# Acelogic/Retrieval-based-Voice-Conversion-MLX

Hardware: AMD Instinct MI355X
Metric: audio-sec/sec (realtime factor) RVCv2 48kHz pipeline (higher is better)
Workload: dtype fp32-accurate (two-plane fp16 MFMA split); 1 GPU; C2: full RVCv2 48kHz pipeline, one 13.5 s utterance per step per GPU; samples_16k=216100, x_pad=1, f0_method=rmvpe, parallelism=dp1

## Files before the change

### retrieval-based-voice-conversion-mlx_amd/csrc/aux_kernels.hip

```cpp
#include <algorithm>
#include <cmath>
#include <cstdlib>

#include "dd_math.h"
#include "rvcx_kernels.h"

namespace rvcx {

namespace {

constexpr int TB = 256;
typedef float f32x4v __attribute__((ext_vector_type(4)));

inline unsigned nblocks(long long n, int per = TB) {
  long long b = (n + per - 1) / per;
  if (b > 65535LL * 32) b = 65535LL * 32;
  return (unsigned)(b < 1 ? 1 : b);
}

__device__ __forceinline__ float warp_sum(float v) {
#pragma unroll
  for (int o = 32; o > 0; o >>= 1) v += __shfl_xor(v, o, 64);
  return v;
}
// ... 306 lines not shown
    const int src = t >> 1 < L ? t >> 1 : L - 1;
    const float f = feats[(long long)src * D + c];
    float v = f;
    if (pitchf) {
      const float pf = pitchf[t];
      const float p = pf < 1.f ? protect : (pf > 0.f ? 1.f : pf);
      v = f * p + feats0[(long long)src * D + c] * (1.f - p);
    }
    out[i] = v;
  }
}
#pragma clang fp contract(on)
hipError_t upsample2_protect(const float* feats, const float* feats0, int L, int D, float* out, int T,
                             const float* pitchf, float protect, hipStream_t s) {
  hipLaunchKernelGGL(k_up2, dim3(nblocks((long long)T * D)), dim3(TB), 0, s, feats, feats0, L, D, out, T, pitchf,
                     protect);
  return hipGetLastError();
}

constexpr int SINE_T = 1024;
__global__ __launch_bounds__(SINE_T) void k_sine_cum(const float* __restrict__ f0, int B, int L, int upp, float sr,
                                                     double* __restrict__ cum) {
  __shared__ double wsum[SINE_T / 64];
  const int b = blockIdx.x;
  const float* fb = f0 + (long long)b * L;
  float* cf = reinterpret_cast<float*>(cum + (long long)b * L);
  const int n = L - 1;
  if (n <= 0) return;
  const int per = (n + SINE_T - 1) / SINE_T;
  const int j0 = min(n, (int)threadIdx.x * per), j1 = min(n, j0 + per);
  auto rem_at = [&](int j) {
    const float inc = (fb[j] / sr) * (float)upp;
    return fmodf(inc + 0.5f, 1.0f) - 0.5f;
  };
  double s = 0.0;
  for (int j = j0; j < j1; ++j) s += (double)rem_at(j);
  const int lane = threadIdx.x & 63, w = threadIdx.x >> 6;
  double v = s;
#pragma unroll
  for (int d = 1; d < 64; d <<= 1) {
    const double u = __shfl_up(v, d);
    if (lane >= d) v += u;
  }
  if (lane == 63) wsum[w] = v;
  __syncthreads();
  double acc = v - s;
  for (int k = 0; k < w; ++k) acc += wsum[k];
  for (int j = j0; j < j1; ++j) {
    acc += (double)rem_at(j);
    cf[j] = fmodf((float)acc, 1.0f);
  }
}
__global__ void k_sine(const float* f0, int B, int L, int upp, float sr, const double* cum, const float* eps,
                       uint64_t seed, float lin_w, float lin_b, float* har, long long har_ld) {
  const long long n = (long long)B * L * upp;
  const float two_pi = 6.283185307179586f;
  const float amp_unv = (float)(0.1 / 3.0);
  for (long long i = blockIdx.x * (long long)blockDim.x + threadIdx.x; i < n; i += (long long)gridDim.x * blockDim.x) {
    const int u = (int)(i % upp);
    const long long bl = i / upp;
    const int b = (int)(bl / L), l = (int)(bl % L);
    const float f = f0[bl];
    float ph = (f / sr) * (float)(u + 1);
    if (l > 0) ph = ph + reinterpret_cast<const float*>(cum + (long long)b * L)[l - 1];
    const float sine = sinf(two_pi * ph) * 0.1f;
    const float uv = f > 0.f ? 1.f : 0.f;
    const float amp = uv * 0.003f + (1.f - uv) * amp_unv;
    const float e = eps ? eps[i] : normal_at(seed, (uint64_t)i);
    const float merged = sine * uv + amp * e;
    har[(long long)b * har_ld + (long long)l * upp + u] = tanhf(merged * lin_w + lin_b);
  }
}
hipError_t sine_source(const float* f0, int B, int L, int upp, float sr, const float* eps, uint64_t seed,
                       float lin_w, float lin_b, double* cum_ws, float* har, long long har_ld, hipStream_t s) {
  hipLaunchKernelGGL(k_sine_cum, dim3(B), dim3(SINE_T), 0, s, f0, B, L, upp, sr, cum_ws);
  hipLaunchKernelGGL(k_sine, dim3(nblocks((long long)B * L * upp)), dim3(TB), 0, s, f0, B, L, upp, sr, cum_ws, eps,
                     seed, lin_w, lin_b, har, har_ld);
  return hipGetLastError();
}

constexpr int CP_T = 256, CP_IT = 24;
__global__ __launch_bounds__(CP_T) void k_conv_post(const float* __restrict__ x, int T, int C,
                                                    const float* __restrict__ wg, int K, float slope,
                                                    float* __restrict__ y, float bias) {
  extern __shared__ float tile[];
  const int b = blockIdx.y;
  const int t0 = blockIdx.x * CP_T;
  const int pad = K / 2;
  const int rows = CP_T + K - 1;
  const int ldt = C + 1;
  const int C4 = C >> 2;
  float* w = tile + rows * ldt;
  for (int i = threadIdx.x; i < C * K; i += blockDim.x) w[i] = wg[i];
  const float* xb = x + (long long)b * T * C;
  f32x4v v[CP_IT];
#pragma unroll
  for (int it = 0; it < CP_IT; ++it) {
    const int idx = it * CP_T + threadIdx.x;
    const int r = idx / C4, c4 = (idx - r * C4) * 4;
    const int g = t0 - pad + r;
    v[it] = (r < rows && g >= 0 && g < T) ? *reinterpret_cast<const f32x4v*>(xb + (long long)g * C + c4)
                                          : f32x4v{0.f, 0.f, 0.f, 0.f};
  }
#pragma unroll
  for (int it = 0; it < CP_IT; ++it) {
    const int idx = it * CP_T + threadIdx.x;
    const int r = idx / C4, c4 = (idx - r * C4) * 4;
    if (r < rows) {
#pragma unroll
      for (int e = 0; e < 4; ++e) {
        const float u = v[it][e];
        tile[r * ldt + c4 + e] = u > 0.f ? u : u * slope;
      }
    }
  }
  __syncthreads();
  const int t = t0 + threadIdx.x;
  if (t >= T) return;
  float acc = 0.f;
  for (int c = 0; c < C; ++c)
    for (int k = 0; k < K; ++k) acc = fmaf(tile[(threadIdx.x + k) * ldt + c], w[c * K + k], acc);
  y[(long long)b * T + t] = tanhf(acc + bias);
}
constexpr int CPF_C = 32, CPF_K = 7, CPF_LD = 36, CPF_ROWS = CP_T + CPF_K - 1;
__global__ __launch_bounds__(CP_T) void k_conv_post32(const float* __restrict__ x, int T,
                                                      const float* __restrict__ wg, float slope,
                                                      float* __restrict__ y, float bias) {
  __shared__ __attribute__((aligned(16))) float tile[CPF_ROWS * CPF_LD];
  __shared__ __attribute__((aligned(16))) float w[CPF_K * CPF_C];
  const int b = blockIdx.y;
  const int t0 = blockIdx.x * CP_T;
  constexpr int pad = CPF_K / 2;
  constexpr int C4 = CPF_C / 4;
  constexpr int IT = (CPF_ROWS * C4 + CP_T - 1) / CP_T;
  if (threadIdx.x < CPF_K * CPF_C) {
    const int k = threadIdx.x / CPF_C, c = threadIdx.x - k * CPF_C;
    w[threadIdx.x] = wg[c * CPF_K + k];
  }
  const float* xb = x + (long long)b * T * CPF_C;
  f32x4v v[IT];
#pragma unroll
  for (int it = 0; it < IT; ++it) {
    const int idx = it * CP_T + threadIdx.x;
    const int r = idx / C4, c4 = (idx - r * C4) * 4;
    const int g = t0 - pad + r;
    const bool ok = r < CPF_ROWS && g >= 0 && g < T;
    v[it] = *reinterpret_cast<const f32x4v*>(xb + (long long)(ok ? g : 0) * CPF_C + c4);
    if (!ok) v[it] = f32x4v{0.f, 0.f, 0.f, 0.f};
  }
#pragma unroll
  for (int it = 0; it < IT; ++it) {
    const int idx = it * CP_T + threadIdx.x;
    const int r = idx / C4, c4 = (idx - r * C4) * 4;
    if (r < CPF_ROWS) {
      f32x4v u = v[it];
#pragma unroll
      for (int e = 0; e < 4; ++e) u[e] = u[e] > 0.f ? u[e] : u[e] * slope;
      *reinterpret_cast<f32x4v*>(&tile[r * CPF_LD + c4]) = u;
    }
  }
  __syncthreads();
  const int t = t0 + threadIdx.x;
  if (t >= T) return;
  f32x4v acc = {0.f, 0.f, 0.f, 0.f};
#pragma unroll
  for (int c4 = 0; c4 < C4; ++c4)
#pragma unroll
    for (int k = 0; k < CPF_K; ++k) {
      const f32x4v xv = *reinterpret_cast<const f32x4v*>(&tile[(threadIdx.x + k) * CPF_LD + 4 * c4]);
      const f32x4v wv = *reinterpret_cast<const f32x4v*>(&w[k * CPF_C + 4 * c4]);
#pragma unroll
      for (int e = 0; e < 4; ++e) acc[e] = fmaf(xv[e], wv[e], acc[e]);
    }
  y[(long long)b * T + t] = tanhf(((acc[0] + acc[1]) + (acc[2] + acc[3])) + bias);
}

hipError_t conv_post_tanh(const float* x, int B, int T, int C, const float* w, int K, float slope, float* y,
                          hipStream_t s, float bias) {
  if (C == CPF_C && K == CPF_K && (reinterpret_cast<uintptr_t>(x) & 15) == 0) {
    hipLaunchKernelGGL(k_conv_post32, dim3((T + CP_T - 1) / CP_T, B), dim3(CP_T), 0, s, x, T, w, slope, y, bias);
    return hipGetLastError();
  }
  if (C % 4 != 0 || (long long)(CP_T + K - 1) * (C / 4) > (long long)CP_IT * CP_T ||
      (reinterpret_cast<uintptr_t>(x) & 15) != 0)
    return hipErrorInvalidValue;
  const size_t smem = ((size_t)(CP_T + K - 1) * (C + 1) + (size_t)C * K) * sizeof(float);
  hipLaunchKernelGGL(k_conv_post, dim3((T + CP_T - 1) / CP_T, B), dim3(CP_T), smem, s, x, T, C, w, K, slope, y, bias);
  return hipGetLastError();
}

__global__ void k_zp(const float* stats, int B, int T, int I, const float* eps, uint64_t seed, const float* mask,
                     float* zp) {
  const long long n = (long long)B * T * I;
  for (long long i = blockIdx.x * (long long)blockDim.x + threadIdx.x; i < n; i += (long long)gridDim.x * blockDim.x) {
    const int c = (int)(i % I);
    const long long bt = i / I;
    const int b = (int)(bt / T), t = (int)(bt % T);
    const float m = stats[bt * 2 * I + c];
    const float lg = stats[bt * 2 * I + I + c];
    const long long ei = ((long long)b * I + c) * T + t;
    const float e = eps ? eps[ei] : normal_at(seed, (uint64_t)ei);
    zp[i] = (m + expf(lg) * e * 0.66666f) * mask[bt];
  }
}
hipError_t zp_sample(const float* stats, int B, int T, int I, const float* eps, uint64_t seed, const float* mask,
                     float* zp, hipStream_t s) {
  hipLaunchKernelGGL(k_zp, dim3(nblocks((long long)B * T * I)), dim3(TB), 0, s, stats, B, T, I, eps, seed, mask, zp);
  return hipGetLastError();
}

__global__ void k_gn_stats(const float* x, int T, int C, int chunk, double* ws) {
  const int c = blockIdx.x * 64 + (threadIdx.x & 63);
  const int rl = threadIdx.x >> 6;
  const int t0 = blockIdx.y * chunk;
  const int t1 = min(T, t0 + chunk);
  x += (long long)blockIdx.z * T * C;
  ws += (long long)blockIdx.z * gridDim.y * C * 2;
  double s = 0.0, q = 0.0;
  if (c < C) {
    for (int t = t0 + rl; t < t1; t += 4) {
      const double v = x[(long long)t * C + c];
      s += v;
      q += v * v;
    }
  }
  __shared__ double ss[4][64], qq[4][64];
  ss[rl][threadIdx.x & 63] = s;
  qq[rl][threadIdx.x & 63] = q;
  __syncthreads();
  if (rl == 0 && c < C) {
    s = ss[0][threadIdx.x] + ss[1][threadIdx.x] + ss[2][threadIdx.x] + ss[3][threadIdx.x];
    q = qq[0][threadIdx.x] + qq[1][threadIdx.x] + qq[2][threadIdx.x] + qq[3][threadIdx.x];
    ws[((long long)blockIdx.y * C + c) * 2] = s;
    ws[((long long)blockIdx.y * C + c) * 2 + 1] = q;
  }
}
__global__ void k_gn_finalize(const double* ws, int nchunks, int T, int C, const float* gamma, const float* beta,
                              float eps, float* ss) {
  const int c = blockIdx.x * 64 + (threadIdx.x & 63);
  const int rl = threadIdx.x >> 6;
  ws += (long long)blockIdx.y * nchunks * C * 2;
  ss += (long long)blockIdx.y * 2 * C;
  double s = 0.0, q = 0.0;
  if (c < C) {
    for (int k = rl; k < nchunks; k += 4) {
      s += ws[((long long)k * C + c) * 2];
      q += ws[((long long)k * C + c) * 2 + 1];
    }
  }
  __shared__ double sp[4][64], qp[4][64];
  sp[rl][threadIdx.x & 63] = s;
  qp[rl][threadIdx.x & 63] = q;
  __syncthreads();
  if (rl != 0 || c >= C) return;
  s = ((sp[0][threadIdx.x] + sp[1][threadIdx.x]) + sp[2][threadIdx.x]) + sp[3][threadIdx.x];
  q = ((qp[0][threadIdx.x] + qp[1][threadIdx.x]) + qp[2][threadIdx.x]) + qp[3][threadIdx.x];
  const double mean = s / T;
  double var = q / T - mean * mean;
  if (var < 0) var = 0;
  const float rstd = (float)(1.0 / sqrt(var + (double)eps));
  const float scale = rstd * gamma[c];
  ss[c] = scale;
  ss[C + c] = beta[c] - (float)mean * scale;
}
__global__ void k_gn_apply(float* __restrict__ x, unsigned n4, unsigned n4_per, unsigned C4, const float* __restrict__ ss,
                           int C) {
  for (unsigned i = blockIdx.x * blockDim.x + threadIdx.x; i < n4; i += gridDim.x * blockDim.x) {
    const int c = (int)(i % C4) * 4;
    const float* sb = ss + (size_t)(i / n4_per) * 2 * C;
    f32x4v v = reinterpret_cast<f32x4v*>(x)[i];
// ... 660 lines not shown
```

### retrieval-based-voice-conversion-mlx_amd/csrc/capi.cpp

```cpp
#include <algorithm>
#include <cmath>
#include <cstdio>
#include <cstdlib>
#include <cstring>
#include <string>
#include <unistd.h>
#include <vector>

#include "../../include/rvcx_test.h"
#include "runtime.h"

extern char** environ;

using namespace rvcx;

namespace rvcx {
static bool experimental_on() {
  const char* e = std::getenv("RVCX_EXPERIMENTAL");
  return e && std::atoi(e) == 1;
}
const char* rvcx_knob(const char* name) { return experimental_on() ? std::getenv(name) : nullptr; }
}

struct rvcx_ctx : public Ctx {};
// ... 160 lines not shown
  if (c.conv_math > 0 && b.math == 0) b.math = c.conv_math;
  if (!(b.w_static || c.is_weight(b.w)) || b.force_cfg >= 0) return false;
  if (!(conv_math_of(b) == 3 || b.lowp)) return false;
  if (conv_wsb_route(b, false) != 1) return false;
  b.wsb = 1;
  return conv_plan_splitk(b, false) == 0 && conv_wsb_pick(b) >= 23;
}

void launch_conv(Ctx& c, const ConvArgs& a_in, bool two_d, hipStream_t s, double flops) {
  ConvArgs a = a_in;
  if (c.conv_math > 0 && a.math == 0) a.math = c.conv_math;
  const bool stat = a.w_static || c.is_weight(a.w);
  a.wsb = !stat ? 0
          : (a.force_cfg >= 30 && a.force_cfg < 40 ? 2
             : (a.force_cfg >= 20 && !two_d) ? 1 : (a.force_cfg < 0 ? conv_wsb_route(a, two_d) : 0));
  if (a.force_cfg == 40 && !two_d && stat) a.wsb = 1;
  const long long need = conv_plan_splitk(a, two_d);
  if (two_d && !a.wsb && stat && !a.wsplit && conv_math_of(a) == 3 && conv2d_small_fits(a)) {
    a.wsplit_fmt = WSPLIT_S2D;
    a.wsplit = c.wsplit_for(a, s);
  }
  if (a.wsb) {
    if (!a.wsplit)
      a.wsplit_fmt = ((a.wsb == 1 && a.lowp) || conv_math_of(a) == 3) ? WSPLIT_H16 : WSPLIT_BF16;
    if (!a.wsplit) a.wsplit = c.wsplit_for(a, s);
    a.wsplit_npad = conv_wsplit_npad(a.N);
  }
  static const int aux_lds = [] {
    const char* e = rvcx_knob("RVCX_AUX_LDS");
    return e ? std::max(0, std::atoi(e)) : 64;
  }();
  if (aux_lds > 0 && c.aux_front) a.lds_pad = aux_lds * 1024;
  if (need > 0) {
    a.ws = c.buf<float>(c.aux && s == c.aux ? "conv.splitk.aux" : "conv.splitk", (size_t)need, s);
  }
  if (flops < 0) {
    const double M = two_d ? (double)a.T_out * a.W_out : (double)a.T_out;
    flops = 2.0 * M * a.N * (double)a.C_in * a.taps * a.batch * a.batch_inner;
  }
  if (!c.prof) {
    check(two_d ? conv2d(a, s) : conv1d(a, s), two_d ? "conv2d" : "conv1d");
    return;
  }
  auto get_ev = [&]() {
    hipEvent_t e;
    if (!c.prof_pool.empty()) {
      e = c.prof_pool.back();
      c.prof_pool.pop_back();
    } else {
      RVCX_HIP(hipEventCreate(&e));
    }
    return e;
  };
  const double in_rows = two_d ? (double)a.T_in * a.W_in : (double)a.T_in;
  const double out_el = (two_d ? (double)a.T_out * a.W_out : (double)a.T_out) * a.N * a.batch * a.batch_inner;
  const double alg_bytes = 4.0 * (in_rows * a.C_in * a.batch * a.batch_inner + (double)a.taps * a.N * a.C_in +
                                  out_el * (1 + (a.res && a.res_mode != RES_NONE ? 1 : 0) +
                                            (a.acc_mode != ACC_STORE ? 1 : 0)));
  const double peak = (a.wsb && a.wsplit_fmt == WSPLIT_H16) ? ((a.lowp && a.wsb == 1) ? Ctx::PEAK_F16 : Ctx::PEAK_F16X2)
                      : (a.wsplit && a.wsplit_fmt == WSPLIT_S2D) ? Ctx::PEAK_F16X2
                                                                  : Ctx::PEAK_SPLIT;
  Ctx::ProfRec r{get_ev(), get_ev(), flops, two_d ? 1 : 0, two_d ? a.T_out * a.W_out : a.T_out, a.N, a.C_in,
                 a.taps, a.batch * a.batch_inner, a.ksplit, alg_bytes, peak};
  RVCX_HIP(hipEventRecord(r.a, s));
  check(two_d ? conv2d(a, s) : conv1d(a, s), two_d ? "conv2d" : "conv1d");
  r.kind = conv_last_kind();
  RVCX_HIP(hipEventRecord(r.b, s));
  c.prof_recs.push_back(r);
}

__global__ void k_set_i32(int32_t* p, int32_t v) { p[0] = v; }
void set_i32(int32_t* p, int32_t v, hipStream_t s) {
  hipLaunchKernelGGL(k_set_i32, dim3(1), dim3(1), 0, s, p, v);
  check(hipGetLastError(), "set_i32");
}
void set_i32_once(Ctx& c, const std::string& name, int32_t* p, int32_t v, hipStream_t s) {
  auto it = c.i32_marks.find(name);
  if (it != c.i32_marks.end() && it->second.first == p && it->second.second == v) return;
  set_i32(p, v, s);
  c.i32_marks[name] = {p, v};
}
}

extern "C" {

int rvcx_create(rvcx_ctx** out, int device) {
  if (!out) return RVCX_E_INVALID;
  *out = nullptr;
  int n = 0;
  if (hipGetDeviceCount(&n) != hipSuccess || device < 0 || device >= n) return RVCX_E_HIP;
  auto* c = new rvcx_ctx();
  c->device = device;
  *out = c;
  return RVCX_OK;
}

int rvcx_destroy(rvcx_ctx* ctx) {
  if (!ctx) return RVCX_E_INVALID;
  (void)hipSetDevice(ctx->device);
  (void)hipDeviceSynchronize();
  delete ctx;
  return RVCX_OK;
}

const char* rvcx_last_error(const rvcx_ctx* ctx) { return ctx ? ctx->err.c_str() : "null context"; }

int rvcx_set_synth_config(rvcx_ctx* ctx, const rvcx_synth_desc* d) {
  return guard(ctx, [&] {
    if (!d) throw Error(RVCX_E_INVALID, "null desc");
    SynthCfg g;
    g.I = d->inter_channels;
    g.H = d->hidden_channels;
    g.F = d->filter_channels;
    g.n_heads = d->n_heads;
    g.n_layers = d->n_layers;
    g.ksize = d->kernel_size;
    if (d->n_resblocks < 1 || d->n_resblocks > 4 || d->n_dilations < 1 || d->n_dilations > 4)
      throw Error(RVCX_E_INVALID, "resblock config out of range");
    g.rb_k.assign(d->resblock_kernel_sizes, d->resblock_kernel_sizes + d->n_resblocks);
    g.rb_d.clear();
    for (int j = 0; j < d->n_resblocks; ++j)
      g.rb_d.emplace_back(d->resblock_dilation_sizes[j], d->resblock_dilation_sizes[j] + d->n_dilations);
    if (d->n_upsample < 1 || d->n_upsample > 8) throw Error(RVCX_E_INVALID, "n_upsample out of range");
    g.ups.assign(d->upsample_rates, d->upsample_rates + d->n_upsample);
    g.up_k.assign(d->upsample_kernel_sizes, d->upsample_kernel_sizes + d->n_upsample);
    g.C0 = d->upsample_initial_channel;
    g.n_spk = d->spk_embed_dim;
    g.gin = d->gin_channels;
    g.sr = d->sr;
    g.emb_dim = d->text_enc_hidden_dim;
    g.f0 = d->no_f0 == 0;
    g.vocoder = d->vocoder;
    if (g.vocoder < 0 || g.vocoder > 2) throw Error(RVCX_E_INVALID, "unsupported vocoder id");
    if (!g.f0 && g.vocoder != 0)
      throw Error(RVCX_E_INVALID, "models without pitch guidance use the HiFi-GAN decoder only (synthesizers.py:119-139)");
    if (g.H % g.n_heads || g.I % 2 || g.C0 % (1 << g.ups.size()))
      throw Error(RVCX_E_INVALID, "inconsistent synthesizer dimensions");
    ctx->scfg = g;
    ctx->synth_cfg_set = true;
    ctx->ready[0] = false;
  });
}

int rvcx_upload(rvcx_ctx* ctx, int model, const char* name, const float* host, const int64_t* shape, int ndim) {
  return guard(ctx, [&] {
    if (model < 0 || model > RVCX_MODEL_FCPE || !name || !host || (ndim > 0 && !shape) || ndim < 0 || ndim > 8)
      throw Error(RVCX_E_INVALID, "rvcx_upload: bad arguments");
    HostTensor t;
    size_t n = 1;
    for (int i = 0; i < ndim; ++i) {
      if (shape[i] < 0) throw Error(RVCX_E_INVALID, "negative dim");
      t.shape.push_back(shape[i]);
      n *= (size_t)shape[i];
    }
    t.v.assign(host, host + n);
    ctx->host[model][name] = std::move(t);
    ctx->ready[model] = false;
  });
}

int rvcx_finalize(rvcx_ctx* ctx, int model) {
  return guard(ctx, [&] {
    set_device(ctx);
    if (model == RVCX_MODEL_SYNTH) {
      finalize_synth(*ctx);
    } else if (model == RVCX_MODEL_HUBERT) {
      finalize_hubert(*ctx);
    } else if (model == RVCX_MODEL_RMVPE) {
      finalize_rmvpe(*ctx);
    } else if (model == RVCX_MODEL_CREPE) {
      finalize_crepe(*ctx);
    } else if (model == RVCX_MODEL_FCPE) {
      finalize_fcpe(*ctx);
    } else {
      throw Error(RVCX_E_INVALID, "unknown model");
    }
    RVCX_HIP(hipDeviceSynchronize());
    ctx->ready[model] = true;
  });
}

int rvcx_synth_upp(const rvcx_ctx* ctx) { return ctx ? ctx->scfg.upp() : 0; }

int rvcx_hubert(rvcx_ctx* ctx, const float* d_audio, int64_t n, int version, float* d_feats, int64_t cap_rows,
                int64_t* rows_out, void* stream) {
  return guard(ctx, [&] {
    if (!ctx->ready[1]) throw Error(RVCX_E_STATE, "hubert weights not finalized");
    if (!d_audio || !d_feats || n <= 0) throw Error(RVCX_E_INVALID, "rvcx_hubert: bad arguments");
    set_device(ctx);
    const int64_t L = hubert_forward(*ctx, d_audio, n, version == 1 ? 1 : 2, d_feats, cap_rows,
                                     static_cast<hipStream_t>(stream));
    if (rows_out) *rows_out = L;
  });
}

int rvcx_rmvpe(rvcx_ctx* ctx, const float* d_audio, int64_t n, float thred, double* d_f0, int64_t cap_frames,
               int64_t* frames_out, float* d_hidden, void* stream) {
  return guard(ctx, [&] {
    if (!ctx->ready[2]) throw Error(RVCX_E_STATE, "rmvpe weights not finalized");
    if (!d_audio || !d_f0 || n <= 0) throw Error(RVCX_E_INVALID, "rvcx_rmvpe: bad arguments");
    set_device(ctx);
    const int64_t F = rmvpe_forward(*ctx, d_audio, n, thred, d_f0, cap_frames, d_hidden,
                                    static_cast<hipStream_t>(stream));
    if (frames_out) *frames_out = F;
  });
}

int rvcx_crepe(rvcx_ctx* ctx, const float* d_audio, int64_t n, float f0_min, float f0_max, float threshold,
               float* d_f0, float* d_periodicity, float* d_probs, int64_t cap_frames, int64_t* frames_out,
               void* stream) {
  return guard(ctx, [&] {
    if (!ctx->ready[RVCX_MODEL_CREPE]) throw Error(RVCX_E_STATE, "crepe weights not finalized");
    if (!d_audio || !d_f0 || n <= 0) throw Error(RVCX_E_INVALID, "rvcx_crepe: bad arguments");
    if (cap_frames < 1 + n / 160) throw Error(RVCX_E_SHAPE, "rvcx_crepe: output capacity below 1 + n/160 frames");
    set_device(ctx);
    const int64_t F = crepe_forward(*ctx, d_audio, n, f0_min, f0_max, threshold, d_f0, nullptr, d_periodicity,
                                    d_probs, static_cast<hipStream_t>(stream));
    if (frames_out) *frames_out = F;
  });
}

// ... 381 lines not shown
    try {
      RVCX_HIP(hipMalloc(&audio.p, sizeof(double) * (size_t)(B * n)));
      RVCX_HIP(hipMalloc(&out.p, sizeof(float) * (size_t)(B * cap)));
      RVCX_HIP(hipMemsetAsync(audio.p, 0, sizeof(double) * (size_t)(B * n), s));
      auto measure = [&](const rvcx_pipeline_opts& o) {
        if (B == 1) {
          pipeline_forward_ex(*ctx, static_cast<const double*>(audio.p), n, o, nullptr, nullptr, 0,
                              static_cast<float*>(out.p), cap, nullptr, s);
        } else {
          std::vector<int32_t> sids((size_t)B, o.sid);
          pipeline_forward_batch(*ctx, static_cast<const double*>(audio.p), n, n, B, o, sids.data(), nullptr, nullptr, 0,
                                 static_cast<float*>(out.p), cap, nullptr, nullptr, s);
        }
        RVCX_HIP(hipStreamSynchronize(s));
        return (int64_t)ctx->carved;
      };
      need = measure(*opts);
      if (opts->f0_method == 3) {
        rvcx_pipeline_opts o0 = *opts;
        o0.f0_method = 0;
        ctx->release_pool();
        need = std::max(need, measure(o0));
      }
      if (B == 1 && opts->t_max > 0 && n + 160 > opts->t_max && opts->t_center > 0) {
        const int64_t nts = n > opts->t_center ? (n - 1 - opts->t_center) / opts->t_center + 1 : 0;
        need += (nts + 1) * ((int64_t)ctx->scfg.emb_dim * 4 + 512);
      }
    } catch (...) {
      ctx->release_pool();
      ctx->arena = arena;
      ctx->arena_bytes = arena_bytes;
      throw;
    }
    ctx->release_pool();
    ctx->arena = arena;
    ctx->arena_bytes = arena_bytes;
    *bytes = need;
  });
}

int rvcx_device_status(rvcx_ctx* ctx, void* stream) {
  return guard(ctx, [&] {
    RVCX_HIP(hipSetDevice(ctx->device));
    RVCX_HIP(hipStreamSynchronize(static_cast<hipStream_t>(stream)));
    if (ctx->aux) RVCX_HIP(hipStreamSynchronize(ctx->aux));
    ctx->check_device_status();
  });
}

int rvcx_index_parse(const void* bytes, int64_t nbytes, int64_t* d, int64_t* ntotal, int64_t* nlist,
                     int64_t* nprobe, char* err, int64_t err_cap) {
  try {
    if (!bytes || nbytes <= 0) throw Error(RVCX_E_INVALID, "index_parse: empty buffer");
    const ParsedIvf P = parse_ivf(static_cast<const uint8_t*>(bytes), nbytes);
    if (d) *d = P.d;
    if (ntotal) *ntotal = P.ntotal;
    if (nlist) *nlist = P.nlist;
    if (nprobe) *nprobe = P.nprobe;
    if (err && err_cap > 0) err[0] = 0;
    return RVCX_OK;
  } catch (const Error& e) {
    if (err && err_cap > 0) std::snprintf(err, (size_t)err_cap, "%s", e.what());
    return e.code;
  } catch (const std::exception& e) {
    if (err && err_cap > 0) std::snprintf(err, (size_t)err_cap, "%s", e.what());
    return RVCX_E_INVALID;
  }
}

int rvcx_set_conv_math(rvcx_ctx* ctx, int mode) {
  return guard(ctx, [&] {
    if (mode < 0 || mode > 3) throw Error(RVCX_E_INVALID, "conv math mode must be 0, 1, 2 or 3");
    ctx->conv_math = mode;
  });
}

int rvcx_config_info(const rvcx_ctx* ctx, char* buf, int64_t cap, int64_t* len) {
  std::string j = "{\"arch\": \"gfx950\"";
  if (ctx) j += ", \"conv_math_ctx\": " + std::to_string(ctx->conv_math);
  const char* cm = rvcx_knob("RVCX_CONV_MATH");
  j += ", \"conv_math_default\": \"" + std::string(cm ? cm : "h16") + "\"";
  j += ", \"experimental\": " + std::string(experimental_on() ? "true" : "false");
  if (ctx) j += ", \"arena_bytes\": " + std::to_string(ctx->arena_bytes);
  j += ", \"env\": {";
  bool first = true;
  for (char** e = environ; e && *e; ++e) {
    if (std::strncmp(*e, "RVCX_", 5) != 0) continue;
    const char* eq = std::strchr(*e, '=');
    if (!eq) continue;
    std::string k(*e, eq - *e), v(eq + 1);
    std::string ve;
    for (char ch : v)
      if (ch != '"' && ch != '\\' && (unsigned char)ch >= 32) ve += ch;
    const bool honoured = k == "RVCX_EXPERIMENTAL" || k == "RVCX_PROF_DUMP" || k == "RVCX_LIB" || experimental_on();
    j += std::string(first ? "" : ", ") + "\"" + k + "\": {\"value\": \"" + ve + "\", \"honoured\": " +
         (honoured ? "true" : "false") + "}";
    first = false;
  }
  j += "}}";
  if (len) *len = (int64_t)j.size();
  if (buf && cap > 0) {
    const size_t n = std::min<size_t>(j.size(), (size_t)cap - 1);
    std::memcpy(buf, j.data(), n);
    buf[n] = 0;
  }
  return (int64_t)j.size() < cap || !buf ? RVCX_OK : RVCX_E_CAPACITY;
}

int rvcx_set_generator_precision(rvcx_ctx* ctx, int) {
  return guard(ctx, [&] {
    throw Error(RVCX_E_INVALID,
                "rvcx_set_generator_precision was removed: set rvcx_rt_opts.gen_precision per streaming hop instead");
  });
}

int rvcx_conv1d(rvcx_ctx* ctx, const float* d_x, int64_t T, int C_in, const float* d_w, const float* d_bias, int N,
                int taps, int dilation, int pad, int stride, int math, float* d_y, int64_t T_out, void* stream) {
  return guard(ctx, [&] {
    set_device(ctx);
    ctx->check_device_status();
    if (!d_x || !d_w || !d_y || T <= 0 || C_in <= 0 || N <= 0 || taps <= 0 || dilation <= 0 || stride <= 0 ||
        pad < 0 || T_out <= 0 || math < 0 || math > 7)
      throw Error(RVCX_E_INVALID, "rvcx_conv1d: bad argument");
    if ((T_out - 1) * stride + (int64_t)(taps - 1) * dilation + 1 > T + 2 * (int64_t)pad)
      throw Error(RVCX_E_SHAPE, "rvcx_conv1d: T_out exceeds the padded input");
    if (T > INT32_MAX || T_out > INT32_MAX || (int64_t)taps * N * C_in > INT32_MAX)
      throw Error(RVCX_E_SHAPE, "rvcx_conv1d: size out of range");
    ConvArgs a;
    a.x = d_x; a.ldx = C_in; a.T_in = (int)T; a.C_in = C_in;
    a.w = d_w; a.ldw = C_in; a.w_ts = (long long)N * C_in; a.taps = taps; a.dil = dilation; a.pad = pad;
    a.stride = stride;
    a.y = d_y; a.ldy = N; a.T_out = (int)T_out; a.N = N; a.bias = d_bias;
    a.math = math >= 5 ? 3 : (math >= 3 ? 2 : math);
    if (math == 7) a.wsplit_fmt = WSPLIT_H16;
    if (math == 5 || math == 6) {
      a.wsplit_fmt = WSPLIT_H16;
      a.lowp = math == 6;
    }
    if (math == 3 || math == 5 || math == 6) {
      if (!conv_wsb_eligible(a)) throw Error(RVCX_E_SHAPE, "rvcx_conv1d: shape not eligible for the weight-streamed kernel");
      a.w_static = 1;
      a.force_cfg = conv_wsb_pick(a);
      a.no_splitk = 1;
      void* img = ctx->buf<char>("conv.test.wsplit", (size_t)conv_wsplit_bytes(a), static_cast<hipStream_t>(stream));
      check(conv_wsplit_build(a, img, static_cast<hipStream_t>(stream)), "conv_wsplit_build");
      a.wsplit = img;
    }
    if (math == 4 || math == 7) {
      if (!conv_gs_eligible(a, false)) throw Error(RVCX_E_SHAPE, "rvcx_conv1d: shape not eligible for the gather-streamed kernel");
      a.w_static = 1;
      a.force_cfg = 30;
      void* img = ctx->buf<char>("conv.test.wsplit", (size_t)conv_wsplit_bytes(a), static_cast<hipStream_t>(stream));
      check(conv_wsplit_build(a, img, static_cast<hipStream_t>(stream)), "conv_wsplit_build");
      a.wsplit = img;
    }
    launch_conv(*ctx, a, false, static_cast<hipStream_t>(stream), -1.0);
  });
}

int rvcx_conv1d_gen(rvcx_ctx* ctx, const float* d_x, int64_t T, int C_in, const float* d_w, const float* d_bias,
                    int N, int taps, int dilation, int pad, int pre_act, float pre_slope, int act, float slope,
                    const float* d_res, int acc_mode, float acc_div, int kernel, float* d_y, void* stream) {
  return guard(ctx, [&] {
    set_device(ctx);
    ctx->check_device_status();
    if (!d_x || !d_w || !d_y || T <= 0 || C_in <= 0 || N <= 0 || taps <= 0 || dilation <= 0 || pad < 0 || act < 0 ||
        act > 1 || pre_act < 0 || pre_act > 1 || acc_mode < 0 || acc_mode > 2 || kernel < 0 || kernel > 2 || (d_res && d_res == d_x))
      throw Error(RVCX_E_INVALID, "rvcx_conv1d_gen: bad argument");
    const int64_t T_out = T + 2 * (int64_t)pad - (int64_t)(taps - 1) * dilation;
    if (T_out <= 0 || T > INT32_MAX || (int64_t)taps * N * C_in > INT32_MAX)
      throw Error(RVCX_E_SHAPE, "rvcx_conv1d_gen: size out of range");
    ConvArgs a;
    a.x = d_x; a.ldx = C_in; a.T_in = (int)T; a.C_in = C_in;
    a.w = d_w; a.ldw = C_in; a.w_ts = (long long)N * C_in; a.taps = taps; a.dil = dilation; a.pad = pad;
    a.y = d_y; a.ldy = N; a.T_out = (int)T_out; a.N = N; a.bias = d_bias;
    a.pre_act = pre_act ? ACT_LRELU : ACT_NONE;
    a.pre_slope = pre_slope;
    a.act = act ? ACT_LRELU : ACT_NONE;
    a.slope = slope;
    if (d_res) {
      a.res = d_res;
      a.ldr = N;
      a.res_mode = RES_ADD_POST;
    }
    a.acc_mode = acc_mode == 0 ? ACC_STORE : (acc_mode == 1 ? ACC_ADD : ACC_ADD_DIV);
    a.acc_div = acc_div;
    a.math = 3;
    a.wsplit_fmt = WSPLIT_H16;
    a.w_static = 1;
// ... 474 lines not shown
```

### retrieval-based-voice-conversion-mlx_amd/csrc/conv_dispatch.hip

```cpp
#include <algorithm>
#include <cstdlib>
#include <string>

#include "conv_common.h"

namespace rvcx {

constexpr int CK = 32;

namespace {

inline int env_cfg(const char* name, int dflt) {
  const char* e = rvcx_knob(name);
  return e ? std::atoi(e) : dflt;
}
inline int conv_math(const ConvArgs& a) {
  static const int env = [] {
    const char* e = rvcx_knob("RVCX_CONV_MATH");
    if (e && (std::string(e) == "f32" || std::string(e) == "1")) return 1;
    if (e && (std::string(e) == "split" || std::string(e) == "2")) return 2;
    return 3;
  }();
  return a.math > 0 ? a.math : env;
}

template <bool TWO_D>
int pick_emu(const ConvArgs& a) {
  if (TWO_D) return a.N <= 32 ? 12 : 13;
  if (a.N <= 32) return a.taps >= 5 ? 12 : 1;
  if (a.taps >= 5) return 12;
  return 13;
}

template <bool TWO_D>
int pick_cfg(const ConvArgs& a) {
  if (a.force_cfg >= 0) return a.force_cfg;
  if (conv_math(a) >= 2) return pick_emu<TWO_D>(a);
  if (a.N <= 32) return 1;
  if (!TWO_D && a.taps >= 5) return 1;
  return 3;
}

inline void cfg_tile(int cfg, int& BM, int& BN) {
  if (conv_emu_tile(cfg, BM, BN)) return;
  static const int t[10][2] = {{256, 32}, {128, 32}, {128, 64}, {64, 64}, {128, 128}, {64, 128}, {256, 64},
                               {64, 64}, {128, 32}, {128, 128}};
  BM = t[cfg][0];
  BN = t[cfg][1];
}

inline int pick_wsb(const ConvArgs& a) {
  static const int c_long = env_cfg("RVCX_WCFG_LONG", 0);
  if (a.wsb == 2) return 30;
  if (a.N <= 32) return 24;
  if (a.taps <= 3 && a.N >= 1024 && a.T_out >= 8192 && a.C_in < 512 && c_long == 0) return 25;
  if (a.taps <= 3) return 27;
  if (c_long > 0) return c_long;
  return (a.C_in < 256 && a.N >= 128) ? 25 : 23;
}
}
int conv_wsb_pick(const ConvArgs& a) {
  ConvArgs b = a;
  b.wsb = 1;
  return pick_wsb(b);
}
thread_local int g_conv_kind = CK_OTHER;
int conv_last_kind() { return g_conv_kind; }
const char* conv_kind_name(int k) {
  static const char* const names[CK_COUNT] = {"conv_wsb16_kernel", "conv_wsb_kernel", "conv_gs16_kernel",
                                              "conv_gsw16_kernel", "k_rb_pair", "k_conv2d_h16/k_conv2d_small",
                                              "conv_emu_kernel", "conv_gemm_kernel", "conv_tiny_kernel",
                                              "conv_wst16_kernel", "other"};
  return (k >= 0 && k < CK_COUNT) ? names[k] : "other";
}

namespace {

template <bool TWO_D>
hipError_t dispatch(const ConvArgs& a_in, hipStream_t s) {
  const ConvArgs& a = a_in;
  if (a.N <= 0 || a.T_out <= 0 || a.batch <= 0) return hipSuccess;
  if (a.C_in <= 0 || a.taps <= 0) return hipErrorInvalidValue;
  const bool nz = a.nz_har != nullptr;
  if (nz && (TWO_D || (a.ws && a.ksplit > 1) || a.nz_C <= 0 || a.nz_stride <= 0 ||
             a.nz_kk != 1 ||
             a.N != a.nz_u * a.nz_C || a.out_map != OUT_ROWS))
    return hipErrorInvalidValue;
  if ((a.gate_h > 0 || a.ln_g) && !(a.ws && a.ksplit > 1)) return hipErrorInvalidValue;
  if (tiny_fits(a)) {
    if (nz) return hipErrorInvalidValue;
    g_conv_kind = CK_TINY;
    return launch_tiny(a, TWO_D, s);
  }
  if (!nz && !(a.ws && a.ksplit > 1) && rows1x1_fits(a, TWO_D)) {
    g_conv_kind = CK_TINY;
    return launch_rows1x1(a, TWO_D, s);
  }
  if (a.wsb == 2 && a.wsplit && conv_math(a) >= 2 && conv_gs_eligible(a, TWO_D)) {
    const int ks = (a.ws && a.ksplit > 1) ? a.ksplit : 1;
    const int cfg = a.force_cfg >= 30 ? a.force_cfg : pick_wsb(a);
    g_conv_kind = (TWO_D && cfg == 30 && conv_gsw_eligible(a)) ? CK_GSW : CK_GS;
    hipError_t e = conv_gs_launch(a, cfg, s, TWO_D, ks);
    if (e == hipSuccess && ks > 1) e = launch_splitk_reduce(a, ks, TWO_D, s);
    if (e != hipErrorInvalidValue) return e;
  }
  if (a.wsb == 1 && a.wsplit && conv_math(a) >= 2 && conv_wsb_eligible(a, TWO_D)) {
    const int ks = (a.ws && a.ksplit > 1) ? a.ksplit : 1;
    if (ks == 1 && (a.force_cfg < 20 || a.force_cfg == 40) && conv_wst_fits(a, TWO_D)) {
      g_conv_kind = CK_WST;
      hipError_t e = conv_wst_launch(a, s);
      if (e != hipErrorInvalidValue) return e;
    }
    const int cfg = a.force_cfg >= 20 && a.force_cfg < 40 ? a.force_cfg : pick_wsb(a);
    g_conv_kind = CK_WSB16;
    hipError_t e = conv_wsb_launch(a, cfg, s, TWO_D, ks);
    if (e == hipSuccess && ks > 1) e = launch_splitk_reduce(a, ks, TWO_D, s);
    if (e != hipErrorInvalidValue) return e;
  }
  if (nz) return hipErrorInvalidValue;
  if (TWO_D && a.force_cfg < 0 && conv2d_small_fits(a)) {
    g_conv_kind = CK_SMALL2D;
    return conv2d_small(a, s);
  }
  const int cfg = pick_cfg<TWO_D>(a);
  const bool emu = cfg >= 10;
  g_conv_kind = emu ? CK_EMU : CK_GEMM;
  const bool gemm = !TWO_D && a.taps == 1 && a.stride == 1;
  const bool pipe = gemm && a.pipe >= 0;
  const int ksplit = (a.ws && a.ksplit > 1) ? a.ksplit : 1;
  auto run = [&](int c, bool p) -> hipError_t {
    hipError_t e = emu ? conv_emu_launch(a, c, TWO_D, p, ksplit, s) : conv_gemm_launch(a, c, TWO_D, p, ksplit, s);
    if (e != hipSuccess || ksplit == 1) return e;
    return launch_splitk_reduce(a, ksplit, TWO_D, s);
  };
  hipError_t e = run(cfg, pipe);
  if (e == hipErrorInvalidValue && pipe) e = run(cfg, false);
  if (e == hipErrorInvalidValue && a.force_cfg < 0) {
    for (int alt : {emu ? 13 : 3, emu ? 12 : 1}) {
      if (alt == cfg) continue;
      e = run(alt, false);
      if (e != hipErrorInvalidValue) break;
    }
  }
  return e;
}

}

long long conv_plan_splitk(ConvArgs& a, bool two_d) {
  a.ksplit = 1;
  if (a.N <= 0 || a.T_out <= 0 || a.no_splitk) return 0;
  if (tiny_fits(a)) return 0;
  if (two_d && a.force_cfg < 0 && conv2d_small_fits(a)) return 0;
  int BM, BN;
  if (a.wsb == 2) {
    conv_gs_tile(a.force_cfg >= 30 ? a.force_cfg : pick_wsb(a), BM, BN);
  } else if (a.wsb) {
    if (!conv_wsb_tile(a.force_cfg >= 20 ? a.force_cfg : pick_wsb(a), BM, BN)) return 0;
  } else {
    cfg_tile(two_d ? pick_cfg<true>(a) : pick_cfg<false>(a), BM, BN);
  }
  long long mtiles;
  if (!two_d) {
    mtiles = (a.T_out + BM - 1) / BM;
  } else {
    const int rw = a.W_out < BM ? a.W_out : BM;
    const int rh = BM / rw;
    mtiles = (long long)((a.T_out + rh - 1) / rh) * ((a.W_out + rw - 1) / rw);
  }
  const long long tiles = mtiles * ((a.N + BN - 1) / BN) * a.batch * a.batch_inner;
  const int iters = ((a.C_in + CK - 1) / CK) * a.taps;
  const double M = two_d ? (double)a.T_out * a.W_out : (double)a.T_out;
  const double flops = 2.0 * M * a.N * (double)a.C_in * a.taps * a.batch * a.batch_inner;
  static const int target = env_cfg("RVCX_SPLITK_TARGET", 512);
  constexpr int min_tiles = 192;
  constexpr int min_iters = 4;
  const bool combine_epi = a.gate_h > 0 || a.ln_g;
  if (!combine_epi && (tiles >= min_tiles || iters < min_iters || (flops < 1.0e8 && iters < 16))) return 0;
  int ks = (int)((target + tiles - 1) / tiles);
  constexpr int gs_min_steps = 8;
  ks = std::min(ks, a.wsb == 2 ? iters / gs_min_steps : iters / 2);
  ks = std::min(ks, 32);
  if (a.wsb == 2 && two_d && (a.force_cfg < 0 || a.force_cfg == 30) && conv_gsw_eligible(a))
    ks = std::min(ks, (a.C_in + CK - 1) / CK);
  if (combine_epi && iters >= 2) ks = std::max(ks, 2);
  if (ks < 2) return 0;
  a.ksplit = ks;
  a.ws_rows = two_d ? (long long)a.T_out * a.W_out : a.T_out;
  return std::max((long long)ks * a.ws_rows * a.N * a.batch * a.batch_inner, tiles * ks * BM * BN);
}

bool conv_wsb_wants(const ConvArgs& a) {
  if (conv_math(a) < 2 || !conv_wsb_eligible(a)) return false;
  constexpr int min_taps = 2, min_tiles = 512, min_n = 64;
  if (a.N < min_n || a.taps < min_taps) return false;
  const long long tiles = (long long)((a.T_out + 127) / 128) * ((a.N + 63) / 64) * a.batch;
  return tiles >= min_tiles;
}

int conv_wsb_route(const ConvArgs& a, bool two_d) {
  if (conv_math(a) < 2 || tiny_fits(a)) return 0;
  if (two_d && conv2d_small_fits(a)) return 0;
  if (!two_d && conv_wsb_wants(a)) return 1;
  if (a.N >= 64 && conv_gs_eligible(a, two_d)) return 2;
  return 0;
}

int conv_math_of(const ConvArgs& a) { return conv_math(a); }
int conv_unstreamed_kind(const ConvArgs& a) {
  if (tiny_fits(a) || (!(a.ws && a.ksplit > 1) && rows1x1_fits(a, false))) return CK_TINY;
  return pick_cfg<false>(a) >= 10 ? CK_EMU : CK_GEMM;
}
hipError_t conv1d(const ConvArgs& a, hipStream_t s) { return dispatch<false>(a, s); }
hipError_t conv2d(const ConvArgs& a, hipStream_t s) { return dispatch<true>(a, s); }

}
```

### retrieval-based-voice-conversion-mlx_amd/csrc/runtime.h

```cpp
#pragma once
#include <hip/hip_runtime.h>

#include <cstdint>
#include <cstdlib>
#include <functional>
#include <map>
#include <memory>
#include <stdexcept>
#include <string>
#include <tuple>
#include <vector>

#include "../../include/rvcx.h"
#include "rvcx_kernels.h"

namespace rvcx {

struct Error : std::runtime_error {
  int code;
  Error(int c, const std::string& m) : std::runtime_error(m), code(c) {}
};

#define RVCX_HIP(expr)                                                                                 \
  do {                                                                                                 \
// ... 23 lines not shown

struct SynthCfg {
  int I = 192, H = 192, F = 768, n_heads = 2, n_layers = 6, ksize = 3;
  std::vector<int> rb_k{3, 7, 11};
  std::vector<std::vector<int>> rb_d{{1, 3, 5}, {1, 3, 5}, {1, 3, 5}};
  std::vector<int> ups{12, 10, 2, 2};
  int C0 = 512;
  std::vector<int> up_k{24, 20, 4, 4};
  int n_spk = 109, gin = 256, sr = 48000, emb_dim = 768;
  int window = 10, flow_k = 5, flow_layers = 3, flow_n = 4;
  bool f0 = true;
  int vocoder = 0;
  int upp() const {
    int u = 1;
    for (int x : ups) u *= x;
    return u;
  }
  int src_harmonics() const { return vocoder == 1 ? 9 : 1; }
  long long src_noise_row(long long T) const { return f0 ? T * upp() * src_harmonics() : 0; }
  long long src_noise_tail() const { return (f0 && vocoder != 0) ? src_harmonics() : 0; }
  long long src_noise_total(int B, long long T) const;
};

struct FcpeCfg {
  int sr = 16000, n_fft = 1024, win = 1024, hop = 160, n_mels = 128;
  double fmin = 0.0, fmax = 8000.0;
  int n_layers = 6, n_chans = 512, out_dims = 360;
  int n_heads = 8, dim_head = 64;
  int n_feat = 0;
  int conv_k = 31;
};

struct UpsLayer {
  int cin = 0, cout = 0, u = 0, k = 0, taps = 0, pad = 0;
  float* w = nullptr;
  float* b = nullptr;
};

struct IvfIndex {
  IvfView view;
  DevBuf cent, vecs, off, ids, slot_of_id;
};

struct Ctx {
  int device = 0;
  std::string err;
  SynthCfg scfg;
  bool synth_cfg_set = false;
  FcpeCfg fcfg;
  std::map<std::string, HostTensor> host[5];
  std::map<std::string, std::unique_ptr<DevBuf>> dev;
  bool ready[5] = {false, false, false, false, false};
  std::vector<UpsLayer> ups;
  int hp_order = 0;
  std::vector<double> hp_b, hp_a, hp_zi;
  SosPlan hp_sos;
  DevBuf hp_sos_buf;
  std::map<std::string, std::unique_ptr<DevBuf>> ws;
  uint64_t call_counter = 0;
  bool prof = false;
  int conv_math = 0;
  int conv_math_default() const {
    ConvArgs a;
    a.math = conv_math;
    return conv_math_of(a);
  }
  static constexpr double PEAK_SPLIT = 2500.0 / 6.0, PEAK_F16X2 = 2500.0 / 3.0, PEAK_F16 = 2500.0;
  struct ProfRec {
    hipEvent_t a, b;
    double flops;
    int two_d, M, N, C_in, taps, batch, ksplit;
    double bytes;
    double peak_tf;
    int kind = CK_OTHER;
  };
  std::vector<ProfRec> prof_recs;
  std::vector<hipEvent_t> prof_pool;
  std::unique_ptr<IvfIndex> ivf;
  std::map<std::tuple<const void*, int, long long, int, int, int, int>, std::unique_ptr<DevBuf>> wsplit_cache;
  const void* wsplit_for(const ConvArgs& a, hipStream_t s);
  std::map<std::pair<const void*, int>, std::unique_ptr<DevBuf>> rb_wsplit_cache;
  const void* rb_wsplit_for(const float* w, int C, int k, int wfmt, hipStream_t s);
  bool synth_full_lengths = false;
  bool aux_front = false;
  hipStream_t aux = nullptr;
  hipEvent_t ev_fork = nullptr, ev_join = nullptr, ev_gate = nullptr;
  hipStream_t aux_stream();
  std::function<void(hipStream_t)> before_gru;
  std::map<std::string, std::pair<const void*, long long>> zero_marks;
  std::map<std::string, std::pair<const void*, int32_t>> i32_marks;
  bool zero_once(const std::string& name, void* p, size_t bytes, long long layout, hipStream_t s) {
    auto& m = zero_marks[name];
    if (m.first == p && m.second == layout) return false;
    RVCX_HIP(hipMemsetAsync(p, 0, bytes, s));
    m = {p, layout};
    return true;
  }
  std::map<const void*, unsigned> gru_tags;
  unsigned* status_host = nullptr;
  unsigned* status_dev = nullptr;
  unsigned* device_status();
  void check_device_status();
  ~Ctx();

  float* W(const std::string& name) const;
  std::map<uintptr_t, uintptr_t> wranges;
  bool is_weight(const void* p) const;
  void drop_splits(uintptr_t lo, uintptr_t hi);
  float* alloc_weight(const std::string& name, const std::vector<float>& data);
  template <class T>
  T* buf(const std::string& name, size_t count, hipStream_t s);
  char* arena = nullptr;
  size_t arena_bytes = 0, arena_used = 0;
  size_t carved = 0;
  bool sizing_plan = false;
  std::vector<hipStream_t> call_streams;
  std::vector<std::pair<hipStream_t, hipEvent_t>> prev_call_events;
  std::map<hipStream_t, hipEvent_t> call_ev;
  void begin_call() {
    prev_call_events.clear();
    for (hipStream_t st : call_streams) {
      hipEvent_t& e = call_ev[st];
      if (!e) RVCX_HIP(hipEventCreateWithFlags(&e, hipEventDisableTiming));
      RVCX_HIP(hipEventRecord(e, st));
      prev_call_events.emplace_back(st, e);
    }
    call_streams.clear();
    arena_rewind();
  }
  void touch_stream(hipStream_t s) {
    for (hipStream_t st : call_streams)
      if (st == s) return;
    call_streams.push_back(s);
    for (const auto& pe : prev_call_events)
      if (pe.first != s) RVCX_HIP(hipStreamWaitEvent(s, pe.second, 0));
  }
  void arena_rewind() {
    if (!arena) return;
    ws.clear();
    zero_marks.clear();
    i32_marks.clear();
    gru_tags.clear();
    arena_used = 0;
    carved = 0;
  }
  void release_pool() {
    RVCX_HIP(hipDeviceSynchronize());
    ws.clear();
    zero_marks.clear();
    i32_marks.clear();
    gru_tags.clear();
    arena_used = 0;
    carved = 0;
  }
  size_t pool_bytes() const {
    size_t t = 0;
    for (const auto& kv : ws) t += kv.second ? kv.second->bytes : 0;
    return t;
  }
};

template <class T>
T* Ctx::buf(const std::string& name, size_t count, hipStream_t s) {
  size_t bytes = count * sizeof(T);
  if (bytes == 0) bytes = 16;
  bytes = (bytes + 255) & ~size_t(255);
  touch_stream(s);
  auto& slot = ws[name];
  if (!slot || slot->bytes < bytes) {
    if (slot && slot->p) RVCX_HIP(hipStreamSynchronize(s));
    slot.reset(new DevBuf());
    if (arena) {
      const size_t off = (arena_used + 255) & ~size_t(255);
      if (off + bytes > arena_bytes) {
        ws.erase(name);
        throw Error(RVCX_E_OOM, "workspace arena exhausted: " + name + " needs " + std::to_string(bytes) + " B at offset " +
                                    std::to_string(off) + " of " + std::to_string(arena_bytes));
      }
      slot->p = arena + off;
      slot->borrowed = true;
      arena_used = off + bytes;
    } else if (hipMalloc(&slot->p, bytes) != hipSuccess) {
      (void)hipGetLastError();
      ws.erase(name);
      throw Error(RVCX_E_OOM, "workspace allocation failed: " + name + " (" + std::to_string(bytes) + " B)");
    }
    slot->bytes = bytes;
    carved += bytes;
  }
  return static_cast<T*>(slot->p);
}

void finalize_synth(Ctx& c);
void finalize_refinegan(Ctx& c);
long long refinegan_noise_floats(const SynthCfg& g, int B, long long T);
void refinegan_forward(Ctx& c, int B, int T, const float* z_btc, const float* mask, const float* f0, const float* g,
                       const float* eps_src, uint64_t seed, float* out, hipStream_t s);
void finalize_hubert(Ctx& c);
void finalize_rmvpe(Ctx& c);
void finalize_crepe(Ctx& c);
void finalize_fcpe(Ctx& c);
int64_t fcpe_frames(const Ctx& c, int64_t n);
int fcpe_mel(Ctx& c, const float* audio, int64_t n, int64_t ld, int B, float* mel, hipStream_t s);
int64_t fcpe_forward_b(Ctx& c, const float* audio, int64_t n, int64_t ld, int B, float thr, int mode, double* f0,
                       int64_t cap, float* sal_out, hipStream_t s);
int64_t fcpe_forward(Ctx& c, const float* audio, int64_t n, float thr, int mode, int interp_uv, int64_t pad_to,
                     double* f0, float* sal_out, int64_t cap, hipStream_t s);
int64_t fcpe_decode_run(Ctx& c, const float* sal, int64_t F, float thr, int mode, int interp_uv, int64_t pad_to,
                        double* f0, hipStream_t s);
int64_t split_intervals(Ctx& c, const double* audio, int64_t n, int sr, double silence_thresh_db, int min_silence_ms,
                        int64_t* iv, int64_t cap, hipStream_t s);
int64_t crepe_forward(Ctx& c, const float* audio, int64_t n, double f0_min, double f0_max, float thr, float* f0,
                      double* f0d, float* per, float* probs_out, hipStream_t s, int sem = 0,
                      const float* dither = nullptr);
int64_t hubert_forward(Ctx& c, const float* audio, int64_t n, int version, float* feats, int64_t cap,
                       hipStream_t s);
constexpr int HUBERT_LAYERS = 12;
struct HubertRun {
  int B = 0, L = 0, version = 0;
  float* feats = nullptr;
};
HubertRun hubert_front(Ctx& c, const float* audio, int64_t n, int64_t lda, int B, int version, float* feats,
                       int64_t cap, hipStream_t s);
void hubert_layers(Ctx& c, const HubertRun& run, int l0, int l1, hipStream_t s);
int64_t hubert_tail(Ctx& c, const HubertRun& run, hipStream_t s);
int64_t rmvpe_forward(Ctx& c, const float* audio, int64_t n, float thred, double* f0, int64_t cap, float* hidden,
                      hipStream_t s);
int64_t hubert_forward_b(Ctx& c, const float* audio, int64_t n, int64_t lda, int B, int version, float* feats,
                         int64_t cap, hipStream_t s);
int64_t rmvpe_forward_b(Ctx& c, const float* audio, int64_t n, int64_t lda, int B, float thred, double* f0,
                        int64_t cap, float* hidden, hipStream_t s);
void synth_forward(Ctx& c, int B, int T, const float* phone, const int32_t* lengths, const int32_t* pitch,
                   const float* pitchf, const int32_t* sid, const float* eps_z, const float* eps_src, uint64_t seed,
                   float* out, float* zp_out, float* z_out, hipStream_t s, int gen_lowp = 0, int head = 0,
                   float* mp_out = nullptr, float* logsp_out = nullptr);
void dec_forward(Ctx& c, int B, int T, const float* z_btc, const float* mask, const float* f0, const float* g,
                 const float* eps_src, uint64_t seed, float* out, hipStream_t s, int gen_lowp = 0,
                 bool noise_pre = false);
bool dec_noise_prepare(Ctx& c, int B, int T, const float* f0, const float* eps_src, uint64_t seed, hipStream_t s);

void set_highpass(Ctx& c, const double* b, const double* a, const double* zi, int order);
void set_highpass_sos(Ctx& c, const double* sos, int nsec);
void highpass_pad(Ctx& c, const double* audio, int64_t n, int64_t t_pad, double* pad64, float* pad32, hipStream_t s);
int hubert_version_for(const Ctx& c);
int64_t vc_forward(Ctx& c, const float* audio, int64_t n, const int32_t* pitch, const float* pitchf,
                   int64_t pitch_len, int sid, float protect, double index_rate, const float* eps_z,
                   const float* eps_src, uint64_t seed, float* out, int64_t cap, hipStream_t s,
                   const float* feats_pre = nullptr, int64_t L_pre = 0);
struct RtState;
RtState* rt_create(Ctx& c, const rvcx_rt_desc& d);
void rt_destroy(RtState* s);
void rt_geometry(const RtState& s, int64_t* g);
void rt_reset(Ctx& c, RtState& s, hipStream_t st);
void rt_reset_stream(Ctx& c, RtState& s, int stream_index, hipStream_t st);
int rt_streams(const RtState& s);
void rt_process(Ctx& c, RtState& s, const float* in48, const int32_t* sids, const rvcx_rt_opts* opts,
                const uint8_t* active, const float* eps_z, const float* eps_src, uint64_t seed, float* out48,
                float* vol_out, int* offs_out, hipStream_t st);
struct ParsedIvf {
  int d = 0, nprobe = 1;
  long long nlist = 0, ntotal = 0;
  std::vector<float> cent, vecs;
  std::vector<long long> off, ids;
  std::vector<int> slot;
};
ParsedIvf parse_ivf(const uint8_t* bytes, int64_t nbytes);
void index_load(Ctx& c, const uint8_t* bytes, int64_t nbytes);
void index_search(Ctx& c, const float* x, int64_t n, int k, float* dist, int64_t* ids, hipStream_t s);
void index_retrieve(Ctx& c, const float* feats, int64_t L, int d, double index_rate, float* out, hipStream_t s);
void index_retrieve_rows(Ctx& c, const float* feats, int64_t L, int64_t off, int d, int n_seq, const int* seqs,
                         const float* rate, const float* one_minus_rate, float* out, hipStream_t s);
void index_reconstruct_n(Ctx& c, int64_t i0, int64_t ni, float* out, hipStream_t s);
int64_t pipeline_forward_ex(Ctx& c, const double* audio, int64_t n, const rvcx_pipeline_opts& o,
                            const float* eps_z, const float* eps_src, uint64_t seed, float* out, int64_t cap,
                            double* f0_out, hipStream_t s);
int64_t pipeline_forward_batch(Ctx& c, const double* audio, int64_t n, int64_t lda, int B, const rvcx_pipeline_opts& o,
                               const int32_t* sids, const float* eps_z, const float* eps_src, uint64_t seed,
                               float* out, int64_t ldo, double* f0_out, float* hidden_out, hipStream_t s);
rvcx_pipeline_opts default_pipeline_opts();
int proposed_key(const std::vector<double>& f0, double threshold);
int64_t hubert_frames(int64_t n);
void set_i32(int32_t* p, int32_t v, hipStream_t s);
void set_i32_once(Ctx& c, const std::string& name, int32_t* p, int32_t v, hipStream_t s);
hipStream_t fork_aux(Ctx& c, hipStream_t s);
bool conv_routes_wsb16(Ctx& c, const ConvArgs& a);
struct ScopedFullLengths {
  Ctx& c;
  explicit ScopedFullLengths(Ctx& cc) : c(cc) { c.synth_full_lengths = true; }
  ~ScopedFullLengths() { c.synth_full_lengths = false; }
};
void join_aux(Ctx& c, hipStream_t s, hipStream_t ax);
void launch_conv(Ctx& c, const ConvArgs& a_in, bool two_d, hipStream_t s, double flops = -1.0);
void launch_rb_pair(Ctx& c, const RbPairArgs& a, hipStream_t s);
inline void check(hipError_t e, const char* what) {
  if (e != hipSuccess) throw Error(RVCX_E_HIP, std::string(what) + ": " + hipGetErrorString(e));
}

}
```

### retrieval-based-voice-conversion-mlx_amd/csrc/runtime_pipeline.cpp

```cpp
#include <algorithm>
#include <cmath>
#include <cstdlib>
#include <cstring>

#include "runtime.h"

namespace rvcx {

void set_highpass(Ctx& c, const double* b, const double* a, const double* zi, int order) {
  if (order < 1 || order > IIR_MAXO) throw Error(RVCX_E_INVALID, "highpass order out of range");
  if (!(a[0] != 0.0)) throw Error(RVCX_E_INVALID, "highpass a[0] == 0");
  c.hp_order = order;
  c.hp_sos = SosPlan();
  c.hp_b.assign(b, b + order + 1);
  c.hp_a.assign(a, a + order + 1);
  c.hp_zi.assign(zi, zi + order);
  const double a0 = a[0];
  for (auto& v : c.hp_b) v /= a0;
  for (auto& v : c.hp_a) v /= a0;
}

void set_highpass_sos(Ctx& c, const double* sos, int nsec) {
  if (nsec < 1 || nsec > IIR_MAXO) throw Error(RVCX_E_INVALID, "highpass: bad section count");
  SosPlan p;
// ... 34 lines not shown
  const size_t casc_off = tab.size();
  tab.resize(casc_off + 48 + 64 * 12 + 8 * (size_t)L, 0.0);
  double* ct = tab.data() + casc_off;
  std::vector<double> A((size_t)NS * NS), C(NS);
  auto step = [&](const double* z, double x, double* zo) {
    double u = x;
    for (int j = 0; j < nsec; ++j) {
      const double* t = tab.data() + (size_t)j * p.stride();
      const double y = t[0] * u + z[2 * j];
      zo[2 * j] = t[1] * u - t[3] * y + z[2 * j + 1];
      zo[2 * j + 1] = t[2] * u - t[4] * y;
      u = y;
    }
    return u;
  };
  for (int i = 0; i < NS; ++i) {
    std::vector<double> z(NS, 0.0), zo(NS, 0.0);
    z[i] = 1.0;
    C[i] = step(z.data(), 0.0, zo.data());
    for (int r = 0; r < NS; ++r) A[(size_t)r * NS + i] = zo[r];
  }
  for (int j = 0; j < nsec; ++j) {
    const double* t = tab.data() + (size_t)j * p.stride();
    for (int q = 0; q < 5; ++q) ct[5 * j + q] = t[q];
    ct[40 + 2 * j] = t[8];
    ct[40 + 2 * j + 1] = t[9];
  }
  auto mul = [&](const std::vector<double>& X, const std::vector<double>& Y) {
    std::vector<double> Z((size_t)NS * NS, 0.0);
    for (int r = 0; r < NS; ++r)
      for (int q = 0; q < NS; ++q)
        for (int k = 0; k < NS; ++k) Z[(size_t)r * NS + q] += X[(size_t)r * NS + k] * Y[(size_t)k * NS + q];
    return Z;
  };
  std::vector<double> M((size_t)NS * NS, 0.0);
  for (int i = 0; i < NS; ++i) M[(size_t)i * NS + i] = 1.0;
  std::vector<double> row(C);
  for (int k = 0; k < L; ++k) {
    for (int i = 0; i < NS; ++i) ct[48 + 64 * 12 + 8 * k + i] = row[i];
    std::vector<double> nr(NS, 0.0);
    for (int q = 0; q < NS; ++q)
      for (int i = 0; i < NS; ++i) nr[q] += row[i] * A[(size_t)i * NS + q];
    row = nr;
    M = mul(A, M);
  }
  for (int sidx = 0; sidx < 12; ++sidx) {
    for (int r = 0; r < NS; ++r)
      for (int q = 0; q < NS; ++q) ct[48 + 64 * sidx + 8 * r + q] = M[(size_t)r * NS + q];
    M = mul(M, M);
  }
  RVCX_HIP(hipSetDevice(c.device));
  c.hp_sos_buf.~DevBuf();
  new (&c.hp_sos_buf) DevBuf();
  const size_t bytes = tab.size() * sizeof(double);
  if (hipMalloc(&c.hp_sos_buf.p, bytes) != hipSuccess) {
    (void)hipGetLastError();
    throw Error(RVCX_E_OOM, "highpass: device allocation failed");
  }
  c.hp_sos_buf.bytes = bytes;
  RVCX_HIP(hipMemcpy(c.hp_sos_buf.p, tab.data(), bytes, hipMemcpyHostToDevice));
  p.dev = static_cast<const double*>(c.hp_sos_buf.p);
  p.casc = p.dev + casc_off;
  c.hp_sos = p;
}

void highpass_pad(Ctx& c, const double* audio, int64_t n, int64_t t_pad, double* pad64, float* pad32, hipStream_t s) {
  if (c.hp_order == 0) throw Error(RVCX_E_STATE, "pipeline: high-pass filter not configured");
  if (c.hp_sos.nsec > 0) {
    double* ws = c.buf<double>("pl.sosws", filtfilt_sos_ws_doubles(n, c.hp_order, c.hp_sos.L), s);
    check(filtfilt_sos_pad(c.hp_sos, c.hp_order, audio, n, t_pad, ws, pad64, pad32, s), "filtfilt_sos");
    return;
  }
  double* ws = c.buf<double>("pl.iirws", filtfilt_ws_doubles(n, c.hp_order), s);
  check(filtfilt_pad(audio, n, c.hp_b.data(), c.hp_a.data(), c.hp_zi.data(), nullptr, c.hp_order, t_pad, ws, pad64,
                     pad32, s),
        "filtfilt_pad");
}

int hubert_version_for(const Ctx& c) { return c.scfg.emb_dim == 256 ? 1 : 2; }

int64_t vc_forward(Ctx& c, const float* audio, int64_t n, const int32_t* pitch, const float* pitchf,
                   int64_t pitch_len, int sid, float protect, double index_rate, const float* eps_z,
                   const float* eps_src, uint64_t seed, float* out, int64_t cap, hipStream_t s,
                   const float* feats_pre, int64_t L_pre) {
  if (sid < 0 || sid >= c.scfg.n_spk) throw Error(RVCX_E_INVALID, "sid out of range");
  const int E = c.scfg.emb_dim;
  const float* feats = feats_pre;
  int64_t L = L_pre;
  if (!feats) {
    const int64_t cap_rows = n / 320 + 8;
    float* fb = c.buf<float>("vc.feats", (size_t)cap_rows * E, s);
    L = hubert_forward(c, audio, n, hubert_version_for(c), fb, cap_rows, s);
    feats = fb;
  }
  const int T = (int)std::min<int64_t>(n / 160, 2 * L);
  if (T <= 0) throw Error(RVCX_E_SHAPE, "voice_conversion: input shorter than one frame");
  if (c.scfg.f0 && (!pitch || !pitchf)) throw Error(RVCX_E_INVALID, "voice_conversion: pitch-guided model needs pitch");
  if (!c.scfg.f0) pitch = nullptr, pitchf = nullptr;
  if (pitch && T > pitch_len) throw Error(RVCX_E_SHAPE, "voice_conversion: pitch track shorter than the features");
  const int upp = c.scfg.upp();
  if ((int64_t)T * upp > cap)
    throw Error(RVCX_E_CAPACITY, "voice_conversion: output needs " + std::to_string((int64_t)T * upp) + " samples");
  const float* fx = feats;
  if (index_rate > 0 && c.ivf) {
    float* fr = c.buf<float>("vc.feats_idx", (size_t)L * E, s);
    index_retrieve(c, feats, L, E, index_rate, fr, s);
    fx = fr;
  }
  float* phone = c.buf<float>("vc.phone", (size_t)T * E, s);
  check(upsample2_protect(fx, feats, (int)L, E, phone, T, protect < 0.5f ? pitchf : nullptr, protect, s),
        "upsample");
  int32_t* lens = c.buf<int32_t>("vc.len", 4, s);
  set_i32_once(c, "vc.len.T", lens, T, s);
  set_i32_once(c, "vc.len.sid", lens + 1, sid, s);
  {
    ScopedFullLengths full(c);
    synth_forward(c, 1, T, phone, lens, pitch, pitchf, lens + 1, eps_z, eps_src, seed, out, nullptr, nullptr, s);
  }
  return (int64_t)T * upp;
}

int proposed_key(const std::vector<double>& f0, double threshold) {
  std::vector<int64_t> valid;
  for (size_t i = 0; i < f0.size(); ++i)
    if (f0[i] > 0) valid.push_back((int64_t)i);
  if (valid.size() < 2) return 0;
  std::vector<double> v(f0.size());
  size_t k = 0;
  for (size_t i = 0; i < f0.size(); ++i) {
    const int64_t x = (int64_t)i;
    if (x <= valid.front()) {
      v[i] = f0[valid.front()];
    } else if (x >= valid.back()) {
      v[i] = f0[valid.back()];
    } else {
      while (valid[k + 1] < x) ++k;
      const double x0 = (double)valid[k], x1 = (double)valid[k + 1];
      const double y0 = f0[valid[k]], y1 = f0[valid[k + 1]];
      v[i] = (x == valid[k + 1]) ? y1 : y0 + (y1 - y0) * ((double)x - x0) / (x1 - x0);
    }
  }
  std::sort(v.begin(), v.end());
  const size_t m = v.size();
  const double med = (m & 1) ? v[m / 2] : 0.5 * (v[m / 2 - 1] + v[m / 2]);
  if (!(med > 0)) return 0;
  const double key = std::nearbyint(12.0 * std::log2(threshold / med));
  return (int)std::max(-12.0, std::min(12.0, key));
}

static void check_f0_method(const Ctx& c, const rvcx_pipeline_opts& o) {
  if (o.f0_method < 0 || o.f0_method > 3)
    throw Error(RVCX_E_INVALID, "pipeline: f0_method must be 0 (rmvpe), 1 (crepe, MLX), 2 (crepe, rvc/) or 3 (fcpe)");
  if (!c.scfg.f0) return;
  if ((o.f0_method == 1 || o.f0_method == 2) && !c.ready[RVCX_MODEL_CREPE])
    throw Error(RVCX_E_STATE, "pipeline: f0_method crepe but no CREPE weights finalized");
  if (o.f0_method == 3) {
    if (!c.ready[RVCX_MODEL_FCPE]) throw Error(RVCX_E_STATE, "pipeline: f0_method fcpe but no FCPE weights finalized");
    if (c.fcfg.sr != 16000 || c.fcfg.hop != 160)
      throw Error(RVCX_E_SHAPE, "pipeline: the FCPE model must run at 16 kHz with hop_size 160");
  }
}
static float fcpe_thr(const rvcx_pipeline_opts& o) { return o.fcpe_threshold > 0 ? o.fcpe_threshold : 0.006f; }

int64_t pipeline_forward_ex(Ctx& c, const double* audio, int64_t n, const rvcx_pipeline_opts& o,
                            const float* eps_z, const float* eps_src, uint64_t seed, float* out, int64_t cap,
                            double* f0_out, hipStream_t s) {
  if (c.hp_order == 0) throw Error(RVCX_E_STATE, "pipeline: high-pass filter not configured");
  if (o.t_pad < 0 || o.t_pad_tgt < 0 || o.t_pad >= n) throw Error(RVCX_E_INVALID, "pipeline: bad t_pad");
  check_f0_method(c, o);
  if (o.index_rate > 0 && !c.ivf) throw Error(RVCX_E_STATE, "pipeline: index_rate > 0 but no feature index loaded");
  if (o.index_rate > 0 && c.ivf->view.d != c.scfg.emb_dim)
    throw Error(RVCX_E_SHAPE, "pipeline: feature index dimension does not match the model's feature width");
  if (o.version != 0 && o.version != hubert_version_for(c))
    throw Error(RVCX_E_INVALID, "pipeline: version does not match the synthesizer's embedding width");
  const int64_t W = 160;
  const int64_t m = n + 2 * o.t_pad;
  float* pad32 = c.buf<float>("pl.pad32", (size_t)m, s);
  double* pad64 = c.buf<double>("pl.pad64", (size_t)m, s);
  highpass_pad(c, audio, n, o.t_pad, pad64, pad32, s);
  const double* filtered = pad64 + o.t_pad;
  std::vector<int64_t> opt_ts;
  if (o.t_max > 0 && n + W > o.t_max && o.t_center > 0) {
    if (o.t_query <= 0 || o.t_query > o.t_center) throw Error(RVCX_E_INVALID, "pipeline: bad t_query/t_center");
    const int nts = n > o.t_center ? (int)((n - 1 - o.t_center) / o.t_center + 1) : 0;
    double* sum = c.buf<double>("pl.winsum", (size_t)n, s);
    long long* dts = c.buf<long long>("pl.ts", (size_t)std::max(1, nts), s);
    check(split_points(filtered, n, (int)W, o.t_center, o.t_query, sum, dts, nts, s), "split_points");
    opt_ts.resize(nts);
    if (nts > 0 && c.sizing_plan) {
      for (int k = 0; k < nts; ++k) opt_ts[k] = (int64_t)(k + 1) * o.t_center;
      if (nts == 1) opt_ts[0] += o.t_query;
      else opt_ts[0] -= o.t_query, opt_ts[1] += o.t_query;
      for (auto& t : opt_ts) t = std::max<int64_t>(0, std::min<int64_t>(t, n - 1));
    } else if (nts > 0) {
      RVCX_HIP(hipMemcpyAsync(opt_ts.data(), dts, sizeof(long long) * nts, hipMemcpyDeviceToHost, s));
      RVCX_HIP(hipStreamSynchronize(s));
      c.check_device_status();
    }
  }
  struct Chunk {
// ... 68 lines not shown
  if (guided) {
  double* f0 = c.buf<double>("pl.f0", (size_t)F, s);
  if (o.f0_method >= 1) {
    if (c.before_gru) {
      auto rest = std::move(c.before_gru);
      c.before_gru = nullptr;
      gate_here(s);
      rest(s);
    }
    if (o.f0_method == 3) {
      fcpe_forward(c, pad32, m, fcpe_thr(o), 0, 0, 0, f0, nullptr, F, s);
    } else {
      float* f0f = c.buf<float>("pl.f0f", (size_t)F, s);
      crepe_forward(c, pad32, m, 50.0, 1100.0, 0.1f, f0f, f0, nullptr, nullptr, s, o.f0_method == 2 ? 1 : 0);
    }
  } else {
    rmvpe_forward(c, pad32, m, o.rmvpe_threshold > 0 ? o.rmvpe_threshold : 0.03f, f0, F, nullptr, s);
  }
  if (c.before_gru) {
    auto rest = std::move(c.before_gru);
    c.before_gru = nullptr;
    gate_here(s);
    rest(s);
  }
  double shift_semitones = o.pitch;
  if (o.f0_autotune) {
    check(f0_autotune(f0, (int)F, o.f0_autotune_strength, o.mlx_semantics ? 1 : 0, s), "f0_autotune");
    if (!o.mlx_semantics) shift_semitones = 0.0;
  } else if (o.proposed_pitch) {
    std::vector<double> h(F);
    RVCX_HIP(hipMemcpyAsync(h.data(), f0, sizeof(double) * F, hipMemcpyDeviceToHost, s));
    RVCX_HIP(hipStreamSynchronize(s));
    c.check_device_status();
    shift_semitones = o.pitch + proposed_key(h, o.proposed_pitch_threshold);
  }
  pitch = c.buf<int32_t>("pl.pitch", (size_t)F, s);
  pitchf = c.buf<float>("pl.pitchf", (size_t)F, s);
  check(f0_post(f0, (int)F, std::pow(2.0, shift_semitones / 12.0), pitch, pitchf, f0_out, s), "f0_post");
  } else {
    auto rest = std::move(c.before_gru);
    c.before_gru = nullptr;
    gate_here(s);
    rest(s);
    if (f0_out) RVCX_HIP(hipMemsetAsync(f0_out, 0, sizeof(double) * (size_t)F, s));
  }
  join_aux(c, s, ax);
  const int upp = c.scfg.upp();
  const int I = c.scfg.I;
  const size_t nch = chunks.size();
  std::vector<int64_t> ez_off(nch), es_off(nch), pos(nch);
  std::vector<uint64_t> cseed(nch);
  int64_t written = 0;
  {
    int64_t ez = 0, es = 0;
    uint64_t sd = seed;
    for (size_t i = 0; i < nch; ++i) {
      ez_off[i] = ez;
      es_off[i] = es;
      cseed[i] = sd;
      pos[i] = written;
      if (nch > 1) {
        const int64_t T = std::min<int64_t>((chunks[i].a1 - chunks[i].a0) / W, 2 * cL[i]);
        ez += (int64_t)I * T;
        es += c.scfg.src_noise_total(1, T);
        const int64_t keep = T * upp - 2 * o.t_pad_tgt;
        if (keep <= 0) throw Error(RVCX_E_SHAPE, "pipeline: chunk too short for the padding");
        written += keep;
      }
      sd += 0x9E3779B97F4A7C15ull;
    }
    if (written > cap)
      throw Error(RVCX_E_CAPACITY, "pipeline: output needs more than " + std::to_string(cap) + " samples");
  }
  const bool fuse_trim = nch == 1 && o.volume_envelope == 1.0;
  const float* trimmed = out;
  for (size_t i : order) {
    const Chunk& ch = chunks[i];
    const int64_t len = ch.a1 - ch.a0;
    const int64_t cap_vc = (len / W) * upp;
    float* vc = c.buf<float>("pl.vc", (size_t)std::max<int64_t>(cap_vc, 1), s);
    const int64_t nvc = vc_forward(c, pad32 + ch.a0, len, pitch ? pitch + ch.f_lo : nullptr,
                                   pitchf ? pitchf + ch.f_lo : nullptr, ch.f_hi - ch.f_lo, o.sid,
                                   o.protect, o.index_rate, eps_z ? eps_z + ez_off[i] : nullptr,
                                   eps_src ? eps_src + es_off[i] : nullptr, cseed[i], vc, cap_vc, s, cfeats[i], cL[i]);
    const int64_t keep = nvc - 2 * o.t_pad_tgt;
    if (keep <= 0) throw Error(RVCX_E_SHAPE, "pipeline: chunk too short for the padding");
    if (nch == 1) {
      if (keep > cap)
        throw Error(RVCX_E_CAPACITY, "pipeline: output needs more than " + std::to_string(cap) + " samples");
      written = keep;
    }
    if (fuse_trim)
      trimmed = vc + o.t_pad_tgt;
    else
      RVCX_HIP(hipMemcpyAsync(out + pos[i], vc + o.t_pad_tgt, (size_t)keep * sizeof(float), hipMemcpyDeviceToDevice,
                              s));
  }
  if (o.volume_envelope != 1.0) {
    const int n1 = rms_frame_count(n, 16000), n2 = rms_frame_count(written, c.scfg.sr);
    float* rws = c.buf<float>("pl.rms", (size_t)(n1 + n2), s);
    check(change_rms(filtered, n, 16000, out, written, c.scfg.sr, (float)o.volume_envelope, rws, s), "change_rms");
  }
  float* mx = c.buf<float>("pl.max", peak_normalize_ws_floats(1), s);
  check(peak_normalize(trimmed, out, written, mx, s), "peak_normalize");
  return written;
}

int64_t pipeline_forward_batch(Ctx& c, const double* audio, int64_t n, int64_t lda, int B, const rvcx_pipeline_opts& o,
                               const int32_t* sids, const float* eps_z, const float* eps_src, uint64_t seed,
                               float* out, int64_t ldo, double* f0_out, float* hidden_out, hipStream_t s) {
  if (B < 1) throw Error(RVCX_E_INVALID, "pipeline_batch: B < 1");
  if (c.hp_order == 0) throw Error(RVCX_E_STATE, "pipeline: high-pass filter not configured");
  if (o.t_pad < 0 || o.t_pad_tgt < 0 || o.t_pad >= n) throw Error(RVCX_E_INVALID, "pipeline: bad t_pad");
  check_f0_method(c, o);
  if (o.t_max > 0 && n + 160 > o.t_max)
    throw Error(RVCX_E_INVALID, "pipeline_batch: utterances longer than t_max take the single-utterance path");
  if (o.index_rate > 0 && !c.ivf) throw Error(RVCX_E_STATE, "pipeline: index_rate > 0 but no feature index loaded");
  if (o.version != 0 && o.version != hubert_version_for(c))
    throw Error(RVCX_E_INVALID, "pipeline: version does not match the synthesizer's embedding width");
  for (int b = 0; b < B; ++b)
    if (sids[b] < 0 || sids[b] >= c.scfg.n_spk) throw Error(RVCX_E_INVALID, "pipeline_batch: sid out of range");
  const int64_t W = 160;
  const int64_t m = n + 2 * o.t_pad;
  const int64_t ldm = (m + 7) & ~int64_t(7);
  const int E = c.scfg.emb_dim, upp = c.scfg.upp();
  float* pad32 = c.buf<float>("pb.pad32", (size_t)B * ldm, s);
  double* pad64 = c.buf<double>("pb.pad64", (size_t)B * m, s);
  for (int b = 0; b < B; ++b)
    highpass_pad(c, audio + (size_t)b * lda, n, o.t_pad, pad64 + (size_t)b * m, pad32 + (size_t)b * ldm, s);
  const int64_t F = 1 + m / W, T = m / W;
  double* f0 = c.buf<double>("pb.f0", (size_t)B * F, s);
  const int64_t L = hubert_frames(m);
  float* feats = c.buf<float>("pb.feats", (size_t)B * L * E, s);
  hipStream_t ax = fork_aux(c, s);
  hubert_forward_b(c, pad32, m, ldm, B, hubert_version_for(c), feats, L, ax);
  const bool guided = c.scfg.f0;
  int32_t* pitch = nullptr;
  float* pitchf = nullptr;
  if (guided) {
  if (o.f0_method == 3) {
    for (int b = 0; b < B; ++b)
      fcpe_forward(c, pad32 + (size_t)b * ldm, m, fcpe_thr(o), 0, 0, 0, f0 + (size_t)b * F, nullptr, F, s);
  } else if (o.f0_method >= 1) {
    float* f0f = c.buf<float>("pb.f0f", (size_t)F, s);
    for (int b = 0; b < B; ++b)
      crepe_forward(c, pad32 + (size_t)b * ldm, m, 50.0, 1100.0, 0.1f, f0f, f0 + (size_t)b * F, nullptr, nullptr, s,
                    o.f0_method == 2 ? 1 : 0);
  } else {
    rmvpe_forward_b(c, pad32, m, ldm, B, o.rmvpe_threshold > 0 ? o.rmvpe_threshold : 0.03f, f0, F, hidden_out, s);
  }
  std::vector<double> shift(B, o.pitch);
  if (o.f0_autotune) {
    check(f0_autotune(f0, (int)(B * F), o.f0_autotune_strength, o.mlx_semantics ? 1 : 0, s), "f0_autotune");
    if (!o.mlx_semantics) std::fill(shift.begin(), shift.end(), 0.0);
  } else if (o.proposed_pitch) {
    std::vector<double> h((size_t)B * F);
    RVCX_HIP(hipMemcpyAsync(h.data(), f0, sizeof(double) * h.size(), hipMemcpyDeviceToHost, s));
    RVCX_HIP(hipStreamSynchronize(s));
    c.check_device_status();
    for (int b = 0; b < B; ++b) {
      std::vector<double> one(h.begin() + (size_t)b * F, h.begin() + (size_t)(b + 1) * F);
      shift[b] = o.pitch + proposed_key(one, o.proposed_pitch_threshold);
    }
  }
  pitch = c.buf<int32_t>("pb.pitch", (size_t)B * F, s);
  pitchf = c.buf<float>("pb.pitchf", (size_t)B * F, s);
  for (int b = 0; b < B; ++b)
    check(f0_post(f0 + (size_t)b * F, (int)F, std::pow(2.0, shift[b] / 12.0), pitch + (size_t)b * F,
                  pitchf + (size_t)b * F, f0_out ? f0_out + (size_t)b * F : nullptr, s),
          "f0_post");
  } else if (f0_out) {
    RVCX_HIP(hipMemsetAsync(f0_out, 0, sizeof(double) * (size_t)B * F, s));
  }
  join_aux(c, s, ax);
  const int64_t Tv = std::min<int64_t>(T, 2 * L);
  if (Tv <= 0) throw Error(RVCX_E_SHAPE, "pipeline_batch: input shorter than one frame");
  const float* fx = feats;
  if (o.index_rate > 0) {
    if (c.ivf->view.d != E) throw Error(RVCX_E_SHAPE, "pipeline: feature index dimension mismatch");
    float* fr = c.buf<float>("pb.feats_idx", (size_t)B * L * E, s);
    index_retrieve(c, feats, B * L, E, o.index_rate, fr, s);
    fx = fr;
  }
  float* phone = c.buf<float>("pb.phone", (size_t)B * Tv * E, s);
  int32_t* pc = nullptr;
  float* pf = nullptr;
  if (guided) {
    pc = c.buf<int32_t>("pb.pc", (size_t)B * Tv, s);
    pf = c.buf<float>("pb.pf", (size_t)B * Tv, s);
    RVCX_HIP(hipMemcpy2DAsync(pc, Tv * sizeof(int32_t), pitch, F * sizeof(int32_t), Tv * sizeof(int32_t), B,
                              hipMemcpyDeviceToDevice, s));
    RVCX_HIP(hipMemcpy2DAsync(pf, Tv * sizeof(float), pitchf, F * sizeof(float), Tv * sizeof(float), B,
                              hipMemcpyDeviceToDevice, s));
  }
  for (int b = 0; b < B; ++b)
    check(upsample2_protect(fx + (size_t)b * L * E, feats + (size_t)b * L * E, (int)L, E, phone + (size_t)b * Tv * E,
                            (int)Tv, (guided && o.protect < 0.5f) ? pf + (size_t)b * Tv : nullptr, o.protect, s),
          "upsample");
  int32_t* meta = c.buf<int32_t>("pb.meta", 2 * (size_t)B, s);
  std::vector<int32_t> hm(2 * (size_t)B);
  for (int b = 0; b < B; ++b) {
    hm[b] = (int32_t)Tv;
    hm[B + b] = sids[b];
  }
  RVCX_HIP(hipMemcpyAsync(meta, hm.data(), sizeof(int32_t) * hm.size(), hipMemcpyHostToDevice, s));
  const int64_t nvc = Tv * upp;
  float* vc = c.buf<float>("pb.vc", (size_t)B * nvc, s);
  {
    ScopedFullLengths full(c);
    synth_forward(c, B, (int)Tv, phone, meta, pc, pf, meta + B, eps_z, eps_src, seed, vc, nullptr, nullptr, s);
  }
  const int64_t keep = nvc - 2 * o.t_pad_tgt;
  if (keep <= 0) throw Error(RVCX_E_SHAPE, "pipeline_batch: utterance too short for the padding");
  if (keep > ldo) throw Error(RVCX_E_CAPACITY, "pipeline_batch: output rows need " + std::to_string(keep));
  float* mx = c.buf<float>("pb.max", peak_normalize_ws_floats(B), s);
  if (o.volume_envelope == 1.0) {
    check(peak_normalize(vc + o.t_pad_tgt, out, keep, mx, s, B, nvc, ldo), "peak_normalize");
    return keep;
  }
  RVCX_HIP(hipMemcpy2DAsync(out, ldo * sizeof(float), vc + o.t_pad_tgt, nvc * sizeof(float), keep * sizeof(float), B,
                            hipMemcpyDeviceToDevice, s));
  for (int b = 0; b < B; ++b) {
    const int n1 = rms_frame_count(n, 16000), n2 = rms_frame_count(keep, c.scfg.sr);
    float* rws = c.buf<float>("pl.rms", (size_t)(n1 + n2), s);
    check(change_rms(pad64 + (size_t)b * m + o.t_pad, n, 16000, out + (size_t)b * ldo, keep, c.scfg.sr,
                     (float)o.volume_envelope, rws, s),
          "change_rms");
  }
  check(peak_normalize(out, out, keep, mx, s, B, ldo, ldo), "peak_normalize");
  return keep;
}

rvcx_pipeline_opts default_pipeline_opts() {
  rvcx_pipeline_opts o;
  std::memset(&o, 0, sizeof(o));
  o.version = 0;
  o.protect = 0.33f;
  o.rmvpe_threshold = 0.03f;
  o.t_pad = 16000;
  o.t_pad_tgt = 48000;
  o.t_query = 16000 * 6;
  o.t_center = 16000 * 38;
  o.t_max = 16000 * 41;
  o.f0_autotune_strength = 1.0;
  o.proposed_pitch_threshold = 155.0;
  o.volume_envelope = 1.0;
  o.fcpe_threshold = 0.006f;
  return o;
}

}
```

### retrieval-based-voice-conversion-mlx_amd/csrc/runtime_stream.cpp

```cpp
#include <cmath>
#include <cstring>

#include "runtime.h"

namespace rvcx {

namespace {

struct SincKernel {
  int orig = 1, nw = 1, width = 0, K = 0;
  std::vector<float> k;
};

SincKernel sinc_kernel(int orig_freq, int new_freq) {
  auto gcd = [](int a, int b) {
    while (b) {
      const int t = a % b;
      a = b;
      b = t;
    }
    return a;
  };
  const int g = gcd(orig_freq, new_freq);
  SincKernel r;
// ... 303 lines not shown
  const int64_t L = hubert_frames(s.conv16);
  float* feats = c.buf<float>("rt.feats", (size_t)Ba * L * E, st);
  hipStream_t ax = fork_aux(c, st);
  hubert_forward_b(c, conv, s.conv16, s.conv16, Ba, hubert_version_for(c), feats, L, ax);
  if (guided) {
  if (s.f0_method == 1) {
    if (!c.ready[RVCX_MODEL_FCPE] || c.fcfg.sr != 16000 || c.fcfg.hop != 160)
      throw Error(RVCX_E_STATE, "stream: the FCPE model this group was created with has been replaced");
    if (fcpe_forward_b(c, conv + s.silence_front, nf, s.conv16, Ba, s.fcpe_thr, 0, f0, F, nullptr, st) != F)
      throw Error(RVCX_E_SHAPE, "stream: FCPE frame count differs from the pitch track's");
  } else {
    rmvpe_forward_b(c, conv + s.silence_front, nf, s.conv16, Ba, 0.03f, f0, F, nullptr, st);
  }
  }
  if (all) upload_plan();
  if (guided) {
  if (any_tune)
    check(f0_autotune_rows(f0, F, reinterpret_cast<const double*>(dplan + P.strength),
                           reinterpret_cast<const int*>(dplan + P.autotune), Ba, st),
          "f0_autotune");
  if (n_prop > 0) {
    std::vector<double> h((size_t)Ba * F);
    for (int r = 0; r < Ba;) {
      auto asks = [&](int q) { return !opts[row2slot[q]].f0_autotune && opts[row2slot[q]].proposed_pitch; };
      if (!asks(r)) {
        ++r;
        continue;
      }
      int e = r + 1;
      while (e < Ba && asks(e)) ++e;
      RVCX_HIP(hipMemcpyAsync(h.data() + (size_t)r * F, f0 + (size_t)r * F, sizeof(double) * (size_t)(e - r) * F,
                              hipMemcpyDeviceToHost, st));
      r = e;
    }
    RVCX_HIP(hipStreamSynchronize(st));
    c.check_device_status();
    for (int r = 0; r < Ba; ++r) {
      const rvcx_rt_opts& o = opts[row2slot[r]];
      if (o.f0_autotune || !o.proposed_pitch) continue;
      std::vector<double> one(h.begin() + (size_t)r * F, h.begin() + (size_t)(r + 1) * F);
      h_fac[r] = std::pow(2.0, (o.f0_up_key + proposed_key(one, o.proposed_pitch_threshold)) / 12.0);
    }
    RVCX_HIP(hipMemcpyAsync(dplan + P.factor, h_fac, sizeof(double) * Ba, hipMemcpyHostToDevice, st));
  }
  check(rt_pitch(f0, F, d_fac, static_cast<const int*>(s.pbuf[s.cur].p), static_cast<int*>(s.pbuf[nxt].p),
                 static_cast<const float*>(s.fbuf[s.cur].p), static_cast<float*>(s.fbuf[nxt].p), s.pbuf_n, d_s2r, B,
                 st),
        "rt_pitch");
  } else if (!all) {
    RVCX_HIP(hipMemcpyAsync(s.pbuf[nxt].p, s.pbuf[s.cur].p, s.pbuf[nxt].bytes, hipMemcpyDeviceToDevice, st));
    RVCX_HIP(hipMemcpyAsync(s.fbuf[nxt].p, s.fbuf[s.cur].p, s.fbuf[nxt].bytes, hipMemcpyDeviceToDevice, st));
  }
  join_aux(c, st, ax);
  const float* fx = feats;
  if (n_ret > 0) {
    float* fr = c.buf<float>("rt.feats_idx", (size_t)Ba * L * E, st);
    RVCX_HIP(hipMemcpyAsync(fr, feats, sizeof(float) * (size_t)Ba * L * E, hipMemcpyDeviceToDevice, st));
    index_retrieve_rows(c, feats, L, s.skip_head / 2, E, n_ret, reinterpret_cast<const int*>(dplan + P.seqs),
                        reinterpret_cast<const float*>(dplan + P.rate),
                        reinterpret_cast<const float*>(dplan + P.one_minus_rate), fr, st);
    fx = fr;
  }
  float* phone = c.buf<float>("rt.phone", (size_t)Ba * T * E, st);
  int32_t* pitch = c.buf<int32_t>("rt.pitch", (size_t)Ba * T, st);
  float* pitchf = c.buf<float>("rt.pitchf", (size_t)Ba * T, st);
  const double formant = std::ceil(s.return_length * 1.0);
  const float pscale = (float)(formant / (double)s.return_length);
  check(rt_up2(fx, feats, (int)L, E, phone, T, static_cast<const float*>(s.fbuf[nxt].p), s.pbuf_n, pscale,
               reinterpret_cast<const float*>(dplan + P.protect), reinterpret_cast<const int*>(dplan + P.use_protect),
               pitch, static_cast<const int*>(s.pbuf[nxt].p), pitchf, d_r2s, Ba, st),
        "rt_up2");
  const int64_t n_model = (int64_t)T * upp;
  if (!all && eps_z) {
    float* ez = c.buf<float>("rt.eps_z", (size_t)Ba * I * T, st);
    check(gather_rows(eps_z, I * T, d_r2s, ez, Ba, I * T, st), "rt_eps_z");
    eps_z = ez;
  }
  if (!all && eps_src) {
    float* es = c.buf<float>("rt.eps_src", (size_t)Ba * n_model, st);
    check(gather_rows(eps_src, (int)n_model, d_r2s, es, Ba, (int)n_model, st), "rt_eps_src");
    eps_src = es;
  }
  float* model = c.buf<float>("rt.model", (size_t)Ba * n_model, st);
  {
    ScopedFullLengths full(c);
    synth_forward(c, Ba, T, phone, dmeta, guided ? pitch : nullptr, guided ? pitchf : nullptr, dmeta + B, eps_z,
                  eps_src, seed, model, nullptr, nullptr, st, gen_precision);
  }
  check(rt_clip(model, n_model, (int)n_model, Ba, st), "rt_clip");
  if (any_rms) {
    const int n1 = rms_frame_count(s.conv16, 16000), n2 = rms_frame_count(n_model, s.tgt_sr);
    float* ws = c.buf<float>("rt.rms", (size_t)Ba * (n1 + n2), st);
    check(change_rms_f32src_rows(conv, s.conv16, s.conv16, 16000, model, n_model, n_model, s.tgt_sr,
                                 reinterpret_cast<const float*>(dplan + P.rms), ws, Ba, st),
          "change_rms");
  }
  const float* a48 = model;
  int64_t lda = n_model;
  const float* scale = static_cast<const float*>(s.volsq.p);
  if (!s.out_identity) {
    const int64_t n48 = (int64_t)std::ceil((double)s.kout.nw * n_model / s.kout.orig);
    float* r48 = c.buf<float>("rt.model48", (size_t)Ba * n48, st);
    check(rt_resample(model, n_model, (int)n_model, static_cast<const float*>(s.d_kout.p), s.kout.K, s.kout.width,
                      s.kout.orig, s.kout.nw, r48, n48, (int)n48, scale, nullptr, Ba, st),
          "rt_resample_out");
    a48 = r48;
    lda = n48;
    scale = nullptr;
  }
  check(rt_sola(a48, lda, scale, static_cast<const int*>(s.gate.p), static_cast<float*>(s.sola.p), s.cross48,
                s.sola48, static_cast<const float*>(s.fade_in.p), out48, s.block48,
                offs_out ? offs_out : static_cast<int*>(s.offs.p), d_s2r, B, st),
        "rt_sola");
  if (vol_out) RVCX_HIP(hipMemcpyAsync(vol_out, s.vol.p, sizeof(float) * B, hipMemcpyDeviceToDevice, st));
  s.cur = nxt;
}

}
```

### retrieval-based-voice-conversion-mlx_amd/csrc/runtime_synth.cpp

```cpp
#include <algorithm>
#include <cmath>
#include <cstring>

#include "runtime.h"

namespace rvcx {

namespace {
constexpr long long HAR_PAD = 64;

uint64_t splitmix(uint64_t x) {
  x += 0x9E3779B97F4A7C15ull;
  x = (x ^ (x >> 30)) * 0xBF58476D1CE4E5B9ull;
  x = (x ^ (x >> 27)) * 0x94D049BB133111EBull;
  return x ^ (x >> 31);
}

const HostTensor& get(Ctx& c, int model, const std::string& n, std::vector<int64_t> shape) {
  auto it = c.host[model].find(n);
  if (it == c.host[model].end()) throw Error(RVCX_E_STATE, "missing weight: " + n);
  if (it->second.shape != shape) {
    std::string got, want;
    for (auto s : it->second.shape) got += std::to_string(s) + ",";
    for (auto s : shape) want += std::to_string(s) + ",";
// ... 281 lines not shown
                                       : n;
          c.alloc_weight(n + ".w", pack_conv1d(get(c, M, nref + ".weight", {C, C, k})));
          c.alloc_weight(n + ".b", get(c, M, nref + ".bias", {C}).v);
        }
      }
    }
  }
  const int Cl = C0 >> nu;
  c.alloc_weight("dec.post.w", get(c, M, "dec.conv_post.weight", {1, Cl, 7}).v);
  const float post_b = mrf ? get(c, M, "dec.conv_post.bias", {1}).v[0] : 0.f;
  c.host[M]["__post_b__"] = HostTensor{{post_b}, {1}};
}

namespace {
struct NoiseFrame {
  int stride = 1, kern = 1, npad = 0, ntap = 1;
};
NoiseFrame noise_frame(const SynthCfg& cf, size_t i) {
  NoiseFrame f;
  for (size_t j = i + 1; j < cf.ups.size(); ++j) f.stride *= cf.ups[j];
  f.kern = f.stride == 1 ? 1 : f.stride * 2 - f.stride % 2;
  f.npad = f.stride == 1 ? 0 : (f.kern - f.stride) / 2;
  f.ntap = f.kern == 1 ? 1 : 2;
  if (f.npad > HAR_PAD || f.ntap * f.stride - f.npad > HAR_PAD + f.stride)
    throw Error(RVCX_E_SHAPE, "noise conv stride too large for the source padding");
  return f;
}
bool noise_row_kernel(const NoiseFrame& f, int B, long long Ti, int C) {
  return f.ntap * f.stride <= 16 && C % 4 == 0 && (long long)B * Ti * (C / 4) < (1LL << 31) && f.ntap * f.stride * C <= 4096;
}
float* dec_source(Ctx& c, int B, int T, const float* f0, const float* eps_src, uint64_t seed, hipStream_t s) {
  const SynthCfg& cf = c.scfg;
  const int upp = cf.upp();
  const long long Nh = (long long)T * upp;
  const long long har_ld = Nh + 2 * HAR_PAD;
  float* har = c.buf<float>("dec.har", (size_t)(B * har_ld), s);
  c.zero_once("dec.har", har, sizeof(float) * (size_t)(B * har_ld), har_ld * 65536 + B, s);
  const auto& lin_wb = c.host[0].at("__src_lin__").v;
  const uint64_t sseed = splitmix(seed ^ 0x5352434e4f495345ull);
  if (cf.vocoder == 0) {
    double* cum = c.buf<double>("dec.cum", (size_t)B * T, s);
    check(sine_source(f0, B, T, upp, (float)cf.sr, eps_src, sseed, lin_wb[0], lin_wb[1], cum, har + HAR_PAD, har_ld, s),
          "sine_source");
  } else {
    const int Hs = cf.src_harmonics();
    double* ws = c.buf<double>("dec.harm_ws", harm_source_ws_doubles(B, T, upp, Hs), s);
    const float* ini = eps_src ? eps_src + (size_t)B * cf.src_noise_row(T) : nullptr;
    check(harm_source(f0, B, T, upp, (float)cf.sr, Hs, 0, eps_src, ini, sseed, c.W("dec.src.w"), lin_wb[1], ws,
                      har + HAR_PAD, har_ld, s),
          "harm_source");
  }
  return har;
}
}

bool dec_noise_prepare(Ctx& c, int B, int T, const float* f0, const float* eps_src, uint64_t seed, hipStream_t s) {
  const SynthCfg& cf = c.scfg;
  if (!cf.f0 || cf.vocoder == 2 || !f0) return false;
  const long long har_ld = (long long)T * cf.upp() + 2 * HAR_PAD;
  float* har = dec_source(c, B, T, f0, eps_src, seed, s);
  long long Ti = T;
  for (size_t i = 0; i < cf.ups.size(); ++i) {
    const int C = c.ups[i].cout;
    Ti *= cf.ups[i];
    const NoiseFrame f = noise_frame(cf, i);
    if (f.ntap * f.stride == 1) continue;
    const std::string nn = "dec.noise_convs." + std::to_string(i);
    float* nz = c.buf<float>("dec.nz" + std::to_string(i), (size_t)B * Ti * C, s);
    if (noise_row_kernel(f, B, Ti, C)) {
      check(noise_conv_add(har + HAR_PAD - f.npad, har_ld, f.stride, f.ntap, c.W(nn + ".wf"), c.W(nn + ".b"), nz, B,
                           (int)Ti, C, s, true),
            "noise_conv");
    } else {
      ConvArgs an = conv(har + HAR_PAD - f.npad, f.stride, (int)Ti + f.ntap - 1, f.stride, c.W(nn + ".wf"), C, f.ntap, 1,
                         0, c.W(nn + ".b"), nz, C, (int)Ti, B);
      an.x_bs = har_ld;
      an.lds_pad = 64 * 1024;
      run(c, an, s, 2.0 * B * (double)Ti * C * f.kern);
    }
  }
  return true;
}

void dec_forward(Ctx& c, int B, int T, const float* z_btc, const float* mask, const float* f0, const float* g,
                 const float* eps_src, uint64_t seed, float* out, hipStream_t s, int gen_lowp, bool noise_pre) {
  const SynthCfg& cf = c.scfg;
  if (cf.f0 && cf.vocoder == 2) {
    refinegan_forward(c, B, T, z_btc, mask, f0, g, eps_src, seed, out, s);
    return;
  }
  const int I = cf.I, C0 = cf.C0;
  const long long har_ld = (long long)T * cf.upp() + 2 * HAR_PAD;
  float* har = nullptr;
  if (cf.f0) {
    if (noise_pre) {
      har = c.buf<float>("dec.har", (size_t)(B * har_ld), s);
    } else {
      har = dec_source(c, B, T, f0, eps_src, seed, s);
    }
  }
  float* cv = c.buf<float>("dec.cvec", (size_t)B * C0, s);
  run(c, lin(g, cf.gin, B, cf.gin, c.W("dec.cond.w"), C0, c.W("dec.cond.b"), cv, C0), s);
  size_t maxe = (size_t)T * C0;
  {
    long long t = T;
    for (size_t i = 0; i < cf.ups.size(); ++i) {
      t *= cf.ups[i];
      maxe = std::max(maxe, (size_t)t * (C0 >> (i + 1)));
    }
  }
  float* xin = c.buf<float>("dec.x", (size_t)B * maxe, s);
  float* y = c.buf<float>("dec.y", (size_t)B * maxe, s);
  float* R = c.buf<float>("dec.r", (size_t)B * maxe, s);
  float* t1 = c.buf<float>("dec.t", (size_t)B * maxe, s);
  {
    ConvArgs a = conv(z_btc, I, T, I, c.W("dec.pre.w"), C0, 7, 1, 3, c.W("dec.pre.b"), xin, C0, T, B);
    a.pre_mask = mask;
    a.pre_mask_bs = T;
    a.res = cv;
    a.ldr = 0;
    a.res_bs = C0;
    a.res_mode = RES_ADD_PRE;
    run(c, a, s);
  }
  float* cur = xin;
  int curT = T, Cin = C0;
  const int nk = (int)cf.rb_k.size();
  for (size_t i = 0; i < cf.ups.size(); ++i) {
    const UpsLayer& L = c.ups[i];
    const int C = L.cout, u = L.u, Ti = curT * u;
    ConvArgs a = conv(cur, Cin, curT, Cin, L.w, u * C, L.taps, 1, L.pad, L.b, y, u * C, curT, B);
    a.w_static = 1;
    a.lowp = gen_lowp;
    a.pre_act = ACT_LRELU;
    a.pre_slope = 0.1f;
    NoiseFrame nf;
    int& stride = nf.stride;
    int& kern = nf.kern;
    int& npad = nf.npad;
    int& ntap = nf.ntap;
    std::string nn;
    bool nz_fused = false;
    if (cf.f0) {
      nf = noise_frame(cf, i);
      nn = "dec.noise_convs." + std::to_string(i);
      const int kk = ntap * stride;
      if (noise_pre && kk > 1) {
        a.res = c.buf<float>("dec.nz" + std::to_string(i), (size_t)B * Ti * C, s);
        a.ldr = u * C;
        a.res_bs = (long long)Ti * C;
        a.res_mode = RES_ADD_POST;
        nz_fused = true;
      } else if (kk == 1 && conv_routes_wsb16(c, a)) {
        a.nz_har = har + HAR_PAD - npad;
        a.nz_bs = har_ld;
        a.nz_stride = stride;
        a.nz_kk = ntap * stride;
        a.nz_u = u;
        a.nz_C = C;
        a.nz_w = c.W(nn + ".wf");
        a.nz_b = c.W(nn + ".b");
        nz_fused = true;
      }
    }
    run(c, a, s, 2.0 * B * curT * (double)Cin * C * L.k);
    if (cf.f0 && !nz_fused) {
      if (noise_row_kernel(nf, B, Ti, C)) {
        check(noise_conv_add(har + HAR_PAD - npad, har_ld, stride, ntap, c.W(nn + ".wf"), c.W(nn + ".b"), y, B, Ti,
                             C, s),
              "noise_conv_add");
      } else {
        ConvArgs an = conv(har + HAR_PAD - npad, stride, Ti + ntap - 1, stride, c.W(nn + ".wf"), C, ntap, 1, 0,
                           c.W(nn + ".b"), y, C, Ti, B);
        an.x_bs = har_ld;
        an.acc_mode = ACC_ADD;
        run(c, an, s, 2.0 * B * (double)Ti * C * kern);
      }
    }
    float* S = xin;
    float* T1 = t1;
    float* RR = R;
    for (int j = 0; j < nk; ++j) {
      const int k = cf.rb_k[j];
      const auto& dil = cf.rb_d[j];
      const std::string rb = "dec.resblocks." + std::to_string(i * nk + j);
      const float* r_in = y;
      bool fuse = C <= 32;
      for (int d : dil) fuse = fuse && rb_pair_fits(C, k, d);
      if (fuse) {
        for (size_t m = 0; m < dil.size(); ++m) {
          const std::string n1 = rb + ".convs1." + std::to_string(m);
          const std::string n2 = rb + ".convs2." + std::to_string(m);
          const bool last = (m + 1 == dil.size());
          float* dst = last ? S : (m % 2 == 0 ? RR : T1);
          RbPairArgs p;
          p.x = r_in;
          p.x_bs = (long long)Ti * C;
          p.wfmt = (gen_lowp || c.conv_math_default() == 3) ? RB_WF16 : RB_WBF16;
          p.w1s = c.rb_wsplit_for(c.W(n1 + ".w"), C, k, p.wfmt, s);
          p.b1 = c.W(n1 + ".b");
          p.w2s = c.rb_wsplit_for(c.W(n2 + ".w"), C, k, p.wfmt, s);
          p.b2 = c.W(n2 + ".b");
          p.C = C;
          p.k = k;
          p.d = dil[m];
          p.T = Ti;
          p.B = B;
          p.y = dst;
          p.y_bs = (long long)Ti * C;
          p.lowp = gen_lowp;
          if (last) {
            p.acc_mode = (j == 0) ? ACC_STORE : ((j + 1 == nk) ? ACC_ADD_DIV : ACC_ADD);
            p.acc_div = (float)nk;
          }
          launch_rb_pair(c, p, s);
          r_in = dst;
        }
        continue;
      }
      for (size_t m = 0; m < dil.size(); ++m) {
        const int d = dil[m];
        const std::string n1 = rb + ".convs1." + std::to_string(m);
        const std::string n2 = rb + ".convs2." + std::to_string(m);
        ConvArgs a1 = conv(r_in, C, Ti, C, c.W(n1 + ".w"), C, k, d, (k * d - d) / 2, c.W(n1 + ".b"), T1, C, Ti, B);
        a1.w_static = 1;
        a1.lowp = gen_lowp;
        a1.pre_act = ACT_LRELU;
        a1.pre_slope = 0.1f;
        a1.act = ACT_LRELU;
        a1.slope = 0.1f;
        const bool last = (m + 1 == dil.size());
        float* dst = last ? S : RR;
        ConvArgs a2 = conv(T1, C, Ti, C, c.W(n2 + ".w"), C, k, 1, (k - 1) / 2, c.W(n2 + ".b"), dst, C, Ti, B);
        a2.w_static = 1;
        a2.lowp = gen_lowp;
        run(c, a1, s);
        a2.res = r_in;
        a2.ldr = C;
        a2.res_bs = (long long)Ti * C;
        a2.res_mode = RES_ADD_POST;
        if (last) {
          a2.acc_mode = (j == 0) ? ACC_STORE : ((j + 1 == nk) ? ACC_ADD_DIV : ACC_ADD);
          a2.acc_div = (float)nk;
        }
        run(c, a2, s);
        r_in = RR;
      }
    }
    cur = S;
    curT = Ti;
    Cin = C;
  }
  check(conv_post_tanh(cur, B, curT, Cin, c.W("dec.post.w"), 7, 0.01f, out, s, c.host[0].at("__post_b__").v[0]),
        "conv_post");
}

void synth_forward(Ctx& c, int B, int T, const float* phone, const int32_t* lengths, const int32_t* pitch,
                   const float* pitchf, const int32_t* sid, const float* eps_z, const float* eps_src, uint64_t seed,
                   float* out, float* zp_out, float* z_out, hipStream_t s, int gen_lowp, int head, float* mp_out,
                   float* logsp_out) {
  const SynthCfg& cf = c.scfg;
  const int H = cf.H, I = cf.I, F = cf.F, E = cf.emb_dim, nh = cf.n_heads, dk = H / nh;
  const long long BT = (long long)B * T;
  float* mask = c.buf<float>("te.mask", BT, s);
  check(seq_mask(lengths, mask, B, T, s), "seq_mask");
  float* g = c.buf<float>("spk.g", (size_t)B * cf.gin, s);
  check(gather_rows(c.W("emb_g"), cf.gin, sid, g, B, cf.gin, s), "emb_g");
  float* pe = nullptr;
  if (cf.f0) {
    pe = c.buf<float>("te.pe", BT * H, s);
    check(gather_rows(c.W("te.emb_pitch"), H, pitch, pe, (int)BT, H, s), "emb_pitch");
  }
  float* x = c.buf<float>("te.x", BT * H, s);
  {
    ConvArgs a = lin(phone, E, (int)BT, E, c.W("te.emb_phone.w"), H, c.W("te.emb_phone.b"), x, H);
    a.res = pe;
    a.ldr = H;
    a.res_mode = pe ? RES_ADD_PRE : RES_NONE;
    a.alpha = (float)std::sqrt((double)H);
    a.act = ACT_LRELU;
    a.slope = 0.1f;
    a.mask = mask;
    run(c, a, s);
  }
  float* qkv = c.buf<float>("te.qkv", BT * 3 * H, s);
  const int nsplit = flash_attn_splits(B, nh, T);
  float* part_o = c.buf<float>("te.fa_o", (size_t)flash_attn_ws_floats(B, nh, T, dk, nsplit), s);
  float* part_ml = c.buf<float>("te.fa_ml", (size_t)nsplit * B * nh * T * 2, s);
  float* att = c.buf<float>("te.att", BT * H, s);
  float* h1 = c.buf<float>("te.h1", BT * F, s);
  const float qscale = (float)(1.0 / std::sqrt((double)dk));
  for (int i = 0; i < cf.n_layers; ++i) {
    const std::string q = "te." + std::to_string(i);
    run(c, lin(x, H, (int)BT, H, c.W(q + ".qkv.w"), 3 * H, c.W(q + ".qkv.b"), qkv, 3 * H), s);
    check(flash_attn(qkv, 3 * H, B, T, nh, dk, qscale, c.W(q + ".rel_k"), c.W(q + ".rel_v"), cf.window,
                     c.synth_full_lengths ? nullptr : mask, part_o, part_ml, nsplit, att, H, s),
          "flash_attn");
    {
      ConvArgs a = lin(att, H, (int)BT, H, c.W(q + ".o.w"), H, c.W(q + ".o.b"), x, H);
      a.res = x;
      a.ldr = H;
      a.ln_g = c.W(q + ".ln1.g");
      a.ln_b = c.W(q + ".ln1.b");
      run(c, a, s);
    }
    {
      ConvArgs a = conv(x, H, T, H, c.W(q + ".ffn1.w"), F, cf.ksize, 1, (cf.ksize - 1) / 2, c.W(q + ".ffn1.b"), h1,
                        F, T, B);
      a.pre_mask = mask;
      a.pre_mask_bs = T;
      a.act = ACT_RELU;
      run(c, a, s);
      ConvArgs b = conv(h1, F, T, F, c.W(q + ".ffn2.w"), H, cf.ksize, 1, (cf.ksize - 1) / 2, c.W(q + ".ffn2.b"), x,
                        H, T, B);
      b.pre_mask = mask;
      b.pre_mask_bs = T;
      b.mask = mask;
      b.mask_bs = T;
      b.res = x;
      b.ldr = H;
      b.res_bs = (long long)T * H;
      b.ln_g = c.W(q + ".ln2.g");
      b.ln_b = c.W(q + ".ln2.b");
      run(c, b, s);
    }
  }
  float* stats = c.buf<float>("te.stats", BT * 2 * I, s);
  {
    ConvArgs a = lin(x, H, (int)BT, H, c.W("te.proj.w"), 2 * I, c.W("te.proj.b"), stats, 2 * I);
    a.pre_mask = mask;
    a.mask = mask;
    run(c, a, s);
  }
  if (mp_out)
    RVCX_HIP(hipMemcpy2DAsync(mp_out, (size_t)I * 4, stats, (size_t)2 * I * 4, (size_t)I * 4, (size_t)BT,
                              hipMemcpyDeviceToDevice, s));
  if (logsp_out)
    RVCX_HIP(hipMemcpy2DAsync(logsp_out, (size_t)I * 4, stats + I, (size_t)2 * I * 4, (size_t)I * 4, (size_t)BT,
                              hipMemcpyDeviceToDevice, s));
  float* z = c.buf<float>("flow.z", BT * I, s);
  float* xf = c.buf<float>("flow.xf", BT * I, s);
  check(zp_sample(stats, B, T, I, eps_z, splitmix(seed ^ 0x5a505f4e4f495345ull), mask, z, s), "zp_sample");
  const int Tf = T - head;
  const long long BTf = (long long)B * Tf;
  const float* maskf = mask;
  const float* pitchff = pitchf;
  if (head > 0) {
    if (head >= T) throw Error(RVCX_E_SHAPE, "synthesizer: rate leaves no frames");
    float* z2 = c.buf<float>("flow.z_rate", (size_t)BTf * I, s);
    RVCX_HIP(hipMemcpy2DAsync(z2, (size_t)Tf * I * 4, z + (size_t)head * I, (size_t)T * I * 4, (size_t)Tf * I * 4,
                              (size_t)B, hipMemcpyDeviceToDevice, s));
    float* m2 = c.buf<float>("te.mask_rate", (size_t)BTf, s);
    RVCX_HIP(hipMemcpy2DAsync(m2, (size_t)Tf * 4, mask + head, (size_t)T * 4, (size_t)Tf * 4, (size_t)B,
                              hipMemcpyDeviceToDevice, s));
    if (pitchf) {
      float* p2 = c.buf<float>("dec.pitchf_rate", (size_t)BTf, s);
      RVCX_HIP(hipMemcpy2DAsync(p2, (size_t)Tf * 4, pitchf + head, (size_t)T * 4, (size_t)Tf * 4, (size_t)B,
                                hipMemcpyDeviceToDevice, s));
      pitchff = p2;
    }
    z = z2;
    maskf = m2;
  }
  if (zp_out) RVCX_HIP(hipMemcpyAsync(zp_out, z, BTf * I * sizeof(float), hipMemcpyDeviceToDevice, s));
  hipStream_t nax = s;
  bool noise_pre = false;
  if (cf.f0 && cf.vocoder != 2 && pitchff) {
    nax = fork_aux(c, s);
    noise_pre = dec_noise_prepare(c, B, Tf, pitchff, eps_src, seed, nax);
  }
  float* hs = c.buf<float>("flow.hs", BTf * 2 * H, s);
  float* acts = c.buf<float>("flow.acts", BTf * H, s);
  const int cl = 2 * H * cf.flow_layers;
  float* gc = c.buf<float>("flow.gc", (size_t)B * cf.flow_n * cl, s);
  run(c, lin(g, cf.gin, B, cf.gin, c.W("flow.cond.w"), cf.flow_n * cl, c.W("flow.cond.b"), gc, cf.flow_n * cl), s);
  const bool fold = cf.flow_n % 2 == 0;
  for (int f = cf.flow_n - 1; f >= 0; --f) {
    const std::string q = "flow." + std::to_string(f);
    float* x0 = xf;
    float* x1 = xf + I / 2;
    if (fold) {
      const bool rev = (cf.flow_n - 1 - f) % 2 == 0;
      x0 = rev ? z + I / 2 : z;
      x1 = rev ? z : z + I / 2;
    } else {
      check(channel_flip(z, xf, (int)BTf, I, s), "flip");
    }
    {
      ConvArgs a = lin(x0, I, (int)BTf, I / 2, c.W(q + ".pre.w"), 2 * H, c.W(q + ".pre.b"), hs, 2 * H);
      a.mask = maskf;
      run(c, a, s);
    }
    for (int L = 0; L < cf.flow_layers; ++L) {
      const std::string l = std::to_string(L);
      {
        ConvArgs a = conv(hs, 2 * H, Tf, H, c.W(q + ".in" + l + ".w"), 2 * H, cf.flow_k, 1, (cf.flow_k - 1) / 2,
                          c.W(q + ".in" + l + ".b"), acts, H, Tf, B);
        a.x_bs = (long long)Tf * 2 * H;
        a.gate_h = H;
        a.gate_g = gc + (size_t)f * cl + (size_t)L * 2 * H;
        a.gate_g_bs = (long long)cf.flow_n * cl;
        run(c, a, s);
      }
      const float* wrs = c.W(q + ".rs" + l + ".w");
      const float* brs = c.W(q + ".rs" + l + ".b");
      const bool last = L == cf.flow_layers - 1;
      ConvArgs a = lin(acts, H, (int)BTf, H, wrs, last ? H : 2 * H, brs, last ? hs + H : hs, 2 * H);
      a.acc_mode = ACC_ADD;
      a.mask = maskf;
      run(c, a, s);
    }
    {
      ConvArgs a = lin(hs + H, 2 * H, (int)BTf, H, c.W(q + ".post.w"), I / 2, c.W(q + ".post.b"), x1, I);
      a.res = x1;
      a.ldr = I;
      a.res_mode = RES_RSUB_POST;
      a.mask = maskf;
      run(c, a, s);
    }
    if (!fold) std::swap(z, xf);
  }
  if (z_out) RVCX_HIP(hipMemcpyAsync(z_out, z, BTf * I * sizeof(float), hipMemcpyDeviceToDevice, s));
  join_aux(c, s, nax);
  dec_forward(c, B, Tf, z, maskf, pitchff, g, eps_src, seed, out, s, gen_lowp, noise_pre);
}

}
```

### retrieval-based-voice-conversion-mlx_amd/csrc/rvcx_kernels.h

```cpp
#pragma once
#include <hip/hip_runtime.h>
#include <cstdint>

namespace rvcx {

const char* rvcx_knob(const char* name);

enum Act : int {
  ACT_NONE = 0,
  ACT_LRELU = 1,
  ACT_RELU = 2,
  ACT_GELU = 3,
  ACT_TANH = 4,
  ACT_SIGMOID = 5,
  ACT_LOGCLAMP = 6,
};

enum ResMode : int {
  RES_NONE = 0,
  RES_ADD_PRE = 1,
  RES_ADD_POST = 2,
  RES_RSUB_POST = 3,
};

enum AccMode : int {
  ACC_STORE = 0,
  ACC_ADD = 1,
  ACC_ADD_DIV = 2,
};

enum OutMap : int {
  OUT_ROWS = 0,
  OUT_UPSAMPLE2D = 1,
};

enum WsplitFmt : int { WSPLIT_BF16 = 0, WSPLIT_H16 = 1, WSPLIT_S2D = 2 };

struct ConvArgs {
  const float* x = nullptr;
  long long x_bs = 0;
  int ldx = 0;
  int T_in = 0;
  int W_in = 0;
  int C_in = 0;
  int pre_act = ACT_NONE;
  float pre_slope = 0.f;
  const float* pre_mask = nullptr;
  long long pre_mask_bs = 0;
  const float* w = nullptr;
  long long w_bs = 0;
  long long w_ts = 0;
  int ldw = 0;
  int b_kn = 0;
  int taps = 1;
  int stride = 1, dil = 1, pad = 0;
  int KH = 1, KW = 1, padh = 0, padw = 0;
  float* y = nullptr;
  long long y_bs = 0;
  int ldy = 0;
  int T_out = 0;
  int W_out = 0;
  int N = 0;
  int out_map = OUT_ROWS;
  int out_cv = 0;
  const float* bias = nullptr;
  long long bias_bs = 0;
  float alpha = 1.f;
  int act = ACT_NONE;
  float slope = 0.f;
  const float* res = nullptr;
  long long res_bs = 0;
  int ldr = 0;
  int res_mode = RES_NONE;
  const float* mask = nullptr;
  long long mask_bs = 0;
  int acc_mode = ACC_STORE;
  float acc_div = 1.f;
  int gate_h = 0;
  const float* gate_g = nullptr;
  long long gate_g_bs = 0;
  const float* ln_g = nullptr;
  const float* ln_b = nullptr;
  float ln_eps = 1e-5f;
  int batch = 1;
  int batch_inner = 1;
  long long x_bs2 = 0, w_bs2 = 0, y_bs2 = 0, res_bs2 = 0, bias_bs2 = 0;
  int force_cfg = -1;
  int pipe = 0;
  int astage = 0;
  int math = 0;
  int w_static = 0;
  const void* wsplit = nullptr;
  int wsplit_npad = 0;
  int wsb = 0;
  int wsplit_fmt = 0;
  int ksplit = 1;
  int no_splitk = 0;
  int lowp = 0;
  long long ws_rows = 0;
  float* ws = nullptr;
  const float* nz_har = nullptr;
  long long nz_bs = 0;
  int nz_stride = 0, nz_kk = 0, nz_u = 1, nz_C = 0;
  const float* nz_w = nullptr;
  const float* nz_b = nullptr;
  int lds_pad = 0;
};

hipError_t conv1d(const ConvArgs& a, hipStream_t s);
enum ConvKind : int { CK_WSB16 = 0, CK_WSB, CK_GS, CK_GSW, CK_RBPAIR, CK_SMALL2D, CK_EMU, CK_GEMM, CK_TINY, CK_WST,
                      CK_OTHER, CK_COUNT };
int conv_last_kind();
const char* conv_kind_name(int k);
int conv_math_of(const ConvArgs& a);
int conv_unstreamed_kind(const ConvArgs& a);
hipError_t conv2d(const ConvArgs& a, hipStream_t s);
bool conv2d_small_fits(const ConvArgs& a);
hipError_t conv2d_small(const ConvArgs& a, hipStream_t s);
long long small2d_wsplit_bytes(const ConvArgs& a);
hipError_t small2d_wsplit_build(const ConvArgs& a, void* out, hipStream_t s);
long long conv_plan_splitk(ConvArgs& a, bool two_d);

hipError_t fill(float* p, float v, long long n, hipStream_t s);
hipError_t transpose_bct_btc(const float* x, float* y, int B, int C, int T, hipStream_t s);
hipError_t transpose_btc_bct(const float* x, float* y, int B, int T, int C, int ldx, hipStream_t s);
hipError_t channel_flip(const float* x, float* y, int rows, int C, hipStream_t s);
hipError_t gather_rows(const float* table, int ld_table, const int32_t* idx, float* y, int rows, int C,
                       hipStream_t s);
hipError_t seq_mask(const int32_t* lengths, float* mask, int B, int T, hipStream_t s);
hipError_t upconv_phase_pack(const float* w, int C, int co, float* out, hipStream_t s);
hipError_t layernorm_rows(const float* x, const float* r, float* y, const float* gamma, const float* beta,
                          int rows, int D, float eps, const float* mask, hipStream_t s);
hipError_t gate_tanh_sigmoid(const float* xin, int ldx, const float* g, long long g_bs, float* acts, int B,
                             int T, int H, hipStream_t s);
bool conv_wsb_eligible(const ConvArgs& a, bool two_d = false);
bool conv_wsb_wants(const ConvArgs& a);
int conv_wsb_route(const ConvArgs& a, bool two_d);
bool conv_wsb_tile(int cfg, int& BM, int& BN);
int conv_wsb_pick(const ConvArgs& a);
bool conv_gs_eligible(const ConvArgs& a, bool two_d);
bool conv_gsw_eligible(const ConvArgs& a);
bool conv_gs_tile(int cfg, int& BM, int& BN);
hipError_t conv_gs_launch(const ConvArgs& a, int cfg, hipStream_t s, bool two_d, int ksplit);
int conv_wsplit_npad(int N);
long long conv_wsplit_bytes(const ConvArgs& a);
hipError_t conv_wsplit_build(const ConvArgs& a, void* out, hipStream_t s);
hipError_t conv_wsb_launch(const ConvArgs& a, int cfg, hipStream_t s, bool two_d = false,
                           int ksplit = 1);
bool conv_wst_fits(const ConvArgs& a, bool two_d);
hipError_t conv_wst_launch(const ConvArgs& a, hipStream_t s);
struct RbPairArgs {
  const float* x = nullptr;
  long long x_bs = 0;
  const void* w1s = nullptr;
  const float* b1 = nullptr;
  const void* w2s = nullptr;
  const float* b2 = nullptr;
  int C = 0, k = 0, d = 1, T = 0, B = 1;
  float* y = nullptr;
  long long y_bs = 0;
  int acc_mode = ACC_STORE;
  float acc_div = 1.f;
  int wfmt = 0;
  int lowp = 0;
};
enum RbWfmt : int { RB_WBF16 = 0, RB_WF16 = 1 };
bool rb_pair_fits(int C, int k, int d);
long long rb_wsplit_bytes(int C, int k, int wfmt = RB_WBF16);
hipError_t rb_wsplit_build(const float* w, int C, int k, void* out, hipStream_t s, int wfmt = RB_WBF16);
hipError_t rb_pair(const RbPairArgs& a, int cfg, hipStream_t s);
int flash_attn_splits(int B, int nh, int T);
long long flash_attn_ws_floats(int B, int nh, int T, int dk, int nsplit);
hipError_t flash_attn(const float* qkv, int ldq, int B, int T, int nh, int dk, float qscale, const float* rel_k,
                      const float* rel_v, int window, const float* mask, float* part_o, float* part_ml, int nsplit,
                      float* out, int ldo, hipStream_t s);
hipError_t crepe_frames(const float* audio, long long n, long long f_first, int nf, float* out, int ld, hipStream_t s,
                        int torch_sem = 0);
hipError_t crepe_relu_bn_pool(const float* x, long long rows_in, int C, const float* bn, float* y, hipStream_t s);
hipError_t crepe_decode(const float* probs, int F, double lo_cents, double hi_cents, float thr, float* f0_raw,
                        float* per_raw, float* f0, double* f0d, float* per, hipStream_t s);
constexpr int CREPE_RVC_BATCH = 512;
hipError_t crepe_decode_viterbi(const float* probs, int F, int minidx, int maxidx, const float* dither, float thr,
                                float* lp, int* ptr, int* bins, float* f0_raw, float* per_raw, float* f0, double* f0d,
                                float* per, hipStream_t s, int seg = CREPE_RVC_BATCH);
constexpr int PERFORMER_SLAB = 128, PERFORMER_MAX_FEATURES = 512;
int performer_slabs(int T);
long long performer_ws_floats(int H, int T, int M, int B = 1);
hipError_t performer_attention(const float* q, const float* k, const float* v, long long hs, int ld, int H, int T,
                               const float* P, int M, float* ws, float* out, long long out_hs, int out_ld,
                               hipStream_t s, int B = 1, long long bs = 0, long long out_bs = 0);
hipError_t fcpe_magnitude(const float* spec, int F, int nbins, float* mag, int ldm, hipStream_t s);
constexpr int FCPE_GN_CHUNKS = 64;
hipError_t groupnorm_lrelu(float* x, int T, int C, int G, const float* gamma, const float* beta, float eps, float slope,
                           double* ws, hipStream_t s, int B = 1);
hipError_t glu_dwconv_swish(const float* x, int T, int C2, const float* w, const float* b, int K, int pad, float* y,
                            hipStream_t s, int B = 1);
hipError_t fcpe_zero_pad(const float* x, int n, int pad_l, long long ldx, float* y, long long ldy, int B,
                         hipStream_t s);
hipError_t fcpe_dup_last_frame(float* mel, int B, int F, int C, hipStream_t s);
hipError_t fcpe_decode(const float* sal, int F, int nb, const float* cent, float thr, int mode, double* f0,
                       hipStream_t s);
hipError_t fcpe_post_process(const double* f0, int F, int n, int hop, int sr, int* links, double* out, hipStream_t s);
hipError_t noise_conv_add(const float* har, long long har_bs, int stride, int taps, const float* wf, const float* nb,
                          float* y, int B, int T, int C, hipStream_t s, bool store = false);
hipError_t upsample2_protect(const float* feats, const float* feats0, int L, int D, float* out, int T, const float* pitchf,
                             float protect,
                             hipStream_t s);
hipError_t sine_source(const float* f0, int B, int L, int upp, float sr, const float* eps, uint64_t seed,
                       float lin_w, float lin_b, double* cum_ws, float* har, long long har_ld, hipStream_t s);
hipError_t conv_post_tanh(const float* x, int B, int T, int C, const float* w, int K, float slope, float* y,
                          hipStream_t s, float bias = 0.f);
size_t harm_source_ws_doubles(int B, int L, int upp, int H);
hipError_t resample_dw(const float* x, int B, int T_in, int C, const float* ker, int K, int orig, int width, float* y,
                       int T_out, hipStream_t s);
hipError_t lerp_up_cat(const float* x, int B, int T, int C, int ldx, int rate, float slope, const float* skip, int Cd,
                       float* y, int ldy, hipStream_t s);
hipError_t adain(const float* x, int B, int T, int C, const float* w, const float* eps, uint64_t seed, float slope,
                 float* y, int mode, float div, hipStream_t s);
hipError_t harm_source(const float* f0, int B, int L, int upp, float sr, int H, int linear_up, const float* eps,
                       const float* ini, uint64_t seed, const float* lin_w, float lin_b, double* ws, float* har,
                       long long har_ld, hipStream_t st);
hipError_t randn(float* y, long long n, uint64_t seed, uint64_t offset, hipStream_t s);
hipError_t zp_sample(const float* stats, int B, int T, int I, const float* eps, uint64_t seed, const float* mask,
                     float* zp, hipStream_t s);
constexpr int GN_CHUNKS = 256;
inline size_t groupnorm_ws_doubles(int C, int B = 1) { return (size_t)B * (GN_CHUNKS * C * 2 + C); }
hipError_t groupnorm_time_gelu(float* x, int T, int C, const float* gamma, const float* beta, float eps,
                               double* ws, hipStream_t s, int B = 1);
hipError_t hubert_conv0_gn_gelu(const float* x, long long ldx, const float* w10, int T, int C, const float* gamma,
                                const float* beta, float eps, double* ws, float* y, hipStream_t s, int B = 1);
hipError_t act_inplace(float* x, long long n, int act, float slope, hipStream_t s);
hipError_t reflect_pad_1d(const float* x, int n, int pad_l, int pad_r, float* y, hipStream_t s, int B = 1,
                          long long ldx = 0, long long ldy = 0);
hipError_t reflect_pad_rows(const float* x, int rows, int C, int pad_r, float* y, hipStream_t s, int B = 1);
hipError_t stft_magnitude(const float* spec, int F, int nbins, float* mag, int ldm, hipStream_t s);
hipError_t affine_inplace(float* x, long long n, float a, float b, hipStream_t s);
hipError_t avgpool2(const float* x, int H, int W, int C, int ldx, float* y, hipStream_t s);
hipError_t nhwc_to_hcw(const float* x, int H, int W, int C, float* y, hipStream_t s);
hipError_t gru_bidir(const float* gi, const float* whh_f, const float* bhh_f, const float* whh_b,
                     const float* bhh_b, int T, float* out, unsigned long long* xchg, unsigned* status,
                     unsigned* next_tag, hipStream_t s, int B = 1);
inline size_t gru_xchg_words(int B) { return (size_t)B * 4 * 2 * 128; }
hipError_t rmvpe_decode(const float* sal, int F, int ncls, float thred, double* f0, hipStream_t s, int B = 1,
                        int Fs = 0);
hipError_t f0_post(const double* f0, int F, double shift, int32_t* coarse, float* pitchf, double* f0_out,
                   hipStream_t s);

constexpr int IIR_MAXO = 8;
hipError_t filtfilt_pad(const double* x, long long n, const double* b, const double* a, const double* zi,
                        const double* FL, int order, long long t_pad, double* ws, double* pad64, float* pad32,
                        hipStream_t s);
size_t filtfilt_ws_doubles(long long n, int order);
hipError_t peak_normalize(const float* src, float* dst, long long n, float* ws, hipStream_t s, int B = 1,
                          long long lds = 0, long long ldd = 0);
size_t peak_normalize_ws_floats(int B);
hipError_t f0_autotune(double* f0, int F, double strength, int skip_unvoiced, hipStream_t s);
hipError_t f0_autotune_rows(double* f0, int F, const double* strength, const int* on, int B, hipStream_t s);
hipError_t split_points(const double* x, long long n, int window, long long t_center, long long t_query,
                        double* sum_ws, long long* ts, int nts, hipStream_t s);
int rms_frame_count(long long n, int sr);
hipError_t rms_frames_f64(const double* x, long long n, int frame, int hop, double* rms, int nframes, hipStream_t s);
hipError_t change_rms(const double* src, long long n_src, int sr_src, float* y, long long n_y, int sr_y, float rate,
                      float* ws, hipStream_t s);

struct IvfView {
  int d = 0, nprobe = 1;
  long long nlist = 0, ntotal = 0;
  const float* cent = nullptr;
  const float* vecs = nullptr;
  const long long* off = nullptr;
  const long long* ids = nullptr;
  const int* slot_of_id = nullptr;
};
constexpr int IVF_MAX_K = 16;
size_t ivf_ws_floats(long long n, long long nlist, int nprobe);
hipError_t ivf_search(const IvfView& v, const float* x, long long n, int k, float* dist_out, long long* ids_out,
                      float rate, float one_minus_rate, float* out, float* ws, hipStream_t s);
struct IvfRows {
  const int* seqs = nullptr;
  const float* rate = nullptr;
  const float* one_minus_rate = nullptr;
  int L = 0, off = 0;
};
hipError_t ivf_retrieve_rows(const IvfView& v, const float* x, const IvfRows& rows, int n_seq, float* out, float* ws,
                             hipStream_t s);

hipError_t rt_resample(const float* x, long long ldx, int n_in, const float* ker, int K, int width, int orig, int nw,
                       float* y, long long ldy, int n_out, const float* pre, const int* slot2row, int B,
                       hipStream_t s);
hipError_t rt_ingest(const float* in16, int n16, const float* abuf_old, float* abuf_new, int na, const float* cbuf_old,
                     float* cbuf_new, int nc, double sensitivity, float* vol, float* volsq, int* gate,
                     const int* slot2row, float* cbuf_rows, int B, hipStream_t s);
hipError_t rt_pitch(const double* f0, int F, const double* factor, const int* pold, int* pnew, const float* fold,
                    float* fnew, int nbuf, const int* slot2row, int B, hipStream_t s);
// ... 31 lines not shown
```

### retrieval-based-voice-conversion-mlx_amd/rvcx/_lib.py

```python
from __future__ import annotations

import ctypes
import os
from typing import Optional

_HERE = os.path.dirname(os.path.abspath(__file__))
LIB_PATH = os.environ.get("RVCX_LIB", os.path.join(_HERE, "librvcx.so"))

RVCX_MODEL_SYNTH, RVCX_MODEL_HUBERT, RVCX_MODEL_RMVPE, RVCX_MODEL_CREPE, RVCX_MODEL_FCPE = 0, 1, 2, 3, 4

STATUS = {
    0: "RVCX_OK", -1: "RVCX_E_INVALID", -2: "RVCX_E_SHAPE", -3: "RVCX_E_HIP", -4: "RVCX_E_OOM",
    -5: "RVCX_E_STATE", -6: "RVCX_E_CAPACITY",
}

EXPORTS = [
    "rvcx_create", "rvcx_destroy", "rvcx_set_generator_precision", "rvcx_config_info", "rvcx_profile_read_kinds",
    "rvcx_profile_kind_name", "rvcx_synth_infer_ex", "rvcx_last_error", "rvcx_set_synth_config", "rvcx_upload", "rvcx_finalize",
    "rvcx_hubert", "rvcx_rmvpe", "rvcx_f0_post", "rvcx_synth_infer", "rvcx_dec_only", "rvcx_voice_conversion",
    "rvcx_synth_upp", "rvcx_set_highpass", "rvcx_pipeline", "rvcx_pipeline_default_opts", "rvcx_pipeline_ex",
    "rvcx_f0_autotune", "rvcx_rmvpe_decode", "rvcx_profile", "rvcx_profile_read", "rvcx_profile_read_ex", "rvcx_index_load",
    "rvcx_index_unload", "rvcx_index_info", "rvcx_index_set_nprobe", "rvcx_index_search", "rvcx_index_reconstruct_n",
    "rvcx_index_retrieve", "rvcx_rt_default_desc", "rvcx_rt_default_opts", "rvcx_rt_create", "rvcx_rt_destroy",
    "rvcx_rt_geometry", "rvcx_rt_reset", "rvcx_rt_process", "rvcx_rt_process_v", "rvcx_rt_reset_stream", "rvcx_hubert_batch", "rvcx_rmvpe_batch",
    "rvcx_pipeline_batch", "rvcx_set_highpass_sos", "rvcx_highpass_pad", "rvcx_device_status", "rvcx_index_parse",
    "rvcx_set_conv_math", "rvcx_conv1d", "rvcx_conv1d_gen", "rvcx_conv1d_ex", "rvcx_conv2d3x3", "rvcx_convtranspose2d_s2", "rvcx_flash_attention", "rvcx_resblock_pair", "rvcx_crepe", "rvcx_split_audio",
    "rvcx_workspace_bytes", "rvcx_set_workspace", "rvcx_workspace_info", "rvcx_crepe_ex",
    "rvcx_crepe_decode", "rvcx_set_fcpe_config", "rvcx_fcpe", "rvcx_fcpe_decode", "rvcx_fcpe_b",
]
TEST_EXPORTS = ["rvcx_performer_attention", "rvcx_performer_attention_b", "rvcx_fcpe_mel"]


class RvcxLibraryError(ImportError):
    pass


class RvcxError(RuntimeError):
    def __init__(self, code: int, msg: str):
        super().__init__(f"{STATUS.get(code, code)}: {msg}")
        self.code = code


class SynthDesc(ctypes.Structure):
    _fields_ = [
        ("inter_channels", ctypes.c_int), ("hidden_channels", ctypes.c_int), ("filter_channels", ctypes.c_int),
        ("n_heads", ctypes.c_int), ("n_layers", ctypes.c_int), ("kernel_size", ctypes.c_int),
        ("n_resblocks", ctypes.c_int), ("resblock_kernel_sizes", ctypes.c_int * 4),
        ("resblock_dilation_sizes", (ctypes.c_int * 4) * 4), ("n_dilations", ctypes.c_int),
        ("n_upsample", ctypes.c_int), ("upsample_rates", ctypes.c_int * 8),
        ("upsample_initial_channel", ctypes.c_int), ("upsample_kernel_sizes", ctypes.c_int * 8),
        ("spk_embed_dim", ctypes.c_int), ("gin_channels", ctypes.c_int), ("sr", ctypes.c_int),
        ("text_enc_hidden_dim", ctypes.c_int), ("no_f0", ctypes.c_int), ("vocoder", ctypes.c_int),
    ]


VOCODERS = {"HiFi-GAN": 0, "MRF HiFi-GAN": 1, "RefineGAN": 2}


class PipelineOpts(ctypes.Structure):
    _fields_ = [
        ("sid", ctypes.c_int), ("version", ctypes.c_int), ("pitch", ctypes.c_double), ("protect", ctypes.c_float),
        ("rmvpe_threshold", ctypes.c_float), ("t_pad", ctypes.c_int64), ("t_pad_tgt", ctypes.c_int64),
        ("t_query", ctypes.c_int64), ("t_center", ctypes.c_int64), ("t_max", ctypes.c_int64),
        ("f0_autotune", ctypes.c_int), ("f0_autotune_strength", ctypes.c_double), ("proposed_pitch", ctypes.c_int),
        ("proposed_pitch_threshold", ctypes.c_double), ("volume_envelope", ctypes.c_double),
        ("mlx_semantics", ctypes.c_int), ("index_rate", ctypes.c_double), ("f0_method", ctypes.c_int),
        ("fcpe_threshold", ctypes.c_float),
    ]


class FcpeDesc(ctypes.Structure):
    _fields_ = [("sampling_rate", ctypes.c_int), ("n_fft", ctypes.c_int), ("win_size", ctypes.c_int),
                ("hop_size", ctypes.c_int), ("num_mels", ctypes.c_int), ("fmin", ctypes.c_float),
                ("fmax", ctypes.c_float), ("n_layers", ctypes.c_int), ("n_chans", ctypes.c_int),
                ("out_dims", ctypes.c_int)]


class RtDesc(ctypes.Structure):
    _fields_ = [("n_streams", ctypes.c_int), ("read_chunk_size", ctypes.c_int),
                ("cross_fade_overlap_size", ctypes.c_double), ("extra_convert_size", ctypes.c_double),
                ("silent_threshold", ctypes.c_double), ("f0_method", ctypes.c_int),
                ("fcpe_threshold", ctypes.c_float)]


class RtOpts(ctypes.Structure):
    _fields_ = [("f0_up_key", ctypes.c_double), ("index_rate", ctypes.c_double), ("protect", ctypes.c_float),
                ("volume_envelope", ctypes.c_double), ("f0_autotune", ctypes.c_int),
                ("f0_autotune_strength", ctypes.c_double), ("proposed_pitch", ctypes.c_int),
                ("proposed_pitch_threshold", ctypes.c_double), ("gen_precision", ctypes.c_int)]


class ConvTestDesc(ctypes.Structure):
    _fields_ = [
        ("x", ctypes.c_void_p), ("w", ctypes.c_void_p), ("bias", ctypes.c_void_p), ("res", ctypes.c_void_p),
        ("mask", ctypes.c_void_p), ("pre_mask", ctypes.c_void_p), ("y", ctypes.c_void_p),
        ("T_in", ctypes.c_int), ("C_in", ctypes.c_int), ("N", ctypes.c_int), ("taps", ctypes.c_int),
        ("dil", ctypes.c_int), ("pad", ctypes.c_int), ("stride", ctypes.c_int), ("T_out", ctypes.c_int),
        ("ldx", ctypes.c_int), ("ldy", ctypes.c_int), ("ldr", ctypes.c_int),
        ("batch", ctypes.c_int),
        ("x_bs", ctypes.c_int64), ("y_bs", ctypes.c_int64), ("res_bs", ctypes.c_int64), ("mask_bs", ctypes.c_int64),
        ("pre_mask_bs", ctypes.c_int64),
        ("batch_inner", ctypes.c_int),
        ("x_bs2", ctypes.c_int64), ("w_bs2", ctypes.c_int64), ("y_bs2", ctypes.c_int64), ("res_bs2", ctypes.c_int64),
        ("bias_bs2", ctypes.c_int64),
        ("pre_act", ctypes.c_int), ("pre_slope", ctypes.c_float),
        ("act", ctypes.c_int), ("slope", ctypes.c_float), ("alpha", ctypes.c_float),
        ("res_mode", ctypes.c_int), ("acc_mode", ctypes.c_int), ("acc_div", ctypes.c_float),
        ("gate_h", ctypes.c_int), ("gate_g", ctypes.c_void_p), ("gate_g_bs", ctypes.c_int64),
        ("ln_g", ctypes.c_void_p), ("ln_b", ctypes.c_void_p), ("ln_eps", ctypes.c_float),
        ("nz_har", ctypes.c_void_p), ("nz_bs", ctypes.c_int64),
        ("nz_stride", ctypes.c_int), ("nz_kk", ctypes.c_int), ("nz_u", ctypes.c_int), ("nz_C", ctypes.c_int),
        ("nz_w", ctypes.c_void_p), ("nz_b", ctypes.c_void_p),
        ("route", ctypes.c_int), ("no_splitk", ctypes.c_int),
    ]


_lib: Optional[ctypes.CDLL] = None


def load(path: Optional[str] = None) -> ctypes.CDLL:
    global _lib
    if _lib is not None and path is None:
        return _lib
    p = path or LIB_PATH
    if not os.path.exists(p):
        raise RvcxLibraryError(f"librvcx.so not found at {p}; build it with __graft_entry__.build() "
                               "(make -C retrieval-based-voice-conversion-mlx_amd/csrc)")
    try:
        lib = ctypes.CDLL(p)
    except OSError as e:
        raise RvcxLibraryError(f"cannot load {p}: {e}") from e
    vp, i64, i32, f32, f64, u64 = (ctypes.c_void_p, ctypes.c_int64, ctypes.c_int, ctypes.c_float, ctypes.c_double,
                                   ctypes.c_uint64)
    P = ctypes.POINTER
    sig = {
        "rvcx_create": (i32, [P(vp), i32]),
        "rvcx_destroy": (i32, [vp]),
        "rvcx_last_error": (ctypes.c_char_p, [vp]),
        "rvcx_set_synth_config": (i32, [vp, P(SynthDesc)]),
        "rvcx_upload": (i32, [vp, i32, ctypes.c_char_p, vp, P(i64), i32]),
        "rvcx_finalize": (i32, [vp, i32]),
        "rvcx_hubert": (i32, [vp, vp, i64, i32, vp, i64, P(i64), vp]),
        "rvcx_rmvpe": (i32, [vp, vp, i64, f32, vp, i64, P(i64), vp, vp]),
        "rvcx_f0_post": (i32, [vp, vp, i64, f64, vp, vp, vp, vp]),
        "rvcx_synth_infer": (i32, [vp, i32, i32, vp, vp, vp, vp, vp, vp, vp, u64, vp, vp, vp, vp]),
        "rvcx_synth_infer_ex": (i32, [vp, i32, i32, vp, vp, vp, vp, vp, f64, vp, vp, u64, vp, vp, vp, vp, vp, P(i32),
                                      vp]),
        "rvcx_dec_only": (i32, [vp, i32, i32, vp, vp, vp, vp, u64, vp, vp]),
        "rvcx_voice_conversion": (i32, [vp, vp, i64, vp, vp, i32, f32, f64, vp, vp, u64, vp, i64, P(i64), vp]),
        "rvcx_synth_upp": (i32, [vp]),
        "rvcx_set_highpass": (i32, [vp, vp, vp, vp, i32]),
        "rvcx_profile": (i32, [vp, i32]),
        "rvcx_profile_read": (i32, [vp, P(f64), P(f64), P(i64)]),
        "rvcx_profile_read_ex": (i32, [vp, P(f64), P(f64), P(i64), P(f64)]),
        "rvcx_pipeline": (i32, [vp, vp, i64, i32, f64, f32, i64, i64, vp, vp, u64, vp, i64, P(i64), vp, vp]),
        "rvcx_pipeline_default_opts": (i32, [P(PipelineOpts)]),
        "rvcx_pipeline_ex": (i32, [vp, vp, i64, P(PipelineOpts), vp, vp, u64, vp, i64, P(i64), vp, vp]),
        "rvcx_f0_autotune": (i32, [vp, vp, i64, f64, i32, vp]),
        "rvcx_rmvpe_decode": (i32, [vp, vp, i64, f32, vp, vp]),
        "rvcx_crepe": (i32, [vp, vp, i64, f32, f32, f32, vp, vp, vp, i64, P(i64), vp]),
        "rvcx_crepe_ex": (i32, [vp, vp, i64, f32, f32, f32, i32, vp, vp, vp, vp, i64, P(i64), vp]),
        "rvcx_crepe_decode": (i32, [vp, vp, i64, f32, f32, f32, i32, vp, vp, vp, vp]),
        "rvcx_set_fcpe_config": (i32, [vp, P(FcpeDesc)]),
        "rvcx_fcpe": (i32, [vp, vp, i64, f32, i32, i32, i64, vp, vp, i64, P(i64), vp]),
        "rvcx_fcpe_decode": (i32, [vp, vp, i64, f32, i32, i32, i64, vp, vp]),
        "rvcx_fcpe_b": (i32, [vp, vp, i64, i64, i32, f32, i32, vp, vp, vp]),
        "rvcx_fcpe_mel": (i32, [vp, vp, i64, vp, i64, P(i64), vp]),
        "rvcx_performer_attention": (i32, [vp, vp, vp, vp, i32, i32, vp, i32, vp, vp]),
        "rvcx_performer_attention_b": (i32, [vp, vp, vp, vp, i32, i32, i32, vp, i32, vp, vp]),
        "rvcx_split_audio": (i32, [vp, vp, i64, i32, f64, i32, P(i64), i64, P(i64), vp]),
        "rvcx_index_load": (i32, [vp, vp, i64]),
        "rvcx_index_unload": (i32, [vp]),
        "rvcx_index_info": (i32, [vp, P(i64), P(i64), P(i64), P(i64)]),
        "rvcx_index_set_nprobe": (i32, [vp, i64]),
        "rvcx_index_search": (i32, [vp, vp, i64, i32, vp, vp, vp]),
        "rvcx_index_reconstruct_n": (i32, [vp, i64, i64, vp, vp]),
        "rvcx_index_retrieve": (i32, [vp, vp, i64, i32, f64, vp, vp]),
        "rvcx_pipeline_batch": (i32, [vp, vp, i64, i64, i32, P(PipelineOpts), P(ctypes.c_int32), vp, vp, u64, vp, i64,
                                      P(i64), vp, vp, vp]),
        "rvcx_set_highpass_sos": (i32, [vp, vp, i32]),
        "rvcx_workspace_bytes": (i32, [vp, i32, i64, P(PipelineOpts), P(i64), vp]),
        "rvcx_set_workspace": (i32, [vp, vp, i64]),
        "rvcx_workspace_info": (i32, [vp, P(i64), P(i64), P(i64)]),
        "rvcx_highpass_pad": (i32, [vp, vp, i64, i64, vp, vp, vp]),
        "rvcx_hubert_batch": (i32, [vp, vp, i64, i64, i32, i32, vp, i64, P(i64), vp]),
        "rvcx_rmvpe_batch": (i32, [vp, vp, i64, i64, i32, f32, vp, i64, P(i64), vp, vp]),
        "rvcx_rt_default_desc": (i32, [P(RtDesc)]),
        "rvcx_rt_default_opts": (i32, [P(RtOpts)]),
        "rvcx_rt_create": (i32, [vp, P(RtDesc), P(vp)]),
        "rvcx_rt_destroy": (i32, [vp, vp]),
        "rvcx_rt_geometry": (i32, [vp, P(i64)]),
        "rvcx_rt_reset": (i32, [vp, vp, vp]),
        "rvcx_rt_process": (i32, [vp, vp, vp, P(ctypes.c_int32), P(RtOpts), vp, vp, u64, vp, vp, vp, vp]),
        "rvcx_rt_process_v": (i32, [vp, vp, vp, P(ctypes.c_int32), P(RtOpts), P(ctypes.c_uint8), vp, vp, u64, vp, vp,
                                    vp, vp]),
        "rvcx_rt_reset_stream": (i32, [vp, vp, i32, vp]),
        "rvcx_device_status": (i32, [vp, vp]),
        "rvcx_index_parse": (i32, [vp, i64, P(i64), P(i64), P(i64), P(i64), ctypes.c_char_p, i64]),
        "rvcx_set_conv_math": (i32, [vp, i32]),
        "rvcx_set_generator_precision": (i32, [vp, i32]),
        "rvcx_config_info": (i32, [vp, vp, i64, P(i64)]),
        "rvcx_profile_read_kinds": (i32, [vp, P(f64), P(f64), P(i64), P(f64), i32, P(f64), P(f64), P(f64), P(f64),
                                          P(i64)]),
        "rvcx_profile_kind_name": (ctypes.c_char_p, [i32]),
        "rvcx_conv1d": (i32, [vp, vp, i64, i32, vp, vp, i32, i32, i32, i32, i32, i32, vp, i64, vp]),
        "rvcx_conv1d_gen": (i32, [vp, vp, i64, i32, vp, vp, i32, i32, i32, i32, i32, f32, i32, f32, vp, i32, f32, i32,
                                  vp, vp]),
        "rvcx_conv1d_ex": (i32, [vp, P(ConvTestDesc), P(i32), P(i32), vp]),
        "rvcx_conv2d3x3": (i32, [vp, vp, i32, i32, i32, vp, vp, i32, i32, i32, vp, vp]),
        "rvcx_convtranspose2d_s2": (i32, [vp, vp, i32, i32, i32, vp, vp, i32, i32, i32, vp, vp]),
        "rvcx_flash_attention": (i32, [vp, vp, i32, i32, i32, i32, ctypes.c_float, vp, vp, i32, vp, vp, vp]),
        "rvcx_resblock_pair": (i32, [vp, vp, i32, i64, i32, vp, vp, vp, vp, i32, i32, i32, f32, i32, vp, vp]),
    }
    for name, (res, args) in sig.items():
        if not hasattr(lib, name):
            continue
        fn = getattr(lib, name)
        fn.restype = res
        fn.argtypes = args
    if path is None:
        _lib = lib
    return lib


def exported_symbols(path: Optional[str] = None):
    lib = load(path)
    return [n for n in EXPORTS + TEST_EXPORTS if hasattr(lib, n)]


def index_parse(data: bytes) -> dict:
    lib = load()
    buf = ctypes.create_string_buffer(bytes(data), len(data))
    v = [ctypes.c_int64(0) for _ in range(4)]
    err = ctypes.create_string_buffer(512)
    rc = lib.rvcx_index_parse(buf, len(data), *[ctypes.byref(x) for x in v], err, 512)
    if rc != 0:
        raise RvcxError(rc, err.value.decode(errors="replace"))
    return dict(zip(("d", "ntotal", "nlist", "nprobe"), (x.value for x in v)))
```

### retrieval-based-voice-conversion-mlx_amd/rvcx/engine.py

```python
from __future__ import annotations

import ctypes
from typing import Dict, Mapping, Optional

import numpy as np

from . import _lib
from .config import SYNTH_48K_V2, SynthConfig
from .weights import normalize_state


def _ptr(t) -> Optional[int]:
    return None if t is None else t.data_ptr()


class Engine:

    def __init__(self, device: int = 0):
        import torch

        self.lib = _lib.load()
        if not torch.cuda.is_available():
            raise RuntimeError("rvcx needs a ROCm GPU: torch.cuda.is_available() is False")
        self.torch = torch
        self.device_index = int(device)
        self.device = torch.device(f"cuda:{self.device_index}")
        ctx = ctypes.c_void_p()
        rc = self.lib.rvcx_create(ctypes.byref(ctx), self.device_index)
        if rc != 0:
            raise _lib.RvcxError(rc, f"rvcx_create(device={device}) failed")
        self.ctx = ctx
        self.synth_cfg: Optional[SynthConfig] = None
        self.loaded = {"synth": False, "hubert": False, "rmvpe": False, "crepe": None, "fcpe": None}
        self.fcpe_cfg = None

    def close(self):
        if getattr(self, "ctx", None):
            self.lib.rvcx_destroy(self.ctx)
            self.ctx = None

    def __del__(self):
        try:
            self.close()
        except Exception:
            pass

    def _check(self, rc: int, what: str):
        if rc != 0:
            msg = self.lib.rvcx_last_error(self.ctx)
            raise _lib.RvcxError(rc, f"{what}: {msg.decode() if msg else ''}")

    def check_device_status(self):
        self._check(self.lib.rvcx_device_status(self.ctx, self.stream()), "device status")

    def host(self, t):
        self.check_device_status()
        return t.cpu().numpy()

    def stream(self) -> int:
        return self.torch.cuda.current_stream(self.device).cuda_stream

    def _dev(self, x, dtype):
        t = self.torch
        if isinstance(x, t.Tensor):
            return x.to(device=self.device, dtype=dtype).contiguous()
        return t.as_tensor(np.ascontiguousarray(x), dtype=dtype, device=self.device).contiguous()

    def set_synth_config(self, cfg: SynthConfig = SYNTH_48K_V2):
        d = _lib.SynthDesc()
        d.inter_channels, d.hidden_channels, d.filter_channels = cfg.inter_channels, cfg.hidden_channels, \
            cfg.filter_channels
        d.n_heads, d.n_layers, d.kernel_size = cfg.n_heads, cfg.n_layers, cfg.kernel_size
        d.n_resblocks = len(cfg.resblock_kernel_sizes)
        d.n_dilations = len(cfg.resblock_dilation_sizes[0])
        for j, k in enumerate(cfg.resblock_kernel_sizes):
            d.resblock_kernel_sizes[j] = k
            for m, dd in enumerate(cfg.resblock_dilation_sizes[j]):
                d.resblock_dilation_sizes[j][m] = dd
        d.n_upsample = len(cfg.upsample_rates)
        for i, (u, k) in enumerate(zip(cfg.upsample_rates, cfg.upsample_kernel_sizes)):
            d.upsample_rates[i] = u
            d.upsample_kernel_sizes[i] = k
        d.upsample_initial_channel = cfg.upsample_initial_channel
        d.spk_embed_dim, d.gin_channels, d.sr = cfg.spk_embed_dim, cfg.gin_channels, cfg.sr
        d.text_enc_hidden_dim = cfg.text_enc_hidden_dim
        d.no_f0 = 0 if cfg.use_f0 else 1
        if cfg.vocoder not in _lib.VOCODERS:
            raise ValueError(f"unknown vocoder {cfg.vocoder!r}; expected one of {sorted(_lib.VOCODERS)}")
        d.vocoder = _lib.VOCODERS[cfg.vocoder]
        self._check(self.lib.rvcx_set_synth_config(self.ctx, ctypes.byref(d)), "set_synth_config")
        self.synth_cfg = cfg

    def upload_state(self, model: int, state: Mapping[str, np.ndarray]):
        for name, arr in state.items():
            a = np.ascontiguousarray(arr, dtype=np.float32)
            shape = (ctypes.c_int64 * max(1, a.ndim))(*a.shape)
            self._check(self.lib.rvcx_upload(self.ctx, model, name.encode(), a.ctypes.data, shape, a.ndim),
                        f"upload {name}")
        self._check(self.lib.rvcx_finalize(self.ctx, model), "finalize")

    def load_synth(self, state: Mapping[str, np.ndarray], cfg: SynthConfig = SYNTH_48K_V2):
        self.set_synth_config(cfg)
        st = {k: v for k, v in normalize_state(state).items() if not k.startswith("enc_q.")}
        self.upload_state(_lib.RVCX_MODEL_SYNTH, st)
        self.loaded["synth"] = True

    def load_hubert(self, state: Mapping[str, np.ndarray]):
        st = {k: v for k, v in normalize_state(state).items() if k != "masked_spec_embed"}
        self.upload_state(_lib.RVCX_MODEL_HUBERT, st)
        self.loaded["hubert"] = True

    def load_rmvpe(self, state: Mapping[str, np.ndarray]):
        self.upload_state(_lib.RVCX_MODEL_RMVPE, normalize_state(state))
        self.loaded["rmvpe"] = True

    def load_crepe(self, state: Mapping[str, np.ndarray], key=None):
        self.upload_state(_lib.RVCX_MODEL_CREPE, {k: v for k, v in state.items() if not k.endswith("num_batches_tracked")})
        self.loaded["crepe"] = key if key is not None else ("full" if np.shape(state["conv1.weight"])[0] == 1024
                                                           else "tiny")

    def crepe(self, audio, f0_min: float = 50.0, f0_max: float = 1100.0, threshold: float = 0.1,
              want_periodicity: bool = False, want_probs: bool = False, semantics: str = "mlx", dither=None):
        t = self.torch
        a = self._dev(audio, t.float32).reshape(-1)
        n = a.numel()
        F = 1 + n // 160
        f0 = t.empty((F,), dtype=t.float32, device=self.device)
        per = t.empty((F,), dtype=t.float32, device=self.device) if want_periodicity else None
        probs = t.empty((F, 360), dtype=t.float32, device=self.device) if want_probs else None
        fo = ctypes.c_int64(0)
        sem = {"mlx": 0, "rvc": 1}[semantics]
        d = None if dither is None else self._dev(dither, t.float32).reshape(-1)
        if d is not None and d.numel() != F:
            raise ValueError(f"dither needs {F} values")
        self._check(self.lib.rvcx_crepe_ex(self.ctx, a.data_ptr(), n, float(f0_min), float(f0_max), float(threshold),
                                           sem, _ptr(d), f0.data_ptr(), _ptr(per), _ptr(probs), F, ctypes.byref(fo),
                                           self.stream()), "crepe")
        out = [f0]
        if want_periodicity:
            out.append(per)
        if want_probs:
            out.append(probs)
        return out[0] if len(out) == 1 else tuple(out)

    def crepe_decode(self, probs, f0_min: float = 50.0, f0_max: float = 1100.0, threshold: float = 0.1,
                     semantics: str = "rvc", dither=None):
        t = self.torch
        p = self._dev(probs, t.float32).contiguous()
        F = int(p.shape[0])
        f0 = t.empty((F,), dtype=t.float32, device=self.device)
        per = t.empty((F,), dtype=t.float32, device=self.device)
        d = None if dither is None else self._dev(dither, t.float32).reshape(-1)
        self._check(self.lib.rvcx_crepe_decode(self.ctx, p.data_ptr(), F, float(f0_min), float(f0_max),
                                               float(threshold), {"mlx": 0, "rvc": 1}[semantics], _ptr(d),
                                               f0.data_ptr(), per.data_ptr(), self.stream()), "crepe_decode")
        return f0, per

    def load_fcpe(self, state: Mapping[str, np.ndarray], config: Mapping, key=None):
        from .weights import check_fcpe_state, fcpe_sizes

        st = check_fcpe_state(state, config)
        z = fcpe_sizes(config)
        d = _lib.FcpeDesc()
        d.sampling_rate, d.n_fft, d.win_size, d.hop_size, d.num_mels = z["sampling_rate"], z["n_fft"], z["win_size"], \
            z["hop_size"], z["num_mels"]
        d.fmin, d.fmax = float(z["fmin"]), float(z["fmax"])
        d.n_layers, d.n_chans, d.out_dims = z["n_layers"], z["n_chans"], z["out_dims"]
        self._check(self.lib.rvcx_set_fcpe_config(self.ctx, ctypes.byref(d)), "set_fcpe_config")
        self.upload_state(_lib.RVCX_MODEL_FCPE, st)
        self.fcpe_cfg = z
        self.loaded["fcpe"] = key if key is not None else True

    _FCPE_DECODERS = {"local_argmax": 0, "argmax": 1}

# ... 617 lines not shown
```

Measured before the change: 1092 audio-sec/sec.

## Run decoder only over the output window needed after padding trim

Adds a decoder window so the HiFi-GAN/NSF generator computes only the frames that survive the t_pad trim, plus a receptive-field margin, instead of the full padded length. The upsample, resblock, noise and post convs run on a sub-range with offsets into full-length buffers, and plan_T keeps tile and split-k planning consistent with the full length. This removes decoder work on padding samples that are discarded anyway. The risk is boundary mismatches if the margin does not cover the receptive field. It is enabled by default.

```diff
diff --git a/retrieval-based-voice-conversion-mlx_amd/csrc/aux_kernels.hip b/retrieval-based-voice-conversion-mlx_amd/csrc/aux_kernels.hip
--- a/retrieval-based-voice-conversion-mlx_amd/csrc/aux_kernels.hip
+++ b/retrieval-based-voice-conversion-mlx_amd/csrc/aux_kernels.hip
@@ -412,7 +412,7 @@
 constexpr int CP_T = 256, CP_IT = 24;
 __global__ __launch_bounds__(CP_T) void k_conv_post(const float* __restrict__ x, int T, int C,
                                                     const float* __restrict__ wg, int K, float slope,
-                                                    float* __restrict__ y, float bias) {
+                                                    float* __restrict__ y, float bias, long long y_bs) {
   extern __shared__ float tile[];
   const int b = blockIdx.y;
   const int t0 = blockIdx.x * CP_T;
@@ -450,12 +450,12 @@
   float acc = 0.f;
   for (int c = 0; c < C; ++c)
     for (int k = 0; k < K; ++k) acc = fmaf(tile[(threadIdx.x + k) * ldt + c], w[c * K + k], acc);
-  y[(long long)b * T + t] = tanhf(acc + bias);
+  y[(long long)b * y_bs + t] = tanhf(acc + bias);
 }
 constexpr int CPF_C = 32, CPF_K = 7, CPF_LD = 36, CPF_ROWS = CP_T + CPF_K - 1;
 __global__ __launch_bounds__(CP_T) void k_conv_post32(const float* __restrict__ x, int T,
                                                       const float* __restrict__ wg, float slope,
-                                                      float* __restrict__ y, float bias) {
+                                                      float* __restrict__ y, float bias, long long y_bs) {
   __shared__ __attribute__((aligned(16))) float tile[CPF_ROWS * CPF_LD];
   __shared__ __attribute__((aligned(16))) float w[CPF_K * CPF_C];
   const int b = blockIdx.y;
@@ -502,20 +502,23 @@
 #pragma unroll
       for (int e = 0; e < 4; ++e) acc[e] = fmaf(xv[e], wv[e], acc[e]);
     }
-  y[(long long)b * T + t] = tanhf(((acc[0] + acc[1]) + (acc[2] + acc[3])) + bias);
+  y[(long long)b * y_bs + t] = tanhf(((acc[0] + acc[1]) + (acc[2] + acc[3])) + bias);
 }
 
 hipError_t conv_post_tanh(const float* x, int B, int T, int C, const float* w, int K, float slope, float* y,
-                          hipStream_t s, float bias) {
+                          hipStream_t s, float bias, long long y_bs) {
+  if (y_bs <= 0) y_bs = T;
   if (C == CPF_C && K == CPF_K && (reinterpret_cast<uintptr_t>(x) & 15) == 0) {
-    hipLaunchKernelGGL(k_conv_post32, dim3((T + CP_T - 1) / CP_T, B), dim3(CP_T), 0, s, x, T, w, slope, y, bias);
+    hipLaunchKernelGGL(k_conv_post32, dim3((T + CP_T - 1) / CP_T, B), dim3(CP_T), 0, s, x, T, w, slope, y, bias,
+                       y_bs);
     return hipGetLastError();
   }
   if (C % 4 != 0 || (long long)(CP_T + K - 1) * (C / 4) > (long long)CP_IT * CP_T ||
       (reinterpret_cast<uintptr_t>(x) & 15) != 0)
     return hipErrorInvalidValue;
   const size_t smem = ((size_t)(CP_T + K - 1) * (C + 1) + (size_t)C * K) * sizeof(float);
-  hipLaunchKernelGGL(k_conv_post, dim3((T + CP_T - 1) / CP_T, B), dim3(CP_T), smem, s, x, T, C, w, K, slope, y, bias);
+  hipLaunchKernelGGL(k_conv_post, dim3((T + CP_T - 1) / CP_T, B), dim3(CP_T), smem, s, x, T, C, w, K, slope, y, bias,
+                     y_bs);
   return hipGetLastError();
 }
 
diff --git a/retrieval-based-voice-conversion-mlx_amd/csrc/capi.cpp b/retrieval-based-voice-conversion-mlx_amd/csrc/capi.cpp
--- a/retrieval-based-voice-conversion-mlx_amd/csrc/capi.cpp
+++ b/retrieval-based-voice-conversion-mlx_amd/csrc/capi.cpp
@@ -266,6 +266,41 @@
 }
 }
 
+namespace {
+SynthCfg synth_cfg_of(const rvcx_synth_desc* d) {
+  if (!d) throw Error(RVCX_E_INVALID, "null desc");
+  SynthCfg g;
+  g.I = d->inter_channels;
+  g.H = d->hidden_channels;
+  g.F = d->filter_channels;
+  g.n_heads = d->n_heads;
+  g.n_layers = d->n_layers;
+  g.ksize = d->kernel_size;
+  if (d->n_resblocks < 1 || d->n_resblocks > 4 || d->n_dilations < 1 || d->n_dilations > 4)
+    throw Error(RVCX_E_INVALID, "resblock config out of range");
+  g.rb_k.assign(d->resblock_kernel_sizes, d->resblock_kernel_sizes + d->n_resblocks);
+  g.rb_d.clear();
+  for (int j = 0; j < d->n_resblocks; ++j)
+    g.rb_d.emplace_back(d->resblock_dilation_sizes[j], d->resblock_dilation_sizes[j] + d->n_dilations);
+  if (d->n_upsample < 1 || d->n_upsample > 8) throw Error(RVCX_E_INVALID, "n_upsample out of range");
+  g.ups.assign(d->upsample_rates, d->upsample_rates + d->n_upsample);
+  g.up_k.assign(d->upsample_kernel_sizes, d->upsample_kernel_sizes + d->n_upsample);
+  g.C0 = d->upsample_initial_channel;
+  g.n_spk = d->spk_embed_dim;
+  g.gin = d->gin_channels;
+  g.sr = d->sr;
+  g.emb_dim = d->text_enc_hidden_dim;
+  g.f0 = d->no_f0 == 0;
+  g.vocoder = d->vocoder;
+  if (g.vocoder < 0 || g.vocoder > 2) throw Error(RVCX_E_INVALID, "unsupported vocoder id");
+  if (!g.f0 && g.vocoder != 0)
+    throw Error(RVCX_E_INVALID, "models without pitch guidance use the HiFi-GAN decoder only (synthesizers.py:119-139)");
+  if (g.H % g.n_heads || g.I % 2 || g.C0 % (1 << g.ups.size()))
+    throw Error(RVCX_E_INVALID, "inconsistent synthesizer dimensions");
+  return g;
+}
+}
+
 extern "C" {
 
 int rvcx_create(rvcx_ctx** out, int device) {
@@ -275,6 +310,7 @@
   if (hipGetDeviceCount(&n) != hipSuccess || device < 0 || device >= n) return RVCX_E_HIP;
   auto* c = new rvcx_ctx();
   c->device = device;
+  if (const char* e = rvcx_knob("RVCX_DEC_WINDOW")) c->dec_window = std::atoi(e) != 0;
   *out = c;
   return RVCX_OK;
 }
@@ -291,36 +327,7 @@
 
 int rvcx_set_synth_config(rvcx_ctx* ctx, const rvcx_synth_desc* d) {
   return guard(ctx, [&] {
-    if (!d) throw Error(RVCX_E_INVALID, "null desc");
-    SynthCfg g;
-    g.I = d->inter_channels;
-    g.H = d->hidden_channels;
-    g.F = d->filter_channels;
-    g.n_heads = d->n_heads;
-    g.n_layers = d->n_layers;
-    g.ksize = d->kernel_size;
-    if (d->n_resblocks < 1 || d->n_resblocks > 4 || d->n_dilations < 1 || d->n_dilations > 4)
-      throw Error(RVCX_E_INVALID, "resblock config out of range");
-    g.rb_k.assign(d->resblock_kernel_sizes, d->resblock_kernel_sizes + d->n_resblocks);
-    g.rb_d.clear();
-    for (int j = 0; j < d->n_resblocks; ++j)
-      g.rb_d.emplace_back(d->resblock_dilation_sizes[j], d->resblock_dilation_sizes[j] + d->n_dilations);
-    if (d->n_upsample < 1 || d->n_upsample > 8) throw Error(RVCX_E_INVALID, "n_upsample out of range");
-    g.ups.assign(d->upsample_rates, d->upsample_rates + d->n_upsample);
-    g.up_k.assign(d->upsample_kernel_sizes, d->upsample_kernel_sizes + d->n_upsample);
-    g.C0 = d->upsample_initial_channel;
-    g.n_spk = d->spk_embed_dim;
-    g.gin = d->gin_channels;
-    g.sr = d->sr;
-    g.emb_dim = d->text_enc_hidden_dim;
-    g.f0 = d->no_f0 == 0;
-    g.vocoder = d->vocoder;
-    if (g.vocoder < 0 || g.vocoder > 2) throw Error(RVCX_E_INVALID, "unsupported vocoder id");
-    if (!g.f0 && g.vocoder != 0)
-      throw Error(RVCX_E_INVALID, "models without pitch guidance use the HiFi-GAN decoder only (synthesizers.py:119-139)");
-    if (g.H % g.n_heads || g.I % 2 || g.C0 % (1 << g.ups.size()))
-      throw Error(RVCX_E_INVALID, "inconsistent synthesizer dimensions");
-    ctx->scfg = g;
+    ctx->scfg = synth_cfg_of(d);
     ctx->synth_cfg_set = true;
     ctx->ready[0] = false;
   });
@@ -868,6 +875,7 @@
   j += ", \"conv_math_default\": \"" + std::string(cm ? cm : "h16") + "\"";
   j += ", \"experimental\": " + std::string(experimental_on() ? "true" : "false");
   if (ctx) j += ", \"arena_bytes\": " + std::to_string(ctx->arena_bytes);
+  if (ctx) j += ", \"dec_window\": " + std::string(ctx->dec_window ? "true" : "false");
   j += ", \"env\": {";
   bool first = true;
   for (char** e = environ; e && *e; ++e) {
@@ -891,6 +899,22 @@
     buf[n] = 0;
   }
   return (int64_t)j.size() < cap || !buf ? RVCX_OK : RVCX_E_CAPACITY;
+}
+
+int rvcx_set_dec_window(rvcx_ctx* ctx, int on) {
+  return guard(ctx, [&] { ctx->dec_window = on != 0; });
+}
+
+int rvcx_dec_margin_frames(const rvcx_synth_desc* d, int* frames) {
+  try {
+    if (!frames) return RVCX_E_INVALID;
+    *frames = dec_margin_frames(synth_cfg_of(d));
+    return RVCX_OK;
+  } catch (const Error& e) {
+    return e.code;
+  } catch (...) {
+    return RVCX_E_INVALID;
+  }
 }
 
 int rvcx_set_generator_precision(rvcx_ctx* ctx, int) {
diff --git a/retrieval-based-voice-conversion-mlx_amd/csrc/conv_dispatch.hip b/retrieval-based-voice-conversion-mlx_amd/csrc/conv_dispatch.hip
--- a/retrieval-based-voice-conversion-mlx_amd/csrc/conv_dispatch.hip
+++ b/retrieval-based-voice-conversion-mlx_amd/csrc/conv_dispatch.hip
@@ -49,11 +49,13 @@
   BN = t[cfg][1];
 }
 
+inline int plan_rows(const ConvArgs& a) { return (a.plan_T > 0 && a.W_out <= 0) ? a.plan_T : a.T_out; }
+
 inline int pick_wsb(const ConvArgs& a) {
   static const int c_long = env_cfg("RVCX_WCFG_LONG", 0);
   if (a.wsb == 2) return 30;
   if (a.N <= 32) return 24;
-  if (a.taps <= 3 && a.N >= 1024 && a.T_out >= 8192 && a.C_in < 512 && c_long == 0) return 25;
+  if (a.taps <= 3 && a.N >= 1024 && plan_rows(a) >= 8192 && a.C_in < 512 && c_long == 0) return 25;
   if (a.taps <= 3) return 27;
   if (c_long > 0) return c_long;
   return (a.C_in < 256 && a.N >= 128) ? 25 : 23;
@@ -160,17 +162,20 @@
   } else {
     cfg_tile(two_d ? pick_cfg<true>(a) : pick_cfg<false>(a), BM, BN);
   }
-  long long mtiles;
+  const int T_plan = two_d ? a.T_out : plan_rows(a);
+  long long mtiles, mtiles_real;
   if (!two_d) {
-    mtiles = (a.T_out + BM - 1) / BM;
+    mtiles = (T_plan + BM - 1) / BM;
+    mtiles_real = (a.T_out + BM - 1) / BM;
   } else {
     const int rw = a.W_out < BM ? a.W_out : BM;
     const int rh = BM / rw;
-    mtiles = (long long)((a.T_out + rh - 1) / rh) * ((a.W_out + rw - 1) / rw);
+    mtiles = mtiles_real = (long long)((a.T_out + rh - 1) / rh) * ((a.W_out + rw - 1) / rw);
   }
   const long long tiles = mtiles * ((a.N + BN - 1) / BN) * a.batch * a.batch_inner;
+  const long long tiles_real = mtiles_real * ((a.N + BN - 1) / BN) * a.batch * a.batch_inner;
   const int iters = ((a.C_in + CK - 1) / CK) * a.taps;
-  const double M = two_d ? (double)a.T_out * a.W_out : (double)a.T_out;
+  const double M = two_d ? (double)a.T_out * a.W_out : (double)T_plan;
   const double flops = 2.0 * M * a.N * (double)a.C_in * a.taps * a.batch * a.batch_inner;
   static const int target = env_cfg("RVCX_SPLITK_TARGET", 512);
   constexpr int min_tiles = 192;
@@ -187,14 +192,14 @@
   if (ks < 2) return 0;
   a.ksplit = ks;
   a.ws_rows = two_d ? (long long)a.T_out * a.W_out : a.T_out;
-  return std::max((long long)ks * a.ws_rows * a.N * a.batch * a.batch_inner, tiles * ks * BM * BN);
+  return std::max((long long)ks * a.ws_rows * a.N * a.batch * a.batch_inner, tiles_real * ks * BM * BN);
 }
 
 bool conv_wsb_wants(const ConvArgs& a) {
   if (conv_math(a) < 2 || !conv_wsb_eligible(a)) return false;
   constexpr int min_taps = 2, min_tiles = 512, min_n = 64;
   if (a.N < min_n || a.taps < min_taps) return false;
-  const long long tiles = (long long)((a.T_out + 127) / 128) * ((a.N + 63) / 64) * a.batch;
+  const long long tiles = (long long)((plan_rows(a) + 127) / 128) * ((a.N + 63) / 64) * a.batch;
   return tiles >= min_tiles;
 }
 
diff --git a/retrieval-based-voice-conversion-mlx_amd/csrc/runtime.h b/retrieval-based-voice-conversion-mlx_amd/csrc/runtime.h
--- a/retrieval-based-voice-conversion-mlx_amd/csrc/runtime.h
+++ b/retrieval-based-voice-conversion-mlx_amd/csrc/runtime.h
@@ -129,6 +129,8 @@
   std::map<std::pair<const void*, int>, std::unique_ptr<DevBuf>> rb_wsplit_cache;
   const void* rb_wsplit_for(const float* w, int C, int k, int wfmt, hipStream_t s);
   bool synth_full_lengths = false;
+  bool dec_window = true;
+  bool use_dec_window() const { return dec_window && !sizing_plan; }
   bool aux_front = false;
   hipStream_t aux = nullptr;
   hipEvent_t ev_fork = nullptr, ev_join = nullptr, ev_gate = nullptr;
@@ -277,13 +279,18 @@
                          int64_t cap, hipStream_t s);
 int64_t rmvpe_forward_b(Ctx& c, const float* audio, int64_t n, int64_t lda, int B, float thred, double* f0,
                         int64_t cap, float* hidden, hipStream_t s);
+struct DecWindow {
+  long long s0 = 0, s1 = -1;
+};
+int dec_margin_frames(const SynthCfg& cf);
+void dec_window_frames(const SynthCfg& cf, int T, const DecWindow& win, int& fa, int& fb);
 void synth_forward(Ctx& c, int B, int T, const float* phone, const int32_t* lengths, const int32_t* pitch,
                    const float* pitchf, const int32_t* sid, const float* eps_z, const float* eps_src, uint64_t seed,
                    float* out, float* zp_out, float* z_out, hipStream_t s, int gen_lowp = 0, int head = 0,
-                   float* mp_out = nullptr, float* logsp_out = nullptr);
+                   float* mp_out = nullptr, float* logsp_out = nullptr, const DecWindow& win = DecWindow());
 void dec_forward(Ctx& c, int B, int T, const float* z_btc, const float* mask, const float* f0, const float* g,
                  const float* eps_src, uint64_t seed, float* out, hipStream_t s, int gen_lowp = 0,
-                 bool noise_pre = false);
+                 bool noise_pre = false, const DecWindow& win = DecWindow());
 bool dec_noise_prepare(Ctx& c, int B, int T, const float* f0, const float* eps_src, uint64_t seed, hipStream_t s);
 
 void set_highpass(Ctx& c, const double* b, const double* a, const double* zi, int order);
@@ -293,7 +300,7 @@
 int64_t vc_forward(Ctx& c, const float* audio, int64_t n, const int32_t* pitch, const float* pitchf,
                    int64_t pitch_len, int sid, float protect, double index_rate, const float* eps_z,
                    const float* eps_src, uint64_t seed, float* out, int64_t cap, hipStream_t s,
-                   const float* feats_pre = nullptr, int64_t L_pre = 0);
+                   const float* feats_pre = nullptr, int64_t L_pre = 0, int64_t trim = 0);
 struct RtState;
 RtState* rt_create(Ctx& c, const rvcx_rt_desc& d);
 void rt_destroy(RtState* s);
diff --git a/retrieval-based-voice-conversion-mlx_amd/csrc/runtime_pipeline.cpp b/retrieval-based-voice-conversion-mlx_amd/csrc/runtime_pipeline.cpp
--- a/retrieval-based-voice-conversion-mlx_amd/csrc/runtime_pipeline.cpp
+++ b/retrieval-based-voice-conversion-mlx_amd/csrc/runtime_pipeline.cpp
@@ -140,7 +140,7 @@
 int64_t vc_forward(Ctx& c, const float* audio, int64_t n, const int32_t* pitch, const float* pitchf,
                    int64_t pitch_len, int sid, float protect, double index_rate, const float* eps_z,
                    const float* eps_src, uint64_t seed, float* out, int64_t cap, hipStream_t s,
-                   const float* feats_pre, int64_t L_pre) {
+                   const float* feats_pre, int64_t L_pre, int64_t trim) {
   if (sid < 0 || sid >= c.scfg.n_spk) throw Error(RVCX_E_INVALID, "sid out of range");
   const int E = c.scfg.emb_dim;
   const float* feats = feats_pre;
@@ -173,7 +173,10 @@
   set_i32_once(c, "vc.len.sid", lens + 1, sid, s);
   {
     ScopedFullLengths full(c);
-    synth_forward(c, 1, T, phone, lens, pitch, pitchf, lens + 1, eps_z, eps_src, seed, out, nullptr, nullptr, s);
+    DecWindow win;
+    if (trim > 0 && c.use_dec_window()) win = {trim, (long long)T * upp - trim};
+    synth_forward(c, 1, T, phone, lens, pitch, pitchf, lens + 1, eps_z, eps_src, seed, out, nullptr, nullptr, s, 0, 0,
+                  nullptr, nullptr, win);
   }
   return (int64_t)T * upp;
 }
@@ -408,7 +411,8 @@
     const int64_t nvc = vc_forward(c, pad32 + ch.a0, len, pitch ? pitch + ch.f_lo : nullptr,
                                    pitchf ? pitchf + ch.f_lo : nullptr, ch.f_hi - ch.f_lo, o.sid,
                                    o.protect, o.index_rate, eps_z ? eps_z + ez_off[i] : nullptr,
-                                   eps_src ? eps_src + es_off[i] : nullptr, cseed[i], vc, cap_vc, s, cfeats[i], cL[i]);
+                                   eps_src ? eps_src + es_off[i] : nullptr, cseed[i], vc, cap_vc, s, cfeats[i], cL[i],
+                                   o.t_pad_tgt);
     const int64_t keep = nvc - 2 * o.t_pad_tgt;
     if (keep <= 0) throw Error(RVCX_E_SHAPE, "pipeline: chunk too short for the padding");
     if (nch == 1) {
@@ -534,7 +538,10 @@
   float* vc = c.buf<float>("pb.vc", (size_t)B * nvc, s);
   {
     ScopedFullLengths full(c);
-    synth_forward(c, B, (int)Tv, phone, meta, pc, pf, meta + B, eps_z, eps_src, seed, vc, nullptr, nullptr, s);
+    DecWindow win;
+    if (o.t_pad_tgt > 0 && c.use_dec_window()) win = {o.t_pad_tgt, nvc - o.t_pad_tgt};
+    synth_forward(c, B, (int)Tv, phone, meta, pc, pf, meta + B, eps_z, eps_src, seed, vc, nullptr, nullptr, s, 0, 0,
+                  nullptr, nullptr, win);
   }
   const int64_t keep = nvc - 2 * o.t_pad_tgt;
   if (keep <= 0) throw Error(RVCX_E_SHAPE, "pipeline_batch: utterance too short for the padding");
diff --git a/retrieval-based-voice-conversion-mlx_amd/csrc/runtime_stream.cpp b/retrieval-based-voice-conversion-mlx_amd/csrc/runtime_stream.cpp
--- a/retrieval-based-voice-conversion-mlx_amd/csrc/runtime_stream.cpp
+++ b/retrieval-based-voice-conversion-mlx_amd/csrc/runtime_stream.cpp
@@ -409,12 +409,17 @@
     eps_src = es;
   }
   float* model = c.buf<float>("rt.model", (size_t)Ba * n_model, st);
+  const int64_t n_need = std::min<int64_t>(n_model, (int64_t)s.sola48 + s.block48 + s.cross48);
+  int64_t n_clip = n_model;
   {
     ScopedFullLengths full(c);
+    DecWindow win;
+    if (s.out_identity && !any_rms && c.use_dec_window()) win = {0, n_need};
     synth_forward(c, Ba, T, phone, dmeta, guided ? pitch : nullptr, guided ? pitchf : nullptr, dmeta + B, eps_z,
-                  eps_src, seed, model, nullptr, nullptr, st, gen_precision);
-  }
-  check(rt_clip(model, n_model, (int)n_model, Ba, st), "rt_clip");
+                  eps_src, seed, model, nullptr, nullptr, st, gen_precision, 0, nullptr, nullptr, win);
+    if (win.s1 >= 0) n_clip = n_need;
+  }
+  check(rt_clip(model, n_model, (int)n_clip, Ba, st), "rt_clip");
   if (any_rms) {
     const int n1 = rms_frame_count(s.conv16, 16000), n2 = rms_frame_count(n_model, s.tgt_sr);
     float* ws = c.buf<float>("rt.rms", (size_t)Ba * (n1 + n2), st);
diff --git a/retrieval-based-voice-conversion-mlx_amd/csrc/runtime_synth.cpp b/retrieval-based-voice-conversion-mlx_amd/csrc/runtime_synth.cpp
--- a/retrieval-based-voice-conversion-mlx_amd/csrc/runtime_synth.cpp
+++ b/retrieval-based-voice-conversion-mlx_amd/csrc/runtime_synth.cpp
@@ -387,8 +387,40 @@
   return true;
 }
 
+int dec_margin_frames(const SynthCfg& cf) {
+  long long E = (7 - 1) / 2;
+  long long rb = 0;
+  for (size_t j = 0; j < cf.rb_k.size(); ++j) {
+    const int k = cf.rb_k[j];
+    long long r = 0;
+    for (int d : cf.rb_d[j]) r += (long long)(k - 1) * d / 2 + (k - 1) / 2;
+    rb = std::max(rb, r);
+  }
+  for (size_t i = cf.ups.size(); i-- > 0;) {
+    const int u = cf.ups[i], k = cf.up_k[i];
+    E += rb;
+    E = (E + u - 1) / u + std::max(1, (k + u - 1) / u - 1);
+  }
+  return (int)(E + (7 - 1) / 2);
+}
+
+constexpr int DEC_WINDOW_MIN_DROP = 4;
+void dec_window_frames(const SynthCfg& cf, int T, const DecWindow& win, int& fa, int& fb) {
+  fa = 0;
+  fb = T;
+  if (win.s1 < 0 || cf.vocoder != 0) return;
+  const long long upp = cf.upp(), M = dec_margin_frames(cf);
+  const long long s0 = std::max<long long>(0, win.s0), s1 = std::min<long long>(win.s1, (long long)T * upp);
+  if (s1 <= s0) return;
+  const long long a = std::max<long long>(0, s0 / upp - M), b = std::min<long long>(T, (s1 + upp - 1) / upp + M);
+  if (T - (b - a) < DEC_WINDOW_MIN_DROP) return;
+  fa = (int)a;
+  fb = (int)b;
+}
+
 void dec_forward(Ctx& c, int B, int T, const float* z_btc, const float* mask, const float* f0, const float* g,
-                 const float* eps_src, uint64_t seed, float* out, hipStream_t s, int gen_lowp, bool noise_pre) {
+                 const float* eps_src, uint64_t seed, float* out, hipStream_t s, int gen_lowp, bool noise_pre,
+                 const DecWindow& win) {
   const SynthCfg& cf = c.scfg;
   if (cf.f0 && cf.vocoder == 2) {
     refinegan_forward(c, B, T, z_btc, mask, f0, g, eps_src, seed, out, s);
@@ -396,6 +428,10 @@
   }
   const int I = cf.I, C0 = cf.C0;
   const long long har_ld = (long long)T * cf.upp() + 2 * HAR_PAD;
+  int fa, fb;
+  dec_window_frames(cf, T, win, fa, fb);
+  const int Tc = fb - fa;
+  const long long har_off = (long long)fa * cf.upp();
   float* har = nullptr;
   if (cf.f0) {
     if (noise_pre) {
@@ -406,9 +442,9 @@
   }
   float* cv = c.buf<float>("dec.cvec", (size_t)B * C0, s);
   run(c, lin(g, cf.gin, B, cf.gin, c.W("dec.cond.w"), C0, c.W("dec.cond.b"), cv, C0), s);
-  size_t maxe = (size_t)T * C0;
+  size_t maxe = (size_t)Tc * C0;
   {
-    long long t = T;
+    long long t = Tc;
     for (size_t i = 0; i < cf.ups.size(); ++i) {
       t *= cf.ups[i];
       maxe = std::max(maxe, (size_t)t * (C0 >> (i + 1)));
@@ -419,8 +455,11 @@
   float* R = c.buf<float>("dec.r", (size_t)B * maxe, s);
   float* t1 = c.buf<float>("dec.t", (size_t)B * maxe, s);
   {
-    ConvArgs a = conv(z_btc, I, T, I, c.W("dec.pre.w"), C0, 7, 1, 3, c.W("dec.pre.b"), xin, C0, T, B);
-    a.pre_mask = mask;
+    ConvArgs a =
+        conv(z_btc + (size_t)fa * I, I, Tc, I, c.W("dec.pre.w"), C0, 7, 1, 3, c.W("dec.pre.b"), xin, C0, Tc, B);
+    a.x_bs = (long long)T * I;
+    a.plan_T = T;
+    a.pre_mask = mask + fa;
     a.pre_mask_bs = T;
     a.res = cv;
     a.ldr = 0;
@@ -429,12 +468,15 @@
     run(c, a, s);
   }
   float* cur = xin;
-  int curT = T, Cin = C0;
+  int curT = Tc, Cin = C0;
+  long long fullT = T, off = fa;
   const int nk = (int)cf.rb_k.size();
   for (size_t i = 0; i < cf.ups.size(); ++i) {
     const UpsLayer& L = c.ups[i];
     const int C = L.cout, u = L.u, Ti = curT * u;
+    const long long fullTi = fullT * u, offi = off * u;
     ConvArgs a = conv(cur, Cin, curT, Cin, L.w, u * C, L.taps, 1, L.pad, L.b, y, u * C, curT, B);
+    a.plan_T = (int)fullT;
     a.w_static = 1;
     a.lowp = gen_lowp;
     a.pre_act = ACT_LRELU;
@@ -451,13 +493,13 @@
       nn = "dec.noise_convs." + std::to_string(i);
       const int kk = ntap * stride;
       if (noise_pre && kk > 1) {
-        a.res = c.buf<float>("dec.nz" + std::to_string(i), (size_t)B * Ti * C, s);
+        a.res = c.buf<float>("dec.nz" + std::to_string(i), (size_t)B * fullTi * C, s) + (size_t)offi * C;
         a.ldr = u * C;
-        a.res_bs = (long long)Ti * C;
+        a.res_bs = fullTi * C;
         a.res_mode = RES_ADD_POST;
         nz_fused = true;
       } else if (kk == 1 && conv_routes_wsb16(c, a)) {
-        a.nz_har = har + HAR_PAD - npad;
+        a.nz_har = har + HAR_PAD - npad + har_off;
         a.nz_bs = har_ld;
         a.nz_stride = stride;
         a.nz_kk = ntap * stride;
@@ -470,13 +512,14 @@
     }
     run(c, a, s, 2.0 * B * curT * (double)Cin * C * L.k);
     if (cf.f0 && !nz_fused) {
-      if (noise_row_kernel(nf, B, Ti, C)) {
-        check(noise_conv_add(har + HAR_PAD - npad, har_ld, stride, ntap, c.W(nn + ".wf"), c.W(nn + ".b"), y, B, Ti,
-                             C, s),
+      const float* hsrc = har + HAR_PAD - npad + har_off;
+      if (noise_row_kernel(nf, B, fullTi, C)) {
+        check(noise_conv_add(hsrc, har_ld, stride, ntap, c.W(nn + ".wf"), c.W(nn + ".b"), y, B, Ti, C, s),
               "noise_conv_add");
       } else {
-        ConvArgs an = conv(har + HAR_PAD - npad, stride, Ti + ntap - 1, stride, c.W(nn + ".wf"), C, ntap, 1, 0,
-                           c.W(nn + ".b"), y, C, Ti, B);
+        ConvArgs an = conv(hsrc, stride, Ti + ntap - 1, stride, c.W(nn + ".wf"), C, ntap, 1, 0, c.W(nn + ".b"), y, C, Ti,
+                           B);
+        an.plan_T = (int)fullTi;
         an.x_bs = har_ld;
         an.acc_mode = ACC_ADD;
         run(c, an, s, 2.0 * B * (double)Ti * C * kern);
@@ -528,6 +571,7 @@
         const std::string n1 = rb + ".convs1." + std::to_string(m);
         const std::string n2 = rb + ".convs2." + std::to_string(m);
         ConvArgs a1 = conv(r_in, C, Ti, C, c.W(n1 + ".w"), C, k, d, (k * d - d) / 2, c.W(n1 + ".b"), T1, C, Ti, B);
+        a1.plan_T = (int)fullTi;
         a1.w_static = 1;
         a1.lowp = gen_lowp;
         a1.pre_act = ACT_LRELU;
@@ -537,6 +581,7 @@
         const bool last = (m + 1 == dil.size());
         float* dst = last ? S : RR;
         ConvArgs a2 = conv(T1, C, Ti, C, c.W(n2 + ".w"), C, k, 1, (k - 1) / 2, c.W(n2 + ".b"), dst, C, Ti, B);
+        a2.plan_T = (int)fullTi;
         a2.w_static = 1;
         a2.lowp = gen_lowp;
         run(c, a1, s);
@@ -555,15 +600,18 @@
     cur = S;
     curT = Ti;
     Cin = C;
-  }
-  check(conv_post_tanh(cur, B, curT, Cin, c.W("dec.post.w"), 7, 0.01f, out, s, c.host[0].at("__post_b__").v[0]),
+    fullT = fullTi;
+    off = offi;
+  }
+  check(conv_post_tanh(cur, B, curT, Cin, c.W("dec.post.w"), 7, 0.01f, out + har_off, s,
+                       c.host[0].at("__post_b__").v[0], fullT),
         "conv_post");
 }
 
 void synth_forward(Ctx& c, int B, int T, const float* phone, const int32_t* lengths, const int32_t* pitch,
                    const float* pitchf, const int32_t* sid, const float* eps_z, const float* eps_src, uint64_t seed,
                    float* out, float* zp_out, float* z_out, hipStream_t s, int gen_lowp, int head, float* mp_out,
-                   float* logsp_out) {
+                   float* logsp_out, const DecWindow& win) {
   const SynthCfg& cf = c.scfg;
   const int H = cf.H, I = cf.I, F = cf.F, E = cf.emb_dim, nh = cf.n_heads, dk = H / nh;
   const long long BT = (long long)B * T;
@@ -727,7 +775,7 @@
   }
   if (z_out) RVCX_HIP(hipMemcpyAsync(z_out, z, BTf * I * sizeof(float), hipMemcpyDeviceToDevice, s));
   join_aux(c, s, nax);
-  dec_forward(c, B, Tf, z, maskf, pitchff, g, eps_src, seed, out, s, gen_lowp, noise_pre);
-}
-
-}
+  dec_forward(c, B, Tf, z, maskf, pitchff, g, eps_src, seed, out, s, gen_lowp, noise_pre, win);
+}
+
+}
diff --git a/retrieval-based-voice-conversion-mlx_amd/csrc/rvcx_kernels.h b/retrieval-based-voice-conversion-mlx_amd/csrc/rvcx_kernels.h
--- a/retrieval-based-voice-conversion-mlx_amd/csrc/rvcx_kernels.h
+++ b/retrieval-based-voice-conversion-mlx_amd/csrc/rvcx_kernels.h
@@ -96,6 +96,7 @@
   int wsplit_fmt = 0;
   int ksplit = 1;
   int no_splitk = 0;
+  int plan_T = 0;
   int lowp = 0;
   long long ws_rows = 0;
   float* ws = nullptr;
@@ -209,7 +210,7 @@
 hipError_t sine_source(const float* f0, int B, int L, int upp, float sr, const float* eps, uint64_t seed,
                        float lin_w, float lin_b, double* cum_ws, float* har, long long har_ld, hipStream_t s);
 hipError_t conv_post_tanh(const float* x, int B, int T, int C, const float* w, int K, float slope, float* y,
-                          hipStream_t s, float bias = 0.f);
+                          hipStream_t s, float bias = 0.f, long long y_bs = 0);
 size_t harm_source_ws_doubles(int B, int L, int upp, int H);
 hipError_t resample_dw(const float* x, int B, int T_in, int C, const float* ker, int K, int orig, int width, float* y,
                        int T_out, hipStream_t s);
diff --git a/retrieval-based-voice-conversion-mlx_amd/rvcx/_lib.py b/retrieval-based-voice-conversion-mlx_amd/rvcx/_lib.py
--- a/retrieval-based-voice-conversion-mlx_amd/rvcx/_lib.py
+++ b/retrieval-based-voice-conversion-mlx_amd/rvcx/_lib.py
@@ -28,7 +28,8 @@
     "rvcx_workspace_bytes", "rvcx_set_workspace", "rvcx_workspace_info", "rvcx_crepe_ex",
     "rvcx_crepe_decode", "rvcx_set_fcpe_config", "rvcx_fcpe", "rvcx_fcpe_decode", "rvcx_fcpe_b",
 ]
-TEST_EXPORTS = ["rvcx_performer_attention", "rvcx_performer_attention_b", "rvcx_fcpe_mel"]
+TEST_EXPORTS = ["rvcx_performer_attention", "rvcx_performer_attention_b", "rvcx_fcpe_mel", "rvcx_set_dec_window",
+                "rvcx_dec_margin_frames"]
 
 
 class RvcxLibraryError(ImportError):
@@ -166,6 +167,8 @@
         "rvcx_fcpe_decode": (i32, [vp, vp, i64, f32, i32, i32, i64, vp, vp]),
         "rvcx_fcpe_b": (i32, [vp, vp, i64, i64, i32, f32, i32, vp, vp, vp]),
         "rvcx_fcpe_mel": (i32, [vp, vp, i64, vp, i64, P(i64), vp]),
+        "rvcx_set_dec_window": (i32, [vp, i32]),
+        "rvcx_dec_margin_frames": (i32, [P(SynthDesc), P(i32)]),
         "rvcx_performer_attention": (i32, [vp, vp, vp, vp, i32, i32, vp, i32, vp, vp]),
         "rvcx_performer_attention_b": (i32, [vp, vp, vp, vp, i32, i32, i32, vp, i32, vp, vp]),
         "rvcx_split_audio": (i32, [vp, vp, i64, i32, f64, i32, P(i64), i64, P(i64), vp]),
diff --git a/retrieval-based-voice-conversion-mlx_amd/rvcx/engine.py b/retrieval-based-voice-conversion-mlx_amd/rvcx/engine.py
--- a/retrieval-based-voice-conversion-mlx_amd/rvcx/engine.py
+++ b/retrieval-based-voice-conversion-mlx_amd/rvcx/engine.py
@@ -66,7 +66,8 @@
             return x.to(device=self.device, dtype=dtype).contiguous()
         return t.as_tensor(np.ascontiguousarray(x), dtype=dtype, device=self.device).contiguous()
 
-    def set_synth_config(self, cfg: SynthConfig = SYNTH_48K_V2):
+    @staticmethod
+    def _synth_desc(cfg: SynthConfig):
         d = _lib.SynthDesc()
         d.inter_channels, d.hidden_channels, d.filter_channels = cfg.inter_channels, cfg.hidden_channels, \
             cfg.filter_channels
@@ -88,8 +89,23 @@
         if cfg.vocoder not in _lib.VOCODERS:
             raise ValueError(f"unknown vocoder {cfg.vocoder!r}; expected one of {sorted(_lib.VOCODERS)}")
         d.vocoder = _lib.VOCODERS[cfg.vocoder]
+        return d
+
+    def set_synth_config(self, cfg: SynthConfig = SYNTH_48K_V2):
+        d = self._synth_desc(cfg)
         self._check(self.lib.rvcx_set_synth_config(self.ctx, ctypes.byref(d)), "set_synth_config")
         self.synth_cfg = cfg
+
+    def set_dec_window(self, on: bool):
+        self._check(self.lib.rvcx_set_dec_window(self.ctx, 1 if on else 0), "set_dec_window")
+
+    def dec_margin_frames(self, cfg: SynthConfig = None) -> int:
+        d = self._synth_desc(cfg if cfg is not None else self.synth_cfg)
+        m = ctypes.c_int32(0)
+        rc = self.lib.rvcx_dec_margin_frames(ctypes.byref(d), ctypes.byref(m))
+        if rc != 0:
+            raise _lib.RvcxError(rc, "dec_margin_frames: bad synthesizer configuration")
+        return m.value
 
     def upload_state(self, model: int, state: Mapping[str, np.ndarray]):
         for name, arr in state.items():
```

Measured after the change: 1162 audio-sec/sec (median of 6 runs). 6.4% higher.
